# Luka140/paig_reproduction

Measured on AMD Instinct MI355X. Metric: video-seqs/sec (train step) spring_color B=100 @ 1/2/4/8 MI355X, higher is better.
Workload: dtype fp32; 1 GPU; spring_color PhysicsNet train step (get_batch gather+fwd+loss+bwd+allreduce+RMSprop), B=100/rank, 32x32x3, seq_len 50 (4 in / 6 pred / 40 extrap); global_batch=100, seq_len=50, parallelism=dp1, conv_math=split, split_graph=False, optimizer_in_graph=True, byte_targets=True, dataset_seqs=800

## Files before the change

include/paig_hip.h:

```cpp
#ifndef PAIG_HIP_H
#define PAIG_HIP_H
#include <stddef.h>

#ifdef __cplusplus
extern "C" {
#endif

#define PAIG_ABI_VERSION 10
const char* paig_last_error(void);
int paig_abi_version(void);
int paig_f16_range_status(int clear);

int paig_conv2d_fwd(const float* in, long long in_fs, int in_grp, long long in_gs, float* out, long long out_fs,
                    const float* aux, long long aux_fs, const float* w, const float* bias, int F, int Cin, int Cout,
                    int H, int W, int ks, int flags, void* stream);
#define PAIG_XMAX_SLOTS 2048
int paig_conv2d_fwd_ex(const float* in, long long in_fs, int in_grp, long long in_gs, float* out, long long out_fs,
                       const float* aux, long long aux_fs, const float* w, const float* bias, int F, int Cin,
                       int Cout, int H, int W, int ks, int flags, float* xmax, int xmax_n, void* stream);
int paig_conv2d_fwd_pw(const float* in, long long in_fs, int in_grp, long long in_gs, float* out, long long out_fs,
                       const float* aux, long long aux_fs, const float* w, const float* bias, int F, int Cin,
                       int Cout, int H, int W, int ks, int flags, float* xmax, int xmax_n, float* pool_out,
                       long long pool_fs, const void* wprep, void* stream);
int paig_conv2d_fwd_pwc(const float* in, long long in_fs, int in_grp, long long in_gs, float* out, long long out_fs,
                        const float* aux, long long aux_fs, const float* w, const float* bias, int F, int Cin,
                        int Cout, int H, int W, int ks, int flags, float* xmax, int xmax_n, float* pool_out,
                        long long pool_fs, unsigned char* pool_code, long long pool_code_fs, const void* wprep,
                        void* stream);
long long paig_conv_wprep_size(int cin, int cout, int ks);
int paig_conv_wprep(int n, const float* const* w, const int* cin, const int* cout, const int* ks, const int* dg,
                    void* const* out, void* stream);
int paig_conv_wprep_defer(int n, const float* const* w, const int* cin, const int* cout, const int* ks, const int* dg,
                          void* const* out, void* stream);
int paig_conv_wprep_flush(void* stream);
int paig_debug_fwd_block_cap(int cap);
int paig_conv2d_mfma_supported(int what, int Cin, int Cout, int H, int W, int ks, int flags);
int paig_conv2d_wgrad(const float* x, long long x_fs, int x_grp, long long x_gs, const float* dy, long long dy_fs,
                      float* slab, int nblk_max, int* nblk_out, int F, int Cin, int Cout, int H, int W, int ks,
                      int flags, void* stream);
int paig_conv2d_wgrad_ex(const float* x, long long x_fs, int x_grp, long long x_gs, const float* dy, long long dy_fs,
                         float* slab, int nblk_max, int* nblk_out, int F, int Cin, int Cout, int H, int W, int ks,
                         int flags, const float* xmax, int xmax_n, void* stream);
int paig_conv2d_bwd_supported(int Cin, int Cout, int H, int W, int ks, int flags);
int paig_conv2d_bwd(const float* x, long long x_fs, int x_grp, long long x_gs, const float* dy, long long dy_fs,
                    float* dx, long long dx_fs, const float* aux, long long aux_fs, const float* w, float* slab,
                    int nblk_max, int* nblk_out, int F, int Cin, int Cout, int H, int W, int ks, int flags,
                    const float* xmax, int xmax_n, const float* dpool, long long dpool_fs,
                    const unsigned char* pcode, long long pcode_fs, const void* wprep, void* stream);

size_t paig_unet_workspace(int net, int F, int H, int K, int math);
int paig_unet_fwd(int net, int F, int H, int K, int math, const float* x, long long x_fs, int x_grp, long long x_gs,
                  const float* const* w, const float* const* b, float* logits, void* ws, size_t ws_bytes,
                  void* stream);
int paig_unet_bwd(int net, int F, int H, int K, int math, const float* x, long long x_fs, int x_grp, long long x_gs,
                  const float* const* w, const float* logits, const float* dlogits, float* const* dwb, void* ws,
                  size_t ws_bytes, void* stream);
#define PAIG_UNET_HEAD_FUSED 1
#define PAIG_UNET_SEPARATE_BWD 2
#define PAIG_UNET_INFERENCE 4
#define PAIG_UNET_EXT_WPREP 8
#define PAIG_UNET_STANDALONE_UP 16
#define PAIG_UNET_STANDALONE_POOL 32
#define PAIG_PROBE_CONV_FWD 0
#define PAIG_PROBE_CONV_BWD 1
#define PAIG_PROBE_CONV_WGRAD 2
#define PAIG_PROBE_CONV_DGRAD 3
typedef void (*paig_unet_probe_fn)(void* ctx, int event, int op, int conv, int kind, int cin, int cout, int H,
                                   int flags);
size_t paig_unet_workspace_ex(int net, int F, int H, int K, int math, int flags);
long long paig_unet_buffer(int net, int F, int H, int K, int math, int flags, int which, int buf);
int paig_unet_query(int net, int K, int what);
int paig_unet_fwd_ex(int net, int F, int H, int K, int math, int flags, const float* x, long long x_fs, int x_grp,
                     long long x_gs, const float* const* w, const float* const* b, float* logits,
                     const void* const* wprep_fwd, const void* const* wprep_dg, void* ws, size_t ws_bytes,
                     paig_unet_probe_fn probe, void* probe_ctx, void* stream);
int paig_unet_bwd_ex(int net, int F, int H, int K, int math, int flags, const float* x, long long x_fs, int x_grp,
                     long long x_gs, const float* const* w, const float* logits, const float* dlogits,
                     float* const* dwb, int n_extra, const float* const* extra_src, const int* extra_nblk,
                     const int* extra_len, float* const* extra_dst, const void* const* wprep_dg, void* ws,
                     size_t ws_bytes, paig_unet_probe_fn probe, void* probe_ctx, void* stream);

int paig_conv2d_wgrad_pf(const float* x, long long x_fs, int x_grp, long long x_gs, const float* dy, long long dy_fs,
                         const float* dpool, long long dpool_fs, const unsigned char* pcode, long long pcode_fs,
                         float* slab, int nblk_max, int* nblk_out, int F, int Cin, int Cout, int H, int W, int ks,
                         int flags, const float* xmax, int xmax_n, void* stream);

int paig_maxpool2_fwd(const float* x, long long x_fs, float* y, long long y_fs, int F, int C, int H, int W,
                      void* stream);
int paig_maxpool2_fwd_codes(const float* x, long long x_fs, float* y, long long y_fs, unsigned char* code,
                            long long code_fs, int F, int C, int H, int W, void* stream);
int paig_maxpool2_bwd_relu(const float* x, long long x_fs, const float* dy, long long dy_fs, float* dx, long long dx_fs,
                           int F, int C, int H, int W, void* stream);
int paig_upsample2_fwd(const float* s, long long s_fs, float* u, long long u_fs, int F, int C, int Hs, int Ws, int Ho,
                       int Wo, void* stream);
int paig_upsample2_bwd(const float* du, long long du_fs, const float* s, long long s_fs, float* ds, long long ds_fs,
                       int F, int C, int Hs, int Ws, int Ho, int Wo, int relu_mask, void* stream);

int paig_mask_softmax_fwd(const float* logits, const float* x, long long x_fs, int x_grp, long long x_gs, float* masks,
                          float* objs, float* pobjs, int F, int K, int C, int H, int W, void* stream);
int paig_mask_softmax_bwd(const float* logits, const float* x, long long x_fs, int x_grp, long long x_gs,
                          const float* masks, const float* dobjs, float* dlogits, int F, int K, int C, int H, int W,
                          int flags, void* stream);
int paig_head_mask_blocks(int F, int H, int W);
int paig_head_mask_fwd(const float* x12, const float* w, const float* b, const float* x, long long x_fs, int x_grp,
                       long long x_gs, float* masks, float* objs, int F, int K, int H, int W, void* stream);
int paig_head_mask_bwd(const float* x12, const float* w, const float* b, const float* x, long long x_fs, int x_grp,
                       long long x_gs, const float* masks, const float* dobjs, float* dx12, float* slab, int F, int K,
                       int H, int W, void* stream);
int paig_head_mask_fwd_ex(const float* xl, const float* w, const float* b, const float* x, long long x_fs, int x_grp,
                          long long x_gs, float* masks, float* objs, float* pobjs, int F, int K, int CI, int H, int W,
                          int flags, void* stream);
int paig_head_mask_bwd_ex(const float* xl, const float* w, const float* b, const float* x, long long x_fs, int x_grp,
                          long long x_gs, const float* masks, const float* dobjs, float* dxl, float* slab, int F, int K,
                          int CI, int H, int W, int flags, void* stream);
int paig_pos_head_fwd(const float* h3, float* pos, int N, int K, float half, void* stream);
int paig_pos_head_bwd(const float* h3, const float* dpos, float* dh3, int N, int K, float half, void* stream);

size_t paig_gemm_workspace(int M, int N, int K);
int paig_gemm_defer_epilogue(int on);
int paig_gemm_flush(void* stream);
int paig_gemm(int ta, int tb, int M, int N, int K, float alpha, const float* A, long long lda, const float* B,
              long long ldb, float beta, float* C, long long ldc, const float* bias, int act, int auxm,
              const float* aux, long long ldaux, float* rowsum, float* ws, size_t ws_floats, void* stream);
int paig_gemm_ex(int ta, int tb, int M, int N, int K, float alpha, const float* A, long long lda, const float* B,
                 long long ldb, float beta, float* C, long long ldc, const float* bias, int act, int auxm,
                 const float* aux, long long ldaux, float* rowsum, float* ws, size_t ws_floats, int math,
                 void* stream);
size_t paig_gemm_parts_size(int M, int N, int K, int math);
int paig_gemm_parts(int ta, int tb, int M, int N, int K, const float* A, long long lda, const float* B,
                    long long ldb, float* part, size_t part_floats, int math, void* stream);
size_t paig_colsum_workspace(int M, int N);
int paig_colsum(const float* X, int M, int N, long long ld, float* out, int accumulate, float* ws, void* stream);
int paig_slab_reduce(const float* slab, int nblk, long long ld, int len, float* out, int accumulate, void* stream);
int paig_slab_reduce_multi(int ntask, const float* const* src, const int* nblk, const int* len, float* const* dst,
                           int accumulate, void* stream);
int paig_axpby(const float* x, float* y, long long n, float a, float b, void* stream);

int paig_vfn_fwd(const float* W1, const float* b1, const float* W2, const float* b2, float* hout, float* y,
                 float* ypost, int P, void* stream);
int paig_vfn_bwd_blocks(int P);
int paig_vfn_bwd(const float* d, const float* y, int sig, const float* h, const float* W2, float* dW1, float* db1,
                 float* dW2, float* db2, float* part, int P, void* stream);
int paig_vfn_fwd_multi(int n, const float* const* W1, const float* const* b1, const float* const* W2,
                       const float* const* b2, float* const* hout, float* const* y, float* const* ypost, const int* P,
                       void* stream);
int paig_vfn_bwd_multi(int n, const float* const* d, const float* const* y, const int* sig, const float* const* h,
                       const float* const* W2, float* const* dW1, float* const* db1, float* const* dW2,
                       float* const* db2, float* const* part, const int* P, void* stream);
int paig_vfn_bwd1_multi(int n, const float* const* d, const float* const* y, const int* sig, const float* const* h,
                        const float* const* W2, float* const* dW1, float* const* db1, float* const* dW2,
                        float* const* db2, float* const* part, const int* P, void* stream);

int paig_velmlp_fwd(const float* pos, int B, int Te, int K, int S, const float* W0, const float* b0, const float* W2,
                    const float* b2, const float* W4, const float* b4, float* X, float* h1, float* h2, float* vel,
                    void* stream);
int paig_velmlp_vfn_fwd(const float* pos, int B, int Te, int K, int S, const float* W0, const float* b0,
                        const float* W2, const float* b2, const float* W4, const float* b4, float* X, float* h1,
                        float* h2, float* vel, int n, const float* const* vW1, const float* const* vb1,
                        const float* const* vW2, const float* const* vb2, float* const* hout, float* const* y,
                        float* const* ypost, const int* P, void* stream);
int paig_velmlp_bwd_blocks(int rows);
int paig_velmlp_slab_len(int S);
int paig_velmlp_bwd(const float* dvel, const float* X, const float* h1, const float* h2, const float* W0,
                    const float* W2, const float* W4, float* dX, float* slab, int rows, int S, void* stream);

int paig_head_fwd(const float* h2, const float* W3, const float* b3, float* h3, float* pos, int F, int K, int IN,
                  float half, void* stream);
int paig_head_bwd_blocks(int rows);
int paig_head_bwd(const float* h2, const float* h3, const float* dpos, const float* W3, float* dh2, float* slab, int F,
                  int K, int IN, float half, void* stream);
int paig_head_bwd_vel(const float* h2, const float* h3, const float* dpos, const float* W3, float* dh2, float* slab,
                      int F, int K, int IN, float half, const float* dX, const float* dpos0, int B, int Te, int S,
                      int alt, void* stream);
int paig_head_bwd_vel_vfn2(const float* h2, const float* h3, const float* dpos, const float* W3, float* dh2,
                           float* slab, int F, int K, int IN, float half, const float* dX, const float* dpos0, int B,
                           int Te, int S, int alt, int n, const float* const* d, const float* const* y,
                           const int* sig, const float* const* h, const float* const* W2, float* const* dW1,
                           float* const* db1, float* const* dW2, float* const* db2, float* const* part, const int* P,
                           void* stream);

int paig_dense_tail_fwd(const float* part, int S, const float* b1, float* h1, const float* W2, float* W2t,
                        const float* b2, float* h2, const float* W3, const float* b3, float* h3, float* pos, int F,
                        int K, int IN, float half, void* stream);
int paig_head_l2_bwd_blocks(int rows);
int paig_head_l2_bwd(const float* h2, const float* h3, const float* dpos, const float* W3, float* dh2, float* slab,
                     int F, int K, int IN, float half, const float* dX, const float* dpos0, int B, int Te, int S,
                     int alt, const float* W2, const float* h1, float* dh1, int n, const float* const* d,
                     const float* const* y, const int* sig, const float* const* h, const float* const* vW2,
                     float* const* dW1, float* const* db1, float* const* dW2, float* const* db2, float* const* part,
                     const int* P, void* stream);

size_t paig_localiser_workspace(int F, int K, int n1, int IN, int math);
int paig_localiser_fwd(const float* x1, const float* W1, const float* b1, const float* W2, const float* b2,
                       const float* W3, const float* b3, float* h1, float* h2, float* h3, float* pos, int F, int K,
                       int n1, int IN, float half, int math, void* ws, size_t ws_bytes, void* stream);
int paig_localiser_bwd(const float* dpos, const float* x1, const float* h1, const float* h2, const float* h3,
                       const float* W1, const float* W2, const float* W3, float* dl1, float* dl2, float* dl3,
                       float* dx1, int F, int K, int n1, int IN, float half, int math, void* ws, size_t ws_bytes,
                       void* stream);
int paig_velmlp_rollout_fwd(int cell, const float* pos, int B, int Te, int K, int S, const float* W0, const float* b0,
                            const float* W2, const float* b2, const float* W4, const float* b4, float* X, float* h1,
                            float* h2, float* vel0, const float* dt, const double* p0, const double* p1, float* pvs,
                            int R, void* stream);
size_t paig_velmlp_rollout_bwd_workspace(int B, int K, int S);
int paig_velmlp_rollout_bwd(int cell, const float* pvs, const float* dpos_roll, const float* dpvs, const float* dt,
                            const double* p0, const double* p1, const float* X, const float* h1, const float* h2,
                            const float* W0, const float* W2, const float* W4, float* dpos, float* dmlp,
                            double* gparam0, double* gparam1, int B, int Te, int K, int S, int R, void* ws,
                            size_t ws_bytes, void* stream);

int paig_vel_pack(const float* pos, float* X, int B, int Te, int K, int S, int alt, void* stream);
int paig_vel_unpack_add(const float* dX, const float* dpos0, float* dpos, int B, int Te, int K, int S, int alt,
                        void* stream);

int paig_rollout_fwd(int cell, const float* pos0, long long pos0_ld, const float* vel0, const float* dt,
                     const double* p0, const double* p1, float* pvs, int B, int D, int R, void* stream);
int paig_rollout_bwd_blocks(int B);
int paig_rollout_bwd(int cell, const float* pvs, const float* dpos_roll, const float* dpvs, const float* dt,
                     const double* p0, const double* p1, float* dpos0, float* dvel0, double* part, double* gparam0,
                     double* gparam1, int accumulate, int B, int D, int R, void* stream);

int paig_decoder_fwd(const float* pos, long long pos_outer, long long pos_inner, int pos_grp, const float* tmpl,
                     const float* cont, const float* bg, float* out, long long out_fs, const float* tgt,
                     long long tgt_fs, int tgt_grp, long long tgt_gs, float* sse, int F, int K, int h, int H,
                     void* stream);
int paig_decoder_fwd_rollout(int cell, const float* pos0, long long pos0_ld, const float* vel0, const float* dt,
                             const double* p0, const double* p1, float* pvs, int B, int D, int R, const float* pos,
                             long long pos_outer, long long pos_inner, int pos_grp, const float* tmpl,
                             const float* cont, const float* bg, float* out, long long out_fs, const float* tgt,
                             long long tgt_fs, int tgt_grp, long long tgt_gs, float* sse, int F, int K, int h, int H,
                             void* stream);
int paig_decoder_fwd_t8(const float* pos, long long pos_outer, long long pos_inner, int pos_grp, const float* tmpl,
                        const float* cont, const float* bg, float* out, long long out_fs, const unsigned char* tgt,
                        const long long* tgt_idx, long long tgt_fs, int tgt_grp, long long tgt_gs, float* sse, int F,
                        int K, int h, int H, void* stream);
int paig_decoder_bwd_blocks(int F, int pos_grp, int live, int K, int h, int H);
size_t paig_decoder_slab_len(int K, int h, int H);
size_t paig_decoder_bwd_scratch(int F, int K, int h, int H);
int paig_decoder_bwd(const float* pos, long long pos_outer, long long pos_inner, int pos_grp, const float* tmpl,
                     const float* cont, const float* bg, const float* tgt, long long tgt_fs, int tgt_grp,
                     long long tgt_gs, const float* dsse, const float* dout, long long dout_fs, float* dpos,
                     float* slab, float* scratch, int F, int live, int K, int h, int H, void* stream);
int paig_decoder_bwd_ex(const float* pos, long long pos_outer, long long pos_inner, int pos_grp, const float* tmpl,
                        const float* cont, const float* bg, const float* tgt, const unsigned char* tgt8,
                        const long long* tgt_idx, long long tgt_fs, int tgt_grp, long long tgt_gs, const float* dsse,
                        int lw_mode, const float* dt, const float* de, const float* dr, float ae, int lB, int lTe,
                        int lR, int lpred, const float* dout, long long dout_fs, float* dpos, float* slab,
                        float* scratch, int F, int live, int K, int h, int H, void* stream);
int paig_decoder_bwd_t8(const float* pos, long long pos_outer, long long pos_inner, int pos_grp, const float* tmpl,
                        const float* cont, const float* bg, const unsigned char* tgt, const long long* tgt_idx,
                        long long tgt_fs, int tgt_grp, long long tgt_gs, const float* dsse, const float* dout,
                        long long dout_fs, float* dpos, float* slab, float* scratch, int F, int live, int K, int h,
                        int H, void* stream);

int paig_decoder_fwd_sigma(const float* pos, long long pos_outer, long long pos_inner, int pos_grp, const float* tmpl,
                           const float* cont, const float* bg, float* out, long long out_fs, const float* tgt,
                           long long tgt_fs, int tgt_grp, long long tgt_gs, float* sse, int F, int K, int h, int H,
                           double sigma, void* stream);
int paig_decoder_fwd_rollout_sigma(int cell, const float* pos0, long long pos0_ld, const float* vel0, const float* dt,
                                   const double* p0, const double* p1, float* pvs, int B, int D, int R,
                                   const float* pos, long long pos_outer, long long pos_inner, int pos_grp,
                                   const float* tmpl, const float* cont, const float* bg, float* out, long long out_fs,
                                   const float* tgt, long long tgt_fs, int tgt_grp, long long tgt_gs, float* sse, int F,
                                   int K, int h, int H, double sigma, void* stream);
int paig_decoder_fwd_t8_sigma(const float* pos, long long pos_outer, long long pos_inner, int pos_grp,
                              const float* tmpl, const float* cont, const float* bg, float* out, long long out_fs,
                              const unsigned char* tgt, const long long* tgt_idx, long long tgt_fs, int tgt_grp,
                              long long tgt_gs, float* sse, int F, int K, int h, int H, double sigma, void* stream);
int paig_decoder_bwd_blocks_sigma(int F, int pos_grp, int live, int K, int h, int H, double sigma);
size_t paig_decoder_bwd_scratch_sigma(int F, int K, int h, int H, double sigma);
int paig_decoder_bwd_ex_sigma(const float* pos, long long pos_outer, long long pos_inner, int pos_grp,
                              const float* tmpl, const float* cont, const float* bg, const float* tgt,
                              const unsigned char* tgt8, const long long* tgt_idx, long long tgt_fs, int tgt_grp,
                              long long tgt_gs, const float* dsse, int lw_mode, const float* dt, const float* de,
                              const float* dr, float ae, int lB, int lTe, int lR, int lpred, const float* dout,
                              long long dout_fs, float* dpos, float* slab, float* scratch, int F, int live, int K,
                              int h, int H, double sigma, void* stream);
int paig_decoder_parts_sigma(const float* pos, long long pos_inner, const float* tmpl, const float* cont,
                             const float* bg, float* contents, float* masks, int F, int K, int h, int H, double sigma,
                             void* stream);

int paig_decoder_parts(const float* pos, long long pos_inner, const float* tmpl, const float* cont, const float* bg,
                       float* contents, float* masks, int F, int K, int h, int H, void* stream);
// ... 45 lines not shown
```

paig_reproduction_amd/_lib.py:

```python
import ctypes
import os

import torch

_HERE = os.path.dirname(os.path.abspath(__file__))
LIB_PATH = os.path.join(_HERE, "libpaig_hip.so")
XMAX_SLOTS = 2048

AB_PATH = os.environ.get("PAIG_AB_LIB")
ABI_VERSION = 10

P = ctypes.c_void_p
I = ctypes.c_int
LL = ctypes.c_longlong
F32 = ctypes.c_float
F64 = ctypes.c_double
SZ = ctypes.c_size_t

SIGNATURES = {
    "paig_last_error": (ctypes.c_char_p, []),
    "paig_abi_version": (I, []),
    "paig_f16_range_status": (I, [I]),
    "paig_conv2d_fwd": (I, [P, LL, I, LL, P, LL, P, LL, P, P, I, I, I, I, I, I, I, P]),
    "paig_conv2d_wgrad": (I, [P, LL, I, LL, P, LL, P, I, P, I, I, I, I, I, I, I, P]),
    "paig_conv2d_fwd_ex": (I, [P, LL, I, LL, P, LL, P, LL, P, P, I, I, I, I, I, I, I, P, I, P]),
    "paig_conv2d_fwd_pw": (I, [P, LL, I, LL, P, LL, P, LL, P, P, I, I, I, I, I, I, I, P, I, P, LL, P, P]),
    "paig_conv_wprep_size": (LL, [I, I, I]),
    "paig_conv_wprep": (I, [I, P, P, P, P, P, P, P]),
    "paig_conv_wprep_defer": (I, [I, P, P, P, P, P, P, P]),
    "paig_conv_wprep_flush": (I, [P]),
    "paig_conv2d_wgrad_ex": (I, [P, LL, I, LL, P, LL, P, I, P, I, I, I, I, I, I, I, P, I, P]),
    "paig_conv2d_wgrad_pf": (I, [P, LL, I, LL, P, LL, P, LL, P, LL, P, I, P, I, I, I, I, I, I, I, P, I, P]),
    "paig_conv2d_mfma_supported": (I, [I, I, I, I, I, I, I]),
    "paig_debug_fwd_block_cap": (I, [I]),
    "paig_conv2d_bwd_supported": (I, [I, I, I, I, I, I]),
    "paig_conv2d_bwd": (I, [P, LL, I, LL, P, LL, P, LL, P, LL, P, P, I, P, I, I, I, I, I, I, I, P, I, P, LL, P, LL,
                            P, P]),
    "paig_conv2d_fwd_pwc": (I, [P, LL, I, LL, P, LL, P, LL, P, P, I, I, I, I, I, I, I, P, I, P, LL, P, LL, P, P]),
    "paig_gather_u8_f32": (I, [P, P, P, I, LL, P]),
    "paig_gather_u8_f32_ex": (I, [P, P, P, I, LL, LL, P, P]),
    "paig_velmlp_fwd": (I, [P, I, I, I, I, P, P, P, P, P, P, P, P, P, P, P]),
    "paig_velmlp_vfn_fwd": (I, [P, I, I, I, I, P, P, P, P, P, P, P, P, P, P, I, P, P, P, P, P, P, P, P, P]),
    "paig_velmlp_bwd_blocks": (I, [I]),
    "paig_velmlp_slab_len": (I, [I]),
    "paig_velmlp_bwd": (I, [P, P, P, P, P, P, P, P, P, I, I, P]),
    "paig_head_fwd": (I, [P, P, P, P, P, I, I, I, F32, P]),
    "paig_dense_tail_fwd": (I, [P, I, P, P, P, P, P, P, P, P, P, P, I, I, I, F32, P]),
    "paig_head_l2_bwd": (I, [P, P, P, P, P, P, I, I, I, F32, P, P, I, I, I, I, P, P, P, I, P, P, P, P, P, P, P, P, P,
                             P, P, P]),
    "paig_head_bwd_blocks": (I, [I]),
    "paig_head_l2_bwd_blocks": (I, [I]),
    "paig_head_bwd": (I, [P, P, P, P, P, P, I, I, I, F32, P]),
    "paig_head_bwd_vel": (I, [P, P, P, P, P, P, I, I, I, F32, P, P, I, I, I, I, P]),
    "paig_head_bwd_vel_vfn2": (I, [P, P, P, P, P, P, I, I, I, F32, P, P, I, I, I, I, I, P, P, P, P, P, P, P, P, P, P, P,
                                   P]),
    "paig_unet_workspace": (SZ, [I, I, I, I, I]),
    "paig_localiser_workspace": (SZ, [I, I, I, I, I]),
    "paig_localiser_fwd": (I, [P, P, P, P, P, P, P, P, P, P, P, I, I, I, I, F32, I, P, SZ, P]),
    "paig_localiser_bwd": (I, [P, P, P, P, P, P, P, P, P, P, P, P, I, I, I, I, F32, I, P, SZ, P]),
    "paig_velmlp_rollout_fwd": (I, [I, P, I, I, I, I, P, P, P, P, P, P, P, P, P, P, P, P, P, P, I, P]),
    "paig_velmlp_rollout_bwd_workspace": (SZ, [I, I, I]),
    "paig_velmlp_rollout_bwd": (I, [I, P, P, P, P, P, P, P, P, P, P, P, P, P, P, P, P, I, I, I, I, I, P, SZ, P]),
    "paig_unet_fwd": (I, [I, I, I, I, I, P, LL, I, LL, P, P, P, P, SZ, P]),
    "paig_unet_bwd": (I, [I, I, I, I, I, P, LL, I, LL, P, P, P, P, P, SZ, P]),
    "paig_unet_workspace_ex": (SZ, [I, I, I, I, I, I]),
    "paig_unet_buffer": (LL, [I, I, I, I, I, I, I, I]),
    "paig_unet_query": (I, [I, I, I]),
    "paig_unet_fwd_ex": (I, [I, I, I, I, I, I, P, LL, I, LL, P, P, P, P, P, P, SZ, P, P, P]),
    "paig_unet_bwd_ex": (I, [I, I, I, I, I, I, P, LL, I, LL, P, P, P, P, I, P, P, P, P, P, P, SZ, P, P, P]),
    "paig_maxpool2_fwd": (I, [P, LL, P, LL, I, I, I, I, P]),
    "paig_maxpool2_fwd_codes": (I, [P, LL, P, LL, P, LL, I, I, I, I, P]),
    "paig_maxpool2_bwd_relu": (I, [P, LL, P, LL, P, LL, I, I, I, I, P]),
    "paig_upsample2_fwd": (I, [P, LL, P, LL, I, I, I, I, I, I, P]),
    "paig_upsample2_bwd": (I, [P, LL, P, LL, P, LL, I, I, I, I, I, I, I, P]),
    "paig_mask_softmax_fwd": (I, [P, P, LL, I, LL, P, P, P, I, I, I, I, I, P]),
    "paig_mask_softmax_bwd": (I, [P, P, LL, I, LL, P, P, P, I, I, I, I, I, I, P]),
    "paig_head_mask_blocks": (I, [I, I, I]),
    "paig_head_mask_fwd": (I, [P, P, P, P, LL, I, LL, P, P, I, I, I, I, P]),
    "paig_head_mask_bwd": (I, [P, P, P, P, LL, I, LL, P, P, P, P, I, I, I, I, P]),
    "paig_head_mask_fwd_ex": (I, [P, P, P, P, LL, I, LL, P, P, P, I, I, I, I, I, I, P]),
    "paig_head_mask_bwd_ex": (I, [P, P, P, P, LL, I, LL, P, P, P, P, I, I, I, I, I, I, P]),
    "paig_pos_head_fwd": (I, [P, P, I, I, F32, P]),
    "paig_pos_head_bwd": (I, [P, P, P, I, I, F32, P]),
    "paig_gemm_workspace": (SZ, [I, I, I]),
    "paig_gemm_parts_size": (SZ, [I, I, I, I]),
    "paig_gemm_parts": (I, [I, I, I, I, I, P, LL, P, LL, P, SZ, I, P]),
    "paig_gemm_defer_epilogue": (I, [I]),
    "paig_gemm_flush": (I, [P]),
    "paig_gemm": (I, [I, I, I, I, I, F32, P, LL, P, LL, F32, P, LL, P, I, I, P, LL, P, P, SZ, P]),
    "paig_gemm_ex": (I, [I, I, I, I, I, F32, P, LL, P, LL, F32, P, LL, P, I, I, P, LL, P, P, SZ, I, P]),
    "paig_colsum_workspace": (SZ, [I, I]),
    "paig_colsum": (I, [P, I, I, LL, P, I, P, P]),
    "paig_slab_reduce": (I, [P, I, LL, I, P, I, P]),
    "paig_slab_reduce_multi": (I, [I, P, P, P, P, I, P]),
    "paig_axpby": (I, [P, P, LL, F32, F32, P]),
    "paig_vfn_fwd": (I, [P, P, P, P, P, P, P, I, P]),
    "paig_vfn_bwd_blocks": (I, [I]),
    "paig_vfn_bwd": (I, [P, P, I, P, P, P, P, P, P, P, I, P]),
    "paig_vfn_fwd_multi": (I, [I, P, P, P, P, P, P, P, P, P]),
    "paig_vfn_bwd_multi": (I, [I, P, P, P, P, P, P, P, P, P, P, P, P]),
    "paig_vfn_bwd1_multi": (I, [I, P, P, P, P, P, P, P, P, P, P, P, P]),
    "paig_vel_pack": (I, [P, P, I, I, I, I, I, P]),
    "paig_vel_unpack_add": (I, [P, P, P, I, I, I, I, I, P]),
    "paig_rollout_fwd": (I, [I, P, LL, P, P, P, P, P, I, I, I, P]),
    "paig_rollout_bwd_blocks": (I, [I]),
    "paig_rollout_bwd": (I, [I, P, P, P, P, P, P, P, P, P, P, P, I, I, I, I, P]),
    "paig_decoder_fwd": (I, [P, LL, LL, I, P, P, P, P, LL, P, LL, I, LL, P, I, I, I, I, P]),
    "paig_decoder_fwd_rollout": (I, [I, P, LL, P, P, P, P, P, I, I, I, P, LL, LL, I, P, P, P, P, LL, P, LL, I, LL, P, I, I,
                                      I, I, P]),
    "paig_decoder_fwd_t8": (I, [P, LL, LL, I, P, P, P, P, LL, P, P, LL, I, LL, P, I, I, I, I, P]),
    "paig_decoder_bwd_blocks": (I, [I, I, I, I, I, I]),
    "paig_decoder_slab_len": (SZ, [I, I, I]),
    "paig_decoder_bwd_scratch": (SZ, [I, I, I, I]),
    "paig_decoder_bwd": (I, [P, LL, LL, I, P, P, P, P, LL, I, LL, P, P, LL, P, P, P, I, I, I, I, I, P]),
    "paig_decoder_bwd_ex": (I, [P, LL, LL, I, P, P, P, P, P, P, LL, I, LL, P, I, P, P, P, F32, I, I, I, I, P, LL, P, P, P,
                                 I, I, I, I, I, P]),
    "paig_decoder_bwd_t8": (I, [P, LL, LL, I, P, P, P, P, P, LL, I, LL, P, P, LL, P, P, P, I, I, I, I, I, P]),
    "paig_decoder_parts": (I, [P, LL, P, P, P, P, P, I, I, I, I, P]),
    "paig_decoder_fwd_sigma": (I, [P, LL, LL, I, P, P, P, P, LL, P, LL, I, LL, P, I, I, I, I, F64, P]),
    "paig_decoder_fwd_rollout_sigma": (I, [I, P, LL, P, P, P, P, P, I, I, I, P, LL, LL, I, P, P, P, P, LL, P, LL, I, LL,
                                            P, I, I, I, I, F64, P]),
    "paig_decoder_fwd_t8_sigma": (I, [P, LL, LL, I, P, P, P, P, LL, P, P, LL, I, LL, P, I, I, I, I, F64, P]),
    "paig_decoder_bwd_blocks_sigma": (I, [I, I, I, I, I, I, F64]),
    "paig_decoder_bwd_scratch_sigma": (SZ, [I, I, I, I, F64]),
    "paig_decoder_bwd_ex_sigma": (I, [P, LL, LL, I, P, P, P, P, P, P, LL, I, LL, P, I, P, P, P, F32, I, I, I, I, P, LL, P,
                                       P, P, I, I, I, I, I, F64, P]),
    "paig_decoder_parts_sigma": (I, [P, LL, P, P, P, P, P, I, I, I, I, F64, P]),
    "paig_stn_fwd": (I, [P, P, P, I, I, I, I, I, I, P]),
    "paig_stn_bwd": (I, [P, P, P, P, P, I, I, I, I, I, I, P]),
    "paig_stn_fwd_f64": (I, [P, P, P, I, I, I, I, I, I, P]),
    "paig_stn_bwd_f64": (I, [P, P, P, P, P, I, I, I, I, I, I, P]),
    "paig_relu_mask": (I, [P, P, LL, P]),
    "paig_loss_reduce": (I, [P, P, I, I, I, I, F32, P, P, P, P]),
    "paig_loss_bwd": (I, [P, P, P, F32, P, P, I, I, I, I, P]),
    "paig_frame_sse": (I, [P, LL, I, LL, P, LL, I, LL, P, I, I, P]),
    "paig_frame_sse_bwd": (I, [P, LL, I, LL, P, LL, I, LL, P, P, I, I, P]),
    "paig_synth_integrate": (I, [I, P, P, LL, I, I, I, F64, F64, F64, F64, F64, P, P, P]),
    "paig_synth_raster": (I, [P, P, LL, I, I, I, F64, P, P, P]),
    "paig_rmsprop_f32": (I, [P, P, P, LL, F32, F32, F32, P]),
    "paig_rmsprop_f64": (I, [P, P, P, LL, F64, F64, F64, P]),
    "paig_rmsprop_mixed": (I, [P, P, P, LL, P, P, P, LL, F64, F64, F64, P]),
    "paig_adam_f32": (I, [P, P, P, P, LL, F32, F32, F32, F32, F32, F32, P]),
    "paig_adam_f64": (I, [P, P, P, P, LL, F64, F64, F64, F64, F64, F64, P]),
    "paig_sgd_f32": (I, [P, P, P, LL, F32, F32, I, P]),
    "paig_sgd_f64": (I, [P, P, P, LL, F64, F64, I, P]),
}

_QUERY = {"paig_last_error", "paig_abi_version", "paig_f16_range_status", "paig_conv2d_mfma_supported",
          "paig_debug_fwd_block_cap",
          "paig_conv2d_bwd_supported", "paig_velmlp_bwd_blocks",
          "paig_velmlp_slab_len", "paig_head_bwd_blocks", "paig_head_l2_bwd_blocks", "paig_head_mask_blocks", "paig_conv_wprep_size", "paig_gemm_workspace", "paig_colsum_workspace",
          "paig_gemm_parts_size", "paig_gemm_parts", "paig_unet_workspace", "paig_unet_workspace_ex",
          "paig_unet_buffer", "paig_unet_query", "paig_localiser_workspace",
          "paig_velmlp_rollout_bwd_workspace",
          "paig_vfn_bwd_blocks", "paig_rollout_bwd_blocks", "paig_decoder_bwd_blocks", "paig_decoder_slab_len",
          "paig_decoder_bwd_scratch", "paig_decoder_bwd_blocks_sigma", "paig_decoder_bwd_scratch_sigma"}


class PaigError(RuntimeError):
    pass


class _Lib:
    def __init__(self, path=LIB_PATH):
        if not os.path.exists(path):
            raise PaigError(f"libpaig_hip.so not built at {path}: run `make -C paig_reproduction_amd/csrc` "
                            "(or __graft_entry__.build()); there is no CPU fallback")
        self.path = path
        self.dll = ctypes.CDLL(path)
        self.dll.paig_abi_version.restype = I
        self.dll.paig_abi_version.argtypes = []
        ver = self.dll.paig_abi_version()
        if ver != ABI_VERSION:
            raise PaigError(f"{path}: C ABI version {ver}, this binding is version {ABI_VERSION}")
        self.fns = {}
        for name, (rt, args) in SIGNATURES.items():
            if path != LIB_PATH and not hasattr(self.dll, name):
                continue
            f = getattr(self.dll, name)
            f.restype = rt
            f.argtypes = args
            self.fns[name] = f

    def __getattr__(self, name):
        fns = self.__dict__.get("fns")
        if fns is None or name not in fns:
            raise AttributeError(name)
        f = fns[name]
        if name in _QUERY:
            return f

        def call(*a):
            rc = f(*a)
            if rc != 0:
                msg = self.fns["paig_last_error"]().decode(errors="replace")
                raise PaigError(f"{name} failed (rc={rc}): {msg}")
            return rc

        call.__name__ = name
        return call


_lib = None


def lib():
    global _lib
    if _lib is None:
        _lib = _Lib(AB_PATH or LIB_PATH)
    return _lib


def ptr(t):
    return None if t is None else t.data_ptr()


def stream_handle(device=None):
    return torch.cuda.current_stream(device).cuda_stream


def require_device(t):
    if not (torch.is_tensor(t) and t.is_cuda):
        raise PaigError("paig_reproduction_amd runs only on a HIP device (MI355X); got a "
                        f"{'CPU' if torch.is_tensor(t) else type(t).__name__} tensor. There is no CPU fallback.")
```

paig_reproduction_amd/csrc/conv_split.hip:

```cpp
#include "split_common.h"

#ifndef PAIG_FWD_AUXP
#define PAIG_FWD_AUXP 1
#endif

namespace {


constexpr bool sfwd_sla(bool UPS, int PM, int H, int W, int ups_bytes, int lo_bytes) {
  return UPS && PM == 0 && H * W >= 4096 && ups_bytes <= lo_bytes;
}
constexpr int sfwd_lds(int CIN, int H, int W, int KS, bool UPS, int PM, int tpxm, int ntb) {
  const int CC = rup(CIN, 8) / 8, PS = CC % 2 == 0 ? CC + 1 : CC;
  const int NS = ceil_div(KS * KS * CC, 4);
  const int FPT = H * W <= tpxm ? tpxm / (H * W) : 1;
  const int RT = H * W <= tpxm ? H : rows_fit(H, W, tpxm);
  const int TWPX = W + 2 * (KS / 2);
  const int RP = W == 8 ? to_mod16(TWPX * PS, 8) : TWPX * PS;
  const int img = FPT * (RT + KS - 1) * RP * 8, wimg = NS * ntb * 64 * 8;
  const int ups = UPS ? up_window_floats(CIN, FPT, RT, W) * 4 : 0;
  return (img + wimg) * 2 * (PM == 2 ? 1 : 2) + (sfwd_sla(UPS, PM, H, W, ups, img * 2) ? 0 : ups);
}
constexpr int sfwd_vgprs(int CIN, int H, int W, int KS, bool UPS, int tpxm, int ntb) {
  const int CC = rup(CIN, 8) / 8, NS = ceil_div(KS * KS * CC, 4);
  const int FPT = H * W <= tpxm ? tpxm / (H * W) : 1;
  const int RT = H * W <= tpxm ? H : rows_fit(H, W, tpxm);
  const int MW = ceil_div(ceil_div(FPT * RT * W, 16), 4);
  const int NL = UPS ? 1 : ceil_div(FPT * (RT + KS - 1) * (W % 2 == 0 ? W / 2 : W) * CC, 256);
  return MW * ntb * 4 + NL * 30 + ntb * 8 + NS + MW * 8 + 40;
}
#ifndef PAIG_FWD_UPS_TP
#define PAIG_FWD_UPS_TP 256
#endif
#ifndef PAIG_FWD_TP32
#define PAIG_FWD_TP32 256
#endif
constexpr int sfwd_pick(int CIN, int COUT, int H, int W, int KS, bool UPS, int PM) {
  const int base = UPS && H * W < 4096 && PAIG_FWD_UPS_TP < 256   ? PAIG_FWD_UPS_TP
                   : !UPS && H * W == 1024 && PAIG_FWD_TP32 < 256 ? PAIG_FWD_TP32
                                                                  : (W == 8 ? 128 : 256);
  const int NT = ceil_div(COUT, 16);
  for (int pass = UPS && !(PM == 0 && H * W >= 4096) ? 1 : 0; pass < 3; ++pass)
    for (int nb = 1; nb <= NT; ++nb) {
      if (NT % nb != 0 || NT / nb > 4) continue;
      for (int tp = base; tp >= (pass == 1 ? base / 2 : 64); tp /= 2)
        if (sfwd_lds(CIN, H, W, KS, UPS, PM, tp, NT / nb) <= (pass == 0 ? LDS_MAX / 2 : LDS_MAX) &&
            sfwd_vgprs(CIN, H, W, KS, UPS, tp, NT / nb) <= 264 && (pass > 0 || tp >= base / 2))
          return tp * 256 + nb;
    }
  return 0;
}

template <int CIN, int COUT, int H, int W, int KS, bool UPS, int PM>
struct SFwdCfg {
  static constexpr int KK = KS * KS, PADL = KS / 2;
  static constexpr int NIMG = PM == 2 ? 1 : 2;
  static constexpr int CINP = rup(CIN, 8), CC = CINP / 8;
  static constexpr int KC = KK * CC, NS = ceil_div(KC, 4);
  static constexpr int GEO = sfwd_pick(CIN, COUT, H, W, KS, UPS, PM);
  static_assert(GEO > 0, "no forward tile geometry fits the LDS");
  static constexpr int NB = GEO % 256;
  static constexpr int NT = ceil_div(COUT, 16) / NB;
  static constexpr int TPXM = GEO / 256;
  static constexpr int FPT = H * W <= TPXM ? TPXM / (H * W) : 1;
  static constexpr int RT = H * W <= TPXM ? H : rows_fit(H, W, TPXM);
  static constexpr int TPXV = FPT * RT * W;
  static constexpr int NMT = ceil_div(TPXV, 16);
  static constexpr int MW = ceil_div(NMT, 4);
  static constexpr int ROWS = RT + KS - 1;
  static constexpr int TWPX = W + 2 * PADL;
  static constexpr int PS = CC % 2 == 0 ? CC + 1 : CC;
  static constexpr int RP = W == 8 ? to_mod16(TWPX * PS, 8) : TWPX * PS;
  static constexpr int IMG = FPT * ROWS * RP * 8;
  static constexpr int WIMG = NS * NT * 64 * 8;
  static constexpr int SLB = UPS ? up_window_floats(CIN, FPT, RT, W) * 4 : 0;
  static constexpr bool SLA = sfwd_sla(UPS, PM, H, W, SLB, IMG * 2);
  static constexpr int LDS = (IMG + WIMG) * 2 * NIMG + (SLA ? 0 : SLB);
  static constexpr int UPX = W % 2 == 0 ? 2 : 1;
  static constexpr int W2 = W / UPX;
  static constexpr int NI = FPT * ROWS * W2 * CC;
  static constexpr int NL = (NI + 255) / 256;
  static constexpr bool VEC4 = W % 4 == 0;
  static_assert(H % RT == 0, "RT divides H");
  static constexpr int PO = W / 16;
  static constexpr bool POOLOK = !UPS && VEC4 && W % 16 == 0 && PO >= 1 && MW % 2 == 0 && NMT == 4 * MW &&
                                 TPXV % (2 * W) == 0 && RT % 2 == 0;
};

__device__ __forceinline__ float pool4(float a, float b, float c, float d) {
  float m = a;
  if (b > m || b != b) m = b;
  if (c > m || c != c) m = c;
  if (d > m || d != d) m = d;
  return m;
}

__device__ __forceinline__ unsigned char pool_code(float a, float b, float c, float d) {
  float m = a;
  int k = 0;
  if (b > m || b != b) { m = b; k = 1; }
  if (c > m || c != c) { m = c; k = 2; }
  if (d > m || d != d) { m = d; k = 3; }
  return (unsigned char)((a > 0.f ? 1 : 0) | (b > 0.f ? 2 : 0) | (c > 0.f ? 4 : 0) | (d > 0.f ? 8 : 0) | (k << 4));
}

template <int MW, int PO, bool POOL>
__device__ __forceinline__ int fwd_mtile(int wv, int mt) {
  if constexpr (POOL) {
    constexpr int HM = MW / 2;
    const int u = wv * HM + mt % HM;
    return ((u / PO) * 2 + mt / HM) * PO + u % PO;
  } else {
    return wv * MW + mt;
  }
}

template <int CIN, int COUT, int H, int W, int KS, bool DG, bool UPS, int PM, bool POOL = false, bool UPT = false,
          bool PF = false>
__device__ __forceinline__ void conv_fwd_split_body(FView in, FViewW out, FView aux, const float* __restrict__ w,
                                                    const float* __restrict__ bias, int F, int flags, int ntiles, XMax xm,
                                                    const s16x8* __restrict__ wp, PoolOut pout, int bx, int gx) {
  using C = SFwdCfg<CIN, COUT, H, W, KS, UPS, PM>;
  static_assert(!PF || (DG && !UPS && !POOL && !UPT && C::UPX == 2 && H % 2 == 0 && CIN % 8 == 0),
                "pool fold: dgrad staging units of one window's pixel pair");
  static_assert(!UPT || (DG && !UPS && !POOL && C::FPT == 1 && C::RT % 2 == 0 && C::VEC4 && W % 2 == 0),
                "transposed-upsample epilogue: dgrad tiles of whole row pairs");
  constexpr int KK = C::KK, CC = C::CC, KC = C::KC, NS = C::NS, NT = C::NT, MW = C::MW;
  constexpr int RT = C::RT, FPT = C::FPT, ROWS = C::ROWS, PS = C::PS, RP = C::RP;
  constexpr int NI = C::NI, NL = C::NL, PADL = C::PADL, W2 = C::W2;
  constexpr long long PLANE = UPS ? (long long)(H / 2) * (W / 2) : (long long)H * W;
  constexpr long long HW = (long long)H * W;
  extern __shared__ __attribute__((aligned(16))) short lds16[];
  short* Xh = lds16;
  short* Xl = Xh + (C::NIMG == 2 ? C::IMG : 0);
  short* Wh = lds16 + C::NIMG * C::IMG;
  short* Wl = Wh + (C::NIMG == 2 ? C::WIMG : 0);
  const int tid = threadIdx.x, lane = tid & 63, wv = tid >> 6, g = lane >> 4;
  constexpr int NRB = H / RT;
  const int co0 = blockIdx.y * NT * 16;
  float rmax = 0.f;
  __shared__ float smax[4];

  auto wval = [&](int idx, int j) {
    const int ln = idx & 63, snt = idx >> 6, nt = snt % NT, s = snt / NT;
    const int kc = 4 * s + (ln >> 4), co = co0 + nt * 16 + (ln & 15);
    float v = 0.f;
    if (kc < KC && co < COUT) {
      const int tap = kc / CC, ci = (kc % CC) * 8 + j;
      if (ci < CIN) v = DG ? w[(ci * COUT + co) * KK + (KK - 1 - tap)] : w[(co * CIN + ci) * KK + tap];
    }
    return v;
  };
  int ewn[NT];
// ... 1056 lines not shown
        float r1 = 0.f;
        stage_d(t, r1, false);
        __syncthreads();
      }
    }
  };

  auto tile_max = [&](int t) {
    if constexpr (!DSYNC) {
      float m = 0.f;
#pragma unroll
      for (int l = 0; l < NLD; ++l) m = amax2(amax2(m, sd[l][0], sd[l][1]), sd[l][2], sd[l][3]);
      m = wave_max_u(m);
      if (lane == 0) smax[wv] = m;
    }
  };

  if ((int)blockIdx.x < ntiles) issue(xcd_tile(blockIdx.x, ntiles));
  if (PM == 0 && xm.p) {
    float m = 0.f;
    for (int i = tid * 4; i < xm.n; i += 1024) {
      const f32x4 v = *reinterpret_cast<const f32x4*>(xm.p + i);
      m = fmaxf(m, fmaxf(fmaxf(v[0], v[1]), fmaxf(v[2], v[3])));
    }
    m = wave_max_u(m);
    if (lane == 0) smax[wv] = m;
    __syncthreads();
    m = fmaxf(fmaxf(smax[0], smax[1]), fmaxf(smax[2], smax[3]));
    if (m > 0.f) ecx = f16_scale_exp(m);
    __syncthreads();
  }
  xsc = __builtin_amdgcn_ldexpf(1.f, ecx);
  for (int lt = blockIdx.x; lt < ntiles; lt += gridDim.x) {
    const int tile = xcd_tile(lt, ntiles);
    fold_all(tile);
    if constexpr (PM == 0 && PAIG_SCALE_MODE < 2) tile_max(tile);
    __syncthreads();
    commit(tile);
    __syncthreads();
    check_sync(tile);
    issue(lt + (int)gridDim.x < ntiles ? xcd_tile(lt + gridDim.x, ntiles) : ntiles);
#pragma unroll
    for (int kb = wp; kb < KB; kb += WP) {
      const int p0 = kb * 32, fi = p0 / (RT * W), pr = p0 % (RT * W);
      const int base = (fi * ROWS + pr / W) * TWPX + pr % W;
      s16x8 ah[MT], al[MT];
#pragma unroll
      for (int m = 0; m < MT; ++m) {
        const int co = m * 16 + (lane & 15);
        const int o = (co < COUTB ? co : co % COUTB) * DP + p0 + 8 * g;
        ah[m] = *reinterpret_cast<const s16x8*>(Dh + o);
        al[m] = PM != 2 ? *reinterpret_cast<const s16x8*>(Dl + o) : ah[m];
      }
      int r0, r1;
      if constexpr (C::FAST) {
        r0 = (base + roff[0]) * 4;
        r1 = (base + roff[1]) * 4;
      } else {
        auto posof = [&](int j) {
          int pp = p0 + j;
          if (pp >= TPXV) pp = 0;
          const int pf = pp / (RT * W), prr = pp % (RT * W);
          return ((pf * ROWS + prr / W) * TWPX + prr % W + (OFFX - PADL)) * 4;
        };
        r0 = posof(8 * g + qq);
        r1 = posof(8 * g + 4 + qq);
      }
      auto ldb = [&](int jn, s16x8& bh, s16x8& bl) {
        if (wn + jn * WN < NT) {
          bh = __builtin_shufflevector(tr_read(Xh + r0 + colt[jn]), tr_read(Xh + r1 + colt[jn]), 0, 1, 2, 3, 4, 5, 6,
                                       7);
          bl = PM != 2 ? __builtin_shufflevector(tr_read(Xl + r0 + colt[jn]), tr_read(Xl + r1 + colt[jn]), 0, 1, 2,
                                                 3, 4, 5, 6, 7)
                       : bh;
        }
      };
      s16x8 bh[2], bl[2];
      ldb(0, bh[0], bl[0]);
#pragma unroll
      for (int jn = 0; jn < NTW; ++jn) {
        if (jn + 1 < NTW) ldb(jn + 1, bh[(jn + 1) & 1], bl[(jn + 1) & 1]);
        if (wn + jn * WN < NT) {
#pragma unroll
          for (int m = 0; m < MT; ++m) acc[m][jn] = mma3<PM>(ah[m], al[m], bh[jn & 1], bl[jn & 1], acc[m][jn]);
        }
      }
    }
  }
  __syncthreads();
  float* R = reinterpret_cast<float*>(lds16);
#pragma unroll
  for (int m = 0; m < MT; ++m)
#pragma unroll
    for (int j = 0; j < NTW; ++j)
#pragma unroll
      for (int r = 0; r < 4; ++r) R[(((wv * MT + m) * NTW + j) * 4 + r) * 64 + lane] = acc[m][j][r];
  __syncthreads();
  float* s = slab + (long long)blockIdx.x * C::SLAB;
  if (wp == 0) {
#pragma unroll
    for (int m = 0; m < MT; ++m)
#pragma unroll
      for (int j = 0; j < NTW; ++j) {
        const int nt = wn + j * WN;
        if (nt >= NT) continue;
        const int col = nt * 16 + (lane & 15), cq = col >> 2;
        const int tap = cq / CQ, ci = (cq % CQ) * 4 + (col & 3);
#pragma unroll
        for (int r = 0; r < 4; ++r) {
          float v = 0.f;
          for (int p = 0; p < WP; ++p) v += R[((((p * WN + wn) * MT + m) * NTW + j) * 4 + r) * 64 + lane];
          const int co = m * 16 + (lane >> 4) * 4 + r;
          if constexpr (PM == 0) v = __builtin_amdgcn_ldexpf(v, -(ecx + ecd));
          if (co < COUTB && cq < NQ && ci < CINB) s[(co0 + co) * NCOL + (ci0 + ci) * KK + tap] = v;
        }
      }
  }
  __syncthreads();
  float* Rb = reinterpret_cast<float*>(lds16);
#pragma unroll
  for (int l = 0; l < NLD; ++l) Rb[l * 256 + tid] = bacc[l];
  __syncthreads();
  if (tid < COUTB && blockIdx.y == 0) {
    float v = 0.f;
    for (int i = tid * NPU; i < (tid + 1) * NPU; ++i) v += Rb[(i / 256) * 256 + i % 256];
    s[COUT * NCOL + co0 + tid] = v;
  }
  if constexpr (PM == 0) f16_range_note(rmax);
}

struct WPrepJob {
  const float* w;
  s16x8* out;
  int cin, cout, ks, dg;
};
constexpr int WPREP_MAX = 64;
struct WPrepJobs {
  WPrepJob j[WPREP_MAX];
  int blk0[WPREP_MAX + 1];
  int n;
};
constexpr int WPREP_T = 256;

__device__ __forceinline__ int wprep_hdr_entries(int cout) { return (cout + 15) / 16 * 16 * 4 / 16; }

#ifndef PAIG_WPREP_S
#define PAIG_WPREP_S 8
#endif
constexpr int WPREP_S = PAIG_WPREP_S;
__device__ __forceinline__ void conv_wprep_body(const WPrepJobs& jobs, int bid) {
  int q = 0;
  while (q + 1 < jobs.n && bid >= jobs.blk0[q + 1]) ++q;
  const WPrepJob jb = jobs.j[q];
  if (jb.dg == 2) {
    __shared__ float T[32][33];
    const int bl = bid - jobs.blk0[q], tx = (bl % ((jb.cin + 31) / 32)) * 32,
              ty = (bl / ((jb.cin + 31) / 32)) * 32, c = threadIdx.x & 31, r = threadIdx.x >> 5;
    for (int y = r; y < 32; y += WPREP_T / 32)
      if (ty + y < jb.cout && tx + c < jb.cin) T[y][c] = jb.w[(long long)(ty + y) * jb.cin + tx + c];
    __syncthreads();
    float* o = reinterpret_cast<float*>(jb.out);
    for (int y = r; y < 32; y += WPREP_T / 32)
      if (tx + y < jb.cin && ty + c < jb.cout) o[(long long)(tx + y) * jb.cout + ty + c] = T[c][y];
    return;
  }
  const int KK = jb.ks * jb.ks, CC = (jb.cin + 7) / 8, KC = KK * CC, NTT = (jb.cout + 15) / 16, NS = (KC + 3) / 4;
  const int NSC = (NS + WPREP_S - 1) / WPREP_S;
  const int bl = bid - jobs.blk0[q], nt = bl / NSC, s0 = (bl % NSC) * WPREP_S;
  const int tid = threadIdx.x;
  auto wv = [&](int kc, int j, int co) {
    float v = 0.f;
    if (kc < KC && co < jb.cout) {
      const int tap = kc / CC, ci = (kc % CC) * 8 + j;
      if (ci < jb.cin) v = jb.dg ? jb.w[(ci * jb.cout + co) * KK + (KK - 1 - tap)] : jb.w[(co * jb.cin + ci) * KK + tap];
    }
    return v;
  };
  __shared__ float red[WPREP_T];
  __shared__ int ex[16];
  const int cl = tid & 15, co = nt * 16 + cl;
  float m = 0.f;
#pragma unroll 8
  for (int i = tid >> 4; i < KC * 8; i += WPREP_T / 16) m = fmaxf(m, fabsf(wv(i >> 3, i & 7, co)));
  red[tid] = m;
  __syncthreads();
  if (tid < 16) {
    float mm = 0.f;
    for (int r = 0; r < WPREP_T / 16; ++r) mm = fmaxf(mm, red[r * 16 + tid]);
    ex[tid] = f16_scale_exp_v(mm);
    if (s0 == 0) reinterpret_cast<int*>(jb.out)[nt * 16 + tid] = ex[tid];
  }
  __syncthreads();
  const int HDR = wprep_hdr_entries(jb.cout), ENT = NS * NTT * 64;
  short* img = reinterpret_cast<short*>(jb.out + HDR);
  const int ns = NS - s0 < WPREP_S ? NS - s0 : WPREP_S;
#pragma unroll 8
  for (int t = tid; t < ns * 64 * 8; t += WPREP_T) {
    const int j = t & 7, ln = (t >> 3) & 63, s = s0 + (t >> 9);
    const int kc = 4 * s + (ln >> 4), c = nt * 16 + (ln & 15);
    float rm = 0.f;
    short h, l;
    split<0>(__builtin_amdgcn_ldexpf(wv(kc, j, c), ex[ln & 15]), h, l, rm);
    const long long e = (long long)(s * NTT + nt) * 64 + ln;
    img[e * 8 + j] = h;
    img[((long long)ENT + e) * 8 + j] = l;
  }
}

__global__ void __launch_bounds__(WPREP_T) conv_wprep_k(WPrepJobs jobs) { conv_wprep_body(jobs, blockIdx.x); }

template <int CIN, int COUT, int H, int W, int KS, int PM>
__global__ void __launch_bounds__(256, 2)
conv_fwd_wprep_k(FView in, FViewW out, FView aux, const float* __restrict__ w, const float* __restrict__ bias, int F,
                 int flags, int ntiles, XMax xm, PoolOut pout, WPrepJobs jobs, int nwp) {
  if ((int)blockIdx.x < nwp) {
    conv_wprep_body(jobs, blockIdx.x);
    return;
  }
  conv_fwd_split_body<CIN, COUT, H, W, KS, false, false, PM>(in, out, aux, w, bias, F, flags, ntiles, xm, nullptr, pout,
                                                            (int)blockIdx.x - nwp, (int)gridDim.x - nwp);
}

WPrepJobs g_wpend{};
int g_wpend_blocks = 0;
int wprep_build(WPrepJobs& jobs, int n, const float* const* w, const int* cin, const int* cout, const int* ks,
                const int* dg, void* const* out, int* blocks_out) {
  jobs = WPrepJobs{};
  jobs.n = n;
  int blocks = 0;
  for (int q = 0; q < n; ++q) {
    PAIG_REQUIRE(w[q] && out[q] && cin[q] > 0 && cout[q] > 0 && ks[q] > 0, "conv_wprep: job %d", q);
    PAIG_REQUIRE(((uintptr_t)out[q] & 15) == 0, "conv_wprep: job %d output not 16-byte aligned", q);
    jobs.j[q] = WPrepJob{w[q], static_cast<s16x8*>(out[q]), cin[q], cout[q], ks[q], dg[q]};
    jobs.blk0[q] = blocks;
    if (dg[q] == 2) {
      blocks += (cin[q] + 31) / 32 * ((cout[q] + 31) / 32);
      continue;
    }
    const int NS = (ks[q] * ks[q] * ((cin[q] + 7) / 8) + 3) / 4;
    blocks += (cout[q] + 15) / 16 * ((NS + WPREP_S - 1) / WPREP_S);
  }
  jobs.blk0[n] = blocks;
  *blocks_out = blocks;
  return 0;
}
int wprep_flush(hipStream_t st) {
  if (!g_wpend_blocks) return 0;
  const int nb = g_wpend_blocks;
  g_wpend_blocks = 0;
  hipLaunchKernelGGL(conv_wprep_k, dim3(nb), dim3(WPREP_T), 0, st, g_wpend);
  PAIG_CHECK_LAUNCH();
  return 0;
}

static int g_fwd_block_cap = 0;
static XMax g_prezero{};

template <int CIN, int COUT, int H, int W, int KS, bool DG, bool UPS, int PM, bool UPT = false, bool PF = false>
static int sfwd_launch(FView in, FViewW out, FView aux, const float* w, const float* b, int F, int flags,
                       hipStream_t st, XMax xm, const void* wp, PoolOut pout) {
  using C = SFwdCfg<CIN, COUT, H, W, KS, UPS, PM>;
  constexpr int LDS = C::LDS;
  static_assert(C::SLB == (UPS ? UpStage<CIN, H, W, C::FPT, C::RT>::SL * 4 : 0), "upsample window bytes");
  const int ntiles = cdiv(F, C::FPT) * (H / C::RT);
  constexpr bool POOLABLE = C::POOLOK && !DG;
  auto k = PF ? conv_fwd_split_k<CIN, COUT, H, W, KS, DG, UPS, PM, false, false, PF>
         : UPT ? conv_fwd_split_k<CIN, COUT, H, W, KS, DG, UPS, PM, false, UPT>
              : (POOLABLE && (flags & 64)) ? conv_fwd_split_k<CIN, COUT, H, W, KS, DG, UPS, PM, POOLABLE>
                                           : conv_fwd_split_k<CIN, COUT, H, W, KS, DG, UPS, PM, false>;
  static int resident[2] = {0, 0};
  const int kv = (POOLABLE && (flags & 64)) ? 1 : 0;
  if (!resident[kv]) {
    if (LDS > 64 * 1024) (void)hipFuncSetAttribute((const void*)k, hipFuncAttributeMaxDynamicSharedMemorySize, LDS);
    resident[kv] = persistent_grid((const void*)k, LDS);
  }
  static const int bpc = [] {
    const char* e = getenv("PAIG_FWD_BPC");
    return e ? atoi(e) : 0;
  }();
  int res = resident[kv];
  if (bpc > 0 && res > bpc * 256) res = bpc * 256;
  int nb = res / C::NB;
  if (nb > (UPT ? F : ntiles)) nb = UPT ? F : ntiles;
  if (g_fwd_block_cap > 0 && nb > g_fwd_block_cap) nb = g_fwd_block_cap;
  if (nb < 1) nb = 1;
  if (PM != 0 || DG) xm.p = nullptr;
  PAIG_REQUIRE(!xm.p || nb <= xm.n, "conv split fwd: %d blocks need more than %d xmax slots", nb, xm.n);
  if (xm.p && g_prezero.z) {
    xm.z = g_prezero.z;
    xm.zn = g_prezero.zn;
    g_prezero = XMax{};
  }
  if (PF) PAIG_REQUIRE(pout.p && pout.code, "conv split dgrad: the pool fold needs the pooled gradient and codes");
  else if (flags & 64) PAIG_REQUIRE(C::POOLOK && pout.p, "conv split fwd: no fused pool for Cin=%d Cout=%d H=%d", CIN, COUT, H);
  if constexpr (CIN == 3 && PM == 0 && !DG && !UPS && !UPT && !PF && C::NB == 1) {
    if (g_wpend_blocks && !(flags & 64)) {
      auto km = conv_fwd_wprep_k<CIN, COUT, H, W, KS, PM>;
      static bool attr = false;
      if (!attr && LDS > 64 * 1024) (void)hipFuncSetAttribute((const void*)km, hipFuncAttributeMaxDynamicSharedMemorySize, LDS);
      attr = true;
      const int nwp = g_wpend_blocks;
      g_wpend_blocks = 0;
      hipLaunchKernelGGL(km, dim3(nwp + nb), dim3(256), LDS, st, in, out, aux, w, b, F, flags, ntiles, xm, pout, g_wpend,
                         nwp);
      PAIG_CHECK_LAUNCH();
      return 0;
    }
  }
  if (int rc = wprep_flush(st)) return rc;
  hipLaunchKernelGGL(k, dim3(nb, C::NB), dim3(256), LDS, st, in, out, aux, w, b, F, flags, ntiles, xm,
                     PM == 0 ? static_cast<const s16x8*>(wp) : nullptr, pout);
  PAIG_CHECK_LAUNCH();
  return 0;
}

template <int CIN, int COUT, int H, int W, int KS, bool UPS, int PM, bool PF = false>
static int swg_launch(FView x, FView dy, float* slab, int nblk_max, int* nblk_out, int F, hipStream_t st, XMax xm,
                      PoolOut pin = PoolOut{nullptr, 0, nullptr, 0}) {
  using C = SWgCfg<CIN, COUT, H, W, KS, UPS, PM>;
  constexpr int STG = C::STG + (UPS && !C::SLA ? UpStage<C::CINB, H, W, C::FPT, C::RT>::SL * 4 : 0);
  constexpr int LDS = STG > C::RED ? STG : C::RED;
  const int ntiles = cdiv(F, C::FPT) * (H / C::RT);
  auto k = conv_wgrad_split_k<CIN, COUT, H, W, KS, UPS, PM, PF>;
  if constexpr (PF) PAIG_REQUIRE(pin.p && pin.code, "conv split wgrad: the pool fold needs the pooled gradient and codes");
  static int resident = 0;
  if (!resident) {
    if (LDS > 64 * 1024) (void)hipFuncSetAttribute((const void*)k, hipFuncAttributeMaxDynamicSharedMemorySize, LDS);
    resident = persistent_grid((const void*)k, LDS);
  }
  int nb = ntiles < nblk_max ? ntiles : nblk_max;
  if (nb > resident / (C::NSI * C::NSO)) nb = resident / (C::NSI * C::NSO);
  if (nb < 1) nb = 1;
  *nblk_out = nb;
  PAIG_REQUIRE(!xm.p || (xm.n % 4 == 0 && (reinterpret_cast<uintptr_t>(xm.p) & 15) == 0),
               "conv split wgrad: xmax needs 16-byte alignment and a multiple of 4 slots (%d)", xm.n);
  hipLaunchKernelGGL(k, dim3(nb, C::NSI, C::NSO), dim3(256), LDS, st, x, dy, slab, F, ntiles, xm, pin);
  PAIG_CHECK_LAUNCH();
  return 0;
}

#define PAIG_SPLIT_FWD(X)                                                                                 \
  X(3, 8, 32, 3) X(8, 8, 32, 3) X(8, 16, 16, 3) X(16, 16, 16, 3) X(16, 32, 8, 3) X(32, 32, 8, 3)         \
  X(32, 16, 16, 3) X(16, 16, 32, 3) X(24, 8, 32, 3) X(8, 2, 32, 1) X(16, 8, 16, 3) X(8, 24, 32, 3)       \
  X(2, 8, 32, 1) X(32, 16, 8, 3) X(16, 32, 16, 3)                                                         \
  PAIG_SPLIT_FWD_3BP(X) PAIG_SPLIT_FWD_UNET(X)
#define PAIG_SPLIT_WG(X)                                                                                  \
  X(3, 8, 32, 3) X(8, 8, 32, 3) X(8, 16, 16, 3) X(16, 16, 16, 3) X(16, 32, 8, 3) X(32, 32, 8, 3)         \
  X(32, 16, 16, 3) X(16, 16, 32, 3) X(24, 8, 32, 3) X(8, 2, 32, 1)                                        \
  PAIG_SPLIT_WG_3BP(X) PAIG_SPLIT_WG_UNET(X)
#define PAIG_SPLIT_UP(X)                                                                                  \
  X(32, 16, 16, 3) X(16, 16, 32, 3) X(32, 16, 18, 3) X(16, 16, 36, 3) X(128, 32, 16, 3) X(64, 32, 32, 3) \
  X(32, 32, 64, 3)
#define PAIG_SPLIT_PF(X) X(32, 32, 32, 3) PAIG_SPLIT_PF_C6(X)
#ifndef PAIG_PF_C6
#define PAIG_PF_C6 0
#endif
#if PAIG_PF_C6
#define PAIG_SPLIT_PF_C6(X) X(64, 64, 16, 3)
#else
#define PAIG_SPLIT_PF_C6(X)
#endif
#define PAIG_SPLIT_UPT(X) X(32, 128, 16, 3) X(32, 64, 32, 3) X(32, 32, 64, 3)
#define PAIG_SPLIT_FWD_3BP(X)                                                                             \
  X(3, 8, 36, 3) X(8, 8, 36, 3) X(8, 16, 18, 3) X(16, 16, 18, 3) X(16, 32, 9, 3) X(32, 32, 9, 3)         \
  X(32, 16, 18, 3) X(16, 16, 36, 3) X(24, 8, 36, 3) X(8, 3, 36, 1) X(16, 8, 18, 3) X(32, 16, 9, 3)       \
  X(16, 32, 18, 3) X(8, 24, 36, 3) X(3, 8, 36, 1)
#define PAIG_SPLIT_FWD_UNET(X)                                                                            \
  X(3, 16, 64, 3) X(16, 16, 64, 3) X(16, 32, 32, 3) X(32, 32, 32, 3) X(32, 64, 16, 3) X(64, 64, 16, 3)   \
  X(64, 128, 8, 3) X(128, 128, 8, 3) X(96, 64, 16, 3) X(64, 32, 32, 3) X(48, 16, 64, 3) X(16, 2, 64, 1)   \
  X(32, 16, 32, 3) X(64, 32, 16, 3) X(128, 64, 8, 3) X(32, 128, 16, 3) X(64, 96, 16, 3) X(32, 64, 32, 3)  \
  X(32, 32, 64, 3) X(16, 48, 64, 3) X(2, 16, 64, 1)
#define PAIG_SPLIT_WG_UNET(X)                                                                             \
  X(3, 16, 64, 3) X(16, 16, 64, 3) X(16, 32, 32, 3) X(32, 32, 32, 3) X(32, 64, 16, 3) X(64, 64, 16, 3)   \
  X(64, 128, 8, 3) X(128, 128, 8, 3) X(96, 64, 16, 3) X(64, 32, 32, 3) X(48, 16, 64, 3) X(16, 2, 64, 1)
#define PAIG_SPLIT_WG_3BP(X)                                                                              \
  X(3, 8, 36, 3) X(8, 8, 36, 3) X(8, 16, 18, 3) X(16, 16, 18, 3) X(16, 32, 9, 3) X(32, 32, 9, 3)         \
  X(32, 16, 18, 3) X(16, 16, 36, 3) X(24, 8, 36, 3) X(8, 3, 36, 1)

}

int paig_conv_split_fwd(FView in, FViewW out, FView aux, const float* w, const float* b, int F, int Cin, int Cout,
                        int H, int W, int ks, int flags, hipStream_t st, int* rc, XMax xm, const void* wp,
                        PoolOut pout) {
  const bool dg = (flags & 8) != 0, up = (flags & 32) != 0, b16 = (flags & 256) != 0;
  const int fl = flags & (7 | 64);
  if (H != W || !(flags & (128 | 256))) return 0;
  if (in.grp > 0 && H * W < 256) return 0;
// ... 184 lines not shown
```

paig_reproduction_amd/csrc/gemm.hip:

```cpp
#include "common.h"

#include <algorithm>
#include <cstdlib>

namespace {

constexpr int BM = 64, BN = 64, BK = 32;
constexpr int LDRK = BK + 2;
constexpr int LDKR = 64 + 16;
constexpr int IMG = (BK * LDKR > 64 * LDRK ? BK * LDKR : 64 * LDRK);

typedef float f32x4 __attribute__((ext_vector_type(4)));

__device__ __attribute__((aligned(16))) float zero16[4];

template <bool KCONTIG>
struct Tile {
  f32x4 v[2];
  __device__ __forceinline__ void load(const float* __restrict__ p, long long ld, int r0, int k0, int R, int K,
                                       bool vec, int tid) {
#pragma unroll
    for (int e = 0; e < 2; ++e) {
      int r, k;
      if (KCONTIG) { r = (tid >> 3) + 32 * e; k = (tid & 7) * 4; }
      else { k = (tid >> 4) + 16 * e; r = (tid & 15) * 4; }
      const int gr = r0 + r, gk = k0 + k;
      f32x4 x = f32x4{0.f, 0.f, 0.f, 0.f};
      if (KCONTIG) {
        if (gr < R) {
          const float* q = p + (long long)gr * ld + gk;
          if (vec && gk + 3 < K) x = *reinterpret_cast<const f32x4*>(q);
          else
#pragma unroll
            for (int i = 0; i < 4; ++i) x[i] = (gk + i < K) ? q[i] : 0.f;
        }
      } else {
        if (gk < K) {
          const float* q = p + (long long)gk * ld + gr;
          if (vec && gr + 3 < R) x = *reinterpret_cast<const f32x4*>(q);
          else
#pragma unroll
            for (int i = 0; i < 4; ++i) x[i] = (gr + i < R) ? q[i] : 0.f;
        }
      }
      v[e] = x;
    }
  }
  template <bool VEC>
  __device__ __forceinline__ void load_bf(const float* __restrict__ p, long long ld, int r0, int k0, int R, int K,
                                          int tid) {
#pragma unroll
    for (int e = 0; e < 2; ++e) {
      int r, k;
      if (KCONTIG) { r = (tid >> 3) + 32 * e; k = (tid & 7) * 4; }
      else { k = (tid >> 4) + 16 * e; r = (tid & 15) * 4; }
      const int gr = r0 + r, gk = k0 + k;
      if constexpr (VEC) {
        const bool ok = gr < R && gk < K;
        const float* q = ok ? p + (KCONTIG ? (long long)gr * ld + gk : (long long)gk * ld + gr) : zero16;
        v[e] = *reinterpret_cast<const f32x4*>(q);
      } else {
#pragma unroll
        for (int i = 0; i < 4; ++i) {
          const int rr = KCONTIG ? gr : gr + i, kk = KCONTIG ? gk + i : gk;
          const bool ok = rr < R && kk < K;
          v[e][i] = *(ok ? p + (KCONTIG ? (long long)rr * ld + kk : (long long)kk * ld + rr) : zero16);
        }
      }
    }
  }
  __device__ __forceinline__ void store(float* img, int tid) const {
#pragma unroll
    for (int e = 0; e < 2; ++e) {
      if (KCONTIG) {
        const int r = (tid >> 3) + 32 * e, k = (tid & 7) * 4;
        float* q = img + r * LDRK + k;
        *reinterpret_cast<float2*>(q) = make_float2(v[e][0], v[e][1]);
        *reinterpret_cast<float2*>(q + 2) = make_float2(v[e][2], v[e][3]);
      } else {
        const int k = (tid >> 4) + 16 * e, r = (tid & 15) * 4;
        *reinterpret_cast<f32x4*>(img + k * LDKR + r) = v[e];
      }
    }
  }
  static __device__ __forceinline__ float at(const float* img, int r, int k) {
    return KCONTIG ? img[r * LDRK + k] : img[k * LDKR + r];
  }
};

struct PendEpi {
  int M, N, S;
  const float* part;
  float* C;
  long long ldc;
  float beta;
  const float* bias;
  int act, auxm;
  const float* aux;
  long long ldaux;
  const float* rowpart;
  float* rowsum;
  int v4;
};
__device__ void splitk_epi_run(const PendEpi& pe, int bid, int nb);
#define PAIG_PENDING_EPI(pe)                                                      \
  if ((pe).S && (int)blockIdx.z == (int)gridDim.z - 1) {                          \
    splitk_epi_run((pe), blockIdx.x + gridDim.x * blockIdx.y, gridDim.x * gridDim.y); \
    return;                                                                      \
  }

struct TileId {
  int x, y, z;
};
__device__ __forceinline__ TileId xcd_tile(int gz) {
  const int nx = gridDim.x, ny = gridDim.y, total = nx * ny * gz;
  int lin = blockIdx.x + nx * (blockIdx.y + ny * blockIdx.z);
  if (total % 8 == 0) lin = (lin % 8) * (total / 8) + lin / 8;
  TileId t;
  if (nx <= ny) {
    t.x = lin % nx;
    t.y = (lin / nx) % ny;
    t.z = lin / (nx * ny);
  } else {
    t.y = lin % ny;
    t.x = (lin / ny) % nx;
    t.z = lin / (nx * ny);
  }
  return t;
}

template <bool TA, bool TB>
__global__ void __launch_bounds__(256)
gemm_k(int M, int N, int K, int kchunk, float alpha, const float* __restrict__ A, long long lda, int veca,
       const float* __restrict__ B, long long ldb, int vecb, float* __restrict__ C, long long ldc, float beta,
       const float* __restrict__ bias, int act, int auxm, const float* __restrict__ aux, long long ldaux,
       float* __restrict__ part, float* __restrict__ rowsum, float* __restrict__ rowpart, PendEpi pe) {
  PAIG_PENDING_EPI(pe)
  __shared__ __attribute__((aligned(16))) float As[IMG];
  __shared__ __attribute__((aligned(16))) float Bs[IMG];
  const int tid = threadIdx.x;
  const int lane = tid & 63, wv = tid >> 6;
  const int wm = wv >> 1, wn = wv & 1;
  const TileId bt = xcd_tile((int)gridDim.z - (pe.S ? 1 : 0));
  const int m0 = bt.y * BM, n0 = bt.x * BN;
  const int kbeg = bt.z * kchunk;
  int kend = kbeg + kchunk;
  if (kend > K) kend = K;
  const bool do_rs = rowsum != nullptr && bt.x == 0;

  f32x4 acc[2][2];
#pragma unroll
  for (int i = 0; i < 2; ++i)
#pragma unroll
    for (int j = 0; j < 2; ++j) acc[i][j] = f32x4{0.f, 0.f, 0.f, 0.f};
  float rs = 0.f;

  Tile<!TA> ta;
  Tile<TB> tb;
  if (kbeg < kend) {
    ta.load(A, lda, m0, kbeg, M, kend, veca, tid);
    tb.load(B, ldb, n0, kbeg, N, kend, vecb, tid);
  }
  for (int k0 = kbeg; k0 < kend; k0 += BK) {
    __syncthreads();
    ta.store(As, tid);
    tb.store(Bs, tid);
    __syncthreads();
    if (k0 + BK < kend) {
      ta.load(A, lda, m0, k0 + BK, M, kend, veca, tid);
      tb.load(B, ldb, n0, k0 + BK, N, kend, vecb, tid);
    }
    if (do_rs && tid < BM) {
#pragma unroll 8
      for (int k = 0; k < BK; ++k) rs += Tile<!TA>::at(As, tid, k);
    }
#pragma unroll
    for (int ks = 0; ks < BK; ks += 4) {
      const int kr = ks + (lane >> 4);
      float a[2], b[2];
#pragma unroll
      for (int i = 0; i < 2; ++i) a[i] = Tile<!TA>::at(As, wm * 32 + i * 16 + (lane & 15), kr);
#pragma unroll
      for (int j = 0; j < 2; ++j) b[j] = Tile<TB>::at(Bs, wn * 32 + j * 16 + (lane & 15), kr);
#pragma unroll
      for (int i = 0; i < 2; ++i)
#pragma unroll
        for (int j = 0; j < 2; ++j) acc[i][j] = __builtin_amdgcn_mfma_f32_16x16x4f32(a[i], b[j], acc[i][j], 0, 0, 0);
    }
  }
  if (do_rs && tid < BM && m0 + tid < M) {
    if (rowpart) rowpart[(long long)bt.z * M + m0 + tid] = alpha * rs;
    else rowsum[m0 + tid] = alpha * rs;
  }

#pragma unroll
  for (int i = 0; i < 2; ++i)
#pragma unroll
    for (int j = 0; j < 2; ++j)
#pragma unroll
      for (int r = 0; r < 4; ++r) {
        const int m = m0 + wm * 32 + i * 16 + (lane >> 4) * 4 + r;
        const int n = n0 + wn * 32 + j * 16 + (lane & 15);
        if (m < M && n < N) {
          float v = alpha * acc[i][j][r];
          if (part) {
            part[((long long)bt.z * M + m) * N + n] = v;
          } else {
            if (beta != 0.f) v += beta * C[(long long)m * ldc + n];
            if (bias) v += bias[n];
            C[(long long)m * ldc + n] = epi(v, act, auxm, aux, (long long)m * ldaux + n);
          }
        }
      }
}

typedef short s16x8 __attribute__((ext_vector_type(8)));
typedef short s16x4 __attribute__((ext_vector_type(4)));
typedef __bf16 bf16x8 __attribute__((ext_vector_type(8)));
typedef _Float16 f16x8 __attribute__((ext_vector_type(8)));
typedef __attribute__((address_space(3))) s16x4 lds_s16x4;
typedef unsigned u32x2 __attribute__((ext_vector_type(2)));

constexpr int SPK = 48;
constexpr int SPR = 80;
constexpr int SIMG = 64 * SPK > BK * SPR ? 64 * SPK : BK * SPR;

__device__ __forceinline__ int kperm(int k) {
  const int g = k >> 3, h = (k >> 2) & 1, q = k & 3;
  return 16 * (g >> 1) + 8 * h + 4 * (g & 1) + q;
}

#define F16PM(PM) ((PM) == 1 || (PM) == 4 || (PM) == 5 || (PM) == 6)
#define SCALED(PM) ((PM) >= 4)

template <int PM>
__device__ __forceinline__ void gsplit(float v, short& h, short& l, float& rmax) {
  if constexpr (F16PM(PM)) {
    rmax = fmaxf(rmax, fabsf(v));
    const _Float16 a = (_Float16)v;
    h = __builtin_bit_cast(short, a);
    l = __builtin_bit_cast(short, (_Float16)(v - (float)a));
  } else {
    const __bf16 a = (__bf16)v;
    h = __builtin_bit_cast(short, a);
    l = PM == 2 ? __builtin_bit_cast(short, (__bf16)(v - (float)a)) : (short)0;
  }
}

template <int PM>
__device__ __forceinline__ f32x4 gmma(s16x8 a, s16x8 b, f32x4 c) {
  if constexpr (F16PM(PM))
    return __builtin_amdgcn_mfma_f32_16x16x32_f16(__builtin_bit_cast(f16x8, a), __builtin_bit_cast(f16x8, b), c, 0,
                                                  0, 0);
  else
    return __builtin_amdgcn_mfma_f32_16x16x32_bf16(__builtin_bit_cast(bf16x8, a), __builtin_bit_cast(bf16x8, b), c,
                                                   0, 0, 0);
}

template <bool KCONTIG, int PM>
__device__ __forceinline__ void store16(const Tile<KCONTIG>& t, short* ih, short* il, int tid, float sc,
                                        float& rmax) {
#pragma unroll
  for (int e = 0; e < 2; ++e) {
    s16x4 hv, lv;
    if constexpr (F16PM(PM)) {
      const pf32x2 a = pf32x2{t.v[e][0], t.v[e][1]} * sc, b = pf32x2{t.v[e][2], t.v[e][3]} * sc;
      rmax = amax2(amax2(rmax, a.x, a.y), b.x, b.y);
      u32x2 h, l;
      { const HiLo q_ = split_pk(a.x, a.y); h[0] = q_.h; l[0] = q_.l; }
      { const HiLo q_ = split_pk(b.x, b.y); h[1] = q_.h; l[1] = q_.l; }
      hv = __builtin_bit_cast(s16x4, h);
      lv = __builtin_bit_cast(s16x4, l);
    } else {
#pragma unroll
      for (int i = 0; i < 4; ++i) {
        short h, l;
        gsplit<PM>(t.v[e][i] * sc, h, l, rmax);
        hv[i] = h;
        lv[i] = l;
      }
    }
    int o;
    if (KCONTIG) o = ((tid >> 3) + 32 * e) * SPK + (tid & 7) * 4;
    else o = kperm((tid >> 4) + 16 * e) * SPR + (tid & 15) * 4;
    *reinterpret_cast<s16x4*>(ih + o) = hv;
    if (PM != 3) *reinterpret_cast<s16x4*>(il + o) = lv;
  }
}

template <bool KCONTIG>
__device__ __forceinline__ s16x8 frag16(const short* img, int r0, int lane) {
  if (KCONTIG) return *reinterpret_cast<const s16x8*>(img + (r0 + (lane & 15)) * SPK + 8 * (lane >> 4));
  const int g = lane >> 4, q = (lane >> 2) & 3, p = lane & 3;
  const short* b0 = img + kperm(8 * g + q) * SPR + r0 + 4 * p;
  const short* b1 = img + kperm(8 * g + 4 + q) * SPR + r0 + 4 * p;
  const s16x4 lo = __builtin_amdgcn_ds_read_tr16_b64_v4i16((lds_s16x4*)b0);
  const s16x4 hi = __builtin_amdgcn_ds_read_tr16_b64_v4i16((lds_s16x4*)b1);
  return __builtin_shufflevector(lo, hi, 0, 1, 2, 3, 4, 5, 6, 7);
}

template <bool TA, bool TB, int PM, bool VEC>
__global__ void __launch_bounds__(256) __attribute__((amdgpu_waves_per_eu(6)))
gemm_split_k(int M, int N, int K, int kchunk, float alpha, const float* __restrict__ A, long long lda, int veca,
             const float* __restrict__ B, long long ldb, int vecb, float* __restrict__ C, long long ldc, float beta,
             const float* __restrict__ bias, int act, int auxm, const float* __restrict__ aux, long long ldaux,
             float* __restrict__ part, float* __restrict__ rowsum, float* __restrict__ rowpart, PendEpi pe) {
  PAIG_PENDING_EPI(pe)
  constexpr int NI = PM == 3 ? 1 : 2;
  __shared__ __attribute__((aligned(16))) short S16[4 * SIMG];
  short* Ah = S16;
  short* Al = S16 + SIMG;
  short* Bh = S16 + 2 * SIMG;
  short* Bl = S16 + 3 * SIMG;
  const int tid = threadIdx.x;
  const int lane = tid & 63, wv = tid >> 6;
  const int wm = wv >> 1, wn = wv & 1;
  const TileId bt = xcd_tile((int)gridDim.z - (pe.S ? 1 : 0));
  const int m0 = bt.y * BM, n0 = bt.x * BN;
  const int kbeg = bt.z * kchunk;
  int kend = kbeg + kchunk;
  if (kend > K) kend = K;
  const bool do_rs = TA && rowsum != nullptr && bt.x == 0;

  f32x4 acc[2][2];
#pragma unroll
  for (int i = 0; i < 2; ++i)
#pragma unroll
    for (int j = 0; j < 2; ++j) acc[i][j] = f32x4{0.f, 0.f, 0.f, 0.f};
  f32x4 rs4 = f32x4{0.f, 0.f, 0.f, 0.f};
  float rmax = 0.f;
  constexpr bool DA = PM == 4 || PM == 6, DB = PM == 6;
  int eca = DA ? 100 : (PM == 5 ? PAIG_A_EXP : 0);
  int ecb = DB ? 100 : (PM == 4 || PM == 5 ? PAIG_A_EXP : 0);
  float asc = __builtin_amdgcn_ldexpf(1.f, eca);
  float bsc = __builtin_amdgcn_ldexpf(1.f, ecb);
  __shared__ float smx[8];

  constexpr int NS = 1;
  Tile<!TA> ta[NS];
  Tile<TB> tb[NS];
#pragma unroll
  for (int st = 0; st < NS; ++st) {
    ta[st].template load_bf<VEC>(A, lda, m0, kbeg + st * BK, M, kend, tid);
    tb[st].template load_bf<VEC>(B, ldb, n0, kbeg + st * BK, N, kend, tid);
  }
  for (int k0 = kbeg; k0 < kend; k0 += NS * BK) {
#pragma unroll
    for (int st = 0; st < NS; ++st) {
      const int kk = k0 + st * BK;
      if (kk < kend) {
      if constexpr (DA) {
        float ma = 0.f;
#pragma unroll
        for (int e = 0; e < 2; ++e) ma = amax2(amax2(ma, ta[st].v[e][0], ta[st].v[e][1]), ta[st].v[e][2], ta[st].v[e][3]);
        ma = wave_max_u(ma);
        if (lane == 0) smx[wv] = ma;
      }
      if constexpr (DB) {
        float mb = 0.f;
#pragma unroll
        for (int e = 0; e < 2; ++e) mb = amax2(amax2(mb, tb[st].v[e][0], tb[st].v[e][1]), tb[st].v[e][2], tb[st].v[e][3]);
        mb = wave_max_u(mb);
        if (lane == 0) smx[4 + wv] = mb;
      }
      __syncthreads();
      if constexpr (DA || DB) {
        int na = eca, nb = ecb;
        if constexpr (DA) na = min(eca, f16_scale_exp(fmaxf(fmaxf(smx[0], smx[1]), fmaxf(smx[2], smx[3]))));
        if constexpr (DB) nb = min(ecb, f16_scale_exp(fmaxf(fmaxf(smx[4], smx[5]), fmaxf(smx[6], smx[7]))));
        if (na + nb < eca + ecb) {
#pragma unroll
          for (int i = 0; i < 2; ++i)
#pragma unroll
            for (int j = 0; j < 2; ++j)
#pragma unroll
              for (int r = 0; r < 4; ++r)
                acc[i][j][r] = __builtin_amdgcn_ldexpf(acc[i][j][r], (na + nb) - (eca + ecb));
        }
        eca = na;
        ecb = nb;
        asc = __builtin_amdgcn_ldexpf(1.f, eca);
        bsc = __builtin_amdgcn_ldexpf(1.f, ecb);
      }
      float dmx = 0.f;
      store16<!TA, PM>(ta[st], Ah, Al, tid, asc, DA ? dmx : rmax);
      store16<TB, PM>(tb[st], Bh, Bl, tid, bsc, DB ? dmx : rmax);
      if (do_rs) rs4 += ta[st].v[0] + ta[st].v[1];
      __syncthreads();
      }
      ta[st].template load_bf<VEC>(A, lda, m0, kk + NS * BK, M, kend, tid);
      tb[st].template load_bf<VEC>(B, ldb, n0, kk + NS * BK, N, kend, tid);
      if (kk < kend) {
      s16x8 ah[2], al[2], bh[2], bl[2];
#pragma unroll
      for (int i = 0; i < 2; ++i) {
        ah[i] = frag16<!TA>(Ah, wm * 32 + i * 16, lane);
        al[i] = PM != 3 ? frag16<!TA>(Al, wm * 32 + i * 16, lane) : ah[i];
      }
#pragma unroll
      for (int j = 0; j < 2; ++j) {
        bh[j] = frag16<TB>(Bh, wn * 32 + j * 16, lane);
        bl[j] = PM != 3 ? frag16<TB>(Bl, wn * 32 + j * 16, lane) : bh[j];
      }
#pragma unroll
      for (int i = 0; i < 2; ++i)
#pragma unroll
        for (int j = 0; j < 2; ++j) {
          if constexpr (PM != 3) {
            acc[i][j] = gmma<PM>(al[i], bh[j], acc[i][j]);
            acc[i][j] = gmma<PM>(ah[i], bl[j], acc[i][j]);
          }
          acc[i][j] = gmma<PM>(ah[i], bh[j], acc[i][j]);
        }
      }
    }
  }
  if (do_rs) {
    __syncthreads();
    float* red = reinterpret_cast<float*>(S16);
    *reinterpret_cast<f32x4*>(red + (tid >> 4) * 64 + (tid & 15) * 4) = rs4;
    __syncthreads();
    if (tid < BM && m0 + tid < M) {
      float v = 0.f;
#pragma unroll
      for (int k = 0; k < 16; ++k) v += red[k * 64 + tid];
      if (rowpart) rowpart[(long long)bt.z * M + m0 + tid] = alpha * v;
      else rowsum[m0 + tid] = alpha * v;
    }
  }
#pragma unroll
  for (int i = 0; i < 2; ++i)
#pragma unroll
    for (int j = 0; j < 2; ++j)
#pragma unroll
      for (int r = 0; r < 4; ++r) {
        const int m = m0 + wm * 32 + i * 16 + (lane >> 4) * 4 + r;
        const int n = n0 + wn * 32 + j * 16 + (lane & 15);
        if (m < M && n < N) {
          float v = alpha * (SCALED(PM) ? __builtin_amdgcn_ldexpf(acc[i][j][r], -(eca + ecb)) : acc[i][j][r]);
          if (part) {
            part[((long long)bt.z * M + m) * N + n] = v;
          } else {
            if (beta != 0.f) v += beta * C[(long long)m * ldc + n];
            if (bias) v += bias[n];
            C[(long long)m * ldc + n] = epi(v, act, auxm, aux, (long long)m * ldaux + n);
          }
        }
      }
  if constexpr (F16PM(PM)) f16_range_note(rmax);
}

template <bool KCONTIG, int ROWS>
struct WTile {
  static constexpr int NTHR = 512;
  static constexpr int E = ROWS * BK / (4 * NTHR);
  static constexpr int RQ = ROWS / 4;
  f32x4 v[E];
  static __device__ __forceinline__ void rk(int tid, int e, int& r, int& k) {
    if (KCONTIG) { r = (tid >> 3) + (NTHR / 8) * e; k = (tid & 7) * 4; }
    else { r = (tid % RQ) * 4; k = tid / RQ + (NTHR / RQ) * e; }
  }
  template <bool VEC>
  __device__ __forceinline__ void load_bf(const float* __restrict__ p, long long ld, int r0, int k0, int R, int K,
                                          int tid) {
#pragma unroll
    for (int e = 0; e < E; ++e) {
      int r, k;
      rk(tid, e, r, k);
      const int gr = r0 + r, gk = k0 + k;
      if constexpr (VEC) {
        const bool ok = gr < R && gk < K;
        const float* q = ok ? p + (KCONTIG ? (long long)gr * ld + gk : (long long)gk * ld + gr) : zero16;
        v[e] = *reinterpret_cast<const f32x4*>(q);
      } else {
#pragma unroll
        for (int i = 0; i < 4; ++i) {
          const int rr = KCONTIG ? gr : gr + i, kk = KCONTIG ? gk + i : gk;
          const bool ok = rr < R && kk < K;
          v[e][i] = *(ok ? p + (KCONTIG ? (long long)rr * ld + kk : (long long)kk * ld + rr) : zero16);
        }
      }
    }
  }
  static constexpr int SPRW = ROWS + 16;
  static constexpr int IMG = ROWS * SPK > BK * SPRW ? ROWS * SPK : BK * SPRW;
  template <int PM>
  __device__ __forceinline__ void store16(short* ih, short* il, int tid, float sc, float& rmax) const {
#pragma unroll
    for (int e = 0; e < E; ++e) {
      const pf32x2 a = pf32x2{v[e][0], v[e][1]} * sc, b = pf32x2{v[e][2], v[e][3]} * sc;
      s16x4 hv, lv;
      if constexpr (F16PM(PM)) {
        rmax = amax2(amax2(rmax, a.x, a.y), b.x, b.y);
        u32x2 h, l;
        { const HiLo q_ = split_pk(a.x, a.y); h[0] = q_.h; l[0] = q_.l; }
        { const HiLo q_ = split_pk(b.x, b.y); h[1] = q_.h; l[1] = q_.l; }
        hv = __builtin_bit_cast(s16x4, h);
        lv = __builtin_bit_cast(s16x4, l);
      } else {
        const float t[4] = {a.x, a.y, b.x, b.y};
#pragma unroll
        for (int i = 0; i < 4; ++i) {
          short hh, ll;
          gsplit<PM>(t[i], hh, ll, rmax);
          hv[i] = hh;
          lv[i] = ll;
        }
      }
      int r, k;
      rk(tid, e, r, k);
      const int o = KCONTIG ? r * SPK + k : kperm(k) * SPRW + r;
      *reinterpret_cast<s16x4*>(ih + o) = hv;
      if (PM != 3) *reinterpret_cast<s16x4*>(il + o) = lv;
    }
  }
  __device__ __forceinline__ float amax() const {
    float m = 0.f;
#pragma unroll
    for (int e = 0; e < E; ++e) m = amax2(amax2(m, v[e][0], v[e][1]), v[e][2], v[e][3]);
    return m;
  }
  static __device__ __forceinline__ s16x8 frag(const short* img, int r0, int lane) {
    if (KCONTIG) return *reinterpret_cast<const s16x8*>(img + (r0 + (lane & 15)) * SPK + 8 * (lane >> 4));
    const int g = lane >> 4, q = (lane >> 2) & 3, p = lane & 3;
    const short* b0 = img + kperm(8 * g + q) * SPRW + r0 + 4 * p;
    const short* b1 = img + kperm(8 * g + 4 + q) * SPRW + r0 + 4 * p;
    const s16x4 lo = __builtin_amdgcn_ds_read_tr16_b64_v4i16((lds_s16x4*)b0);
    const s16x4 hi = __builtin_amdgcn_ds_read_tr16_b64_v4i16((lds_s16x4*)b1);
    return __builtin_shufflevector(lo, hi, 0, 1, 2, 3, 4, 5, 6, 7);
  }
};

template <bool TA, bool TB, int PM, bool VEC, int BMT, int BNT>
__global__ void __launch_bounds__(512)
gemm_split_w_k(int M, int N, int K, int kchunk, float alpha, const float* __restrict__ A, long long lda, int veca,
               const float* __restrict__ B, long long ldb, int vecb, float* __restrict__ C, long long ldc, float beta,
               const float* __restrict__ bias, int act, int auxm, const float* __restrict__ aux, long long ldaux,
               float* __restrict__ part, float* __restrict__ rowsum, float* __restrict__ rowpart, PendEpi pe) {
  PAIG_PENDING_EPI(pe)
  constexpr int WM = BMT == 64 ? 2 : 4, WN = 8 / WM;
  constexpr int PMW = BMT / WM, PNW = BNT / WN;
  constexpr int MI = PMW / 16, NJ = PNW / 16;
  using TTA = WTile<!TA, BMT>;
  using TTB = WTile<TB, BNT>;
  constexpr int IA = TTA::IMG, IB = TTB::IMG;
  __shared__ __attribute__((aligned(16))) short S16[2 * IA + 2 * IB];
  short* Ah = S16;
  short* Al = S16 + IA;
  short* Bh = S16 + 2 * IA;
  short* Bl = Bh + IB;
  const int tid = threadIdx.x;
  const int lane = tid & 63, wv = tid >> 6;
  const int wm = wv / WN, wn = wv % WN;
  const TileId bt = xcd_tile((int)gridDim.z - (pe.S ? 1 : 0));
  const int m0 = bt.y * BMT, n0 = bt.x * BNT;
  const int kbeg = bt.z * kchunk;
  int kend = kbeg + kchunk;
  if (kend > K) kend = K;
  const bool do_rs = TA && rowsum != nullptr && bt.x == 0;

  f32x4 acc[MI][NJ];
#pragma unroll
  for (int i = 0; i < MI; ++i)
#pragma unroll
    for (int j = 0; j < NJ; ++j) acc[i][j] = f32x4{0.f, 0.f, 0.f, 0.f};
  f32x4 rs4 = f32x4{0.f, 0.f, 0.f, 0.f};
  float rmax = 0.f;
  constexpr bool DA = PM == 4 || PM == 6, DB = PM == 6;
  int eca = DA ? 100 : (PM == 5 ? PAIG_A_EXP : 0);
  int ecb = DB ? 100 : (PM == 4 || PM == 5 ? PAIG_A_EXP : 0);
  float asc = __builtin_amdgcn_ldexpf(1.f, eca);
  float bsc = __builtin_amdgcn_ldexpf(1.f, ecb);
  __shared__ float smx[16];

  constexpr int NS = 3;
  TTA ta[NS];
  TTB tb[NS];
#pragma unroll
  for (int st = 0; st < NS; ++st) {
    ta[st].template load_bf<VEC>(A, lda, m0, kbeg + st * BK, M, kend, tid);
    tb[st].template load_bf<VEC>(B, ldb, n0, kbeg + st * BK, N, kend, tid);
  }
  for (int k0 = kbeg; k0 < kend; k0 += NS * BK) {
#pragma unroll
    for (int st = 0; st < NS; ++st) {
      const int kk = k0 + st * BK;
      if (kk < kend) {
      if constexpr (DA) {
        const float ma = wave_max_u(ta[st].amax());
        if (lane == 0) smx[wv] = ma;
      }
      if constexpr (DB) {
        const float mb = wave_max_u(tb[st].amax());
        if (lane == 0) smx[8 + wv] = mb;
      }
      __syncthreads();
      if constexpr (DA || DB) {
        int na = eca, nb = ecb;
        if constexpr (DA) {
          float m = smx[0];
#pragma unroll
          for (int w = 1; w < 8; ++w) m = fmaxf(m, smx[w]);
          na = min(eca, f16_scale_exp(m));
        }
        if constexpr (DB) {
          float m = smx[8];
#pragma unroll
          for (int w = 9; w < 16; ++w) m = fmaxf(m, smx[w]);
          nb = min(ecb, f16_scale_exp(m));
        }
        if (na + nb < eca + ecb) {
#pragma unroll
          for (int i = 0; i < MI; ++i)
#pragma unroll
            for (int j = 0; j < NJ; ++j)
#pragma unroll
              for (int r = 0; r < 4; ++r)
                acc[i][j][r] = __builtin_amdgcn_ldexpf(acc[i][j][r], (na + nb) - (eca + ecb));
        }
        eca = na;
        ecb = nb;
        asc = __builtin_amdgcn_ldexpf(1.f, eca);
        bsc = __builtin_amdgcn_ldexpf(1.f, ecb);
      }
      float dmx = 0.f;
      ta[st].template store16<PM>(Ah, Al, tid, asc, DA ? dmx : rmax);
      tb[st].template store16<PM>(Bh, Bl, tid, bsc, DB ? dmx : rmax);
      if (do_rs) {
#pragma unroll
        for (int e = 0; e < TTA::E; ++e) rs4 += ta[st].v[e];
      }
      __syncthreads();
      }
      ta[st].template load_bf<VEC>(A, lda, m0, kk + NS * BK, M, kend, tid);
      tb[st].template load_bf<VEC>(B, ldb, n0, kk + NS * BK, N, kend, tid);
      if (kk < kend) {
      s16x8 ah[MI], al[MI], bh[NJ], bl[NJ];
#pragma unroll
      for (int i = 0; i < MI; ++i) {
        ah[i] = TTA::frag(Ah, wm * PMW + i * 16, lane);
        al[i] = PM != 3 ? TTA::frag(Al, wm * PMW + i * 16, lane) : ah[i];
      }
#pragma unroll
      for (int j = 0; j < NJ; ++j) {
        bh[j] = TTB::frag(Bh, wn * PNW + j * 16, lane);
        bl[j] = PM != 3 ? TTB::frag(Bl, wn * PNW + j * 16, lane) : bh[j];
      }
#pragma unroll
      for (int i = 0; i < MI; ++i)
#pragma unroll
        for (int j = 0; j < NJ; ++j) {
          if constexpr (PM != 3) {
            acc[i][j] = gmma<PM>(al[i], bh[j], acc[i][j]);
            acc[i][j] = gmma<PM>(ah[i], bl[j], acc[i][j]);
          }
          acc[i][j] = gmma<PM>(ah[i], bh[j], acc[i][j]);
        }
      }
    }
  }
  if (do_rs) {
    constexpr int RQ = TTA::RQ, G = 512 / RQ;
    __syncthreads();
    float* red = reinterpret_cast<float*>(S16);
    *reinterpret_cast<f32x4*>(red + (tid / RQ) * BMT + (tid % RQ) * 4) = rs4;
    __syncthreads();
    if (tid < BMT && m0 + tid < M) {
      float v = 0.f;
#pragma unroll
      for (int k = 0; k < G; ++k) v += red[k * BMT + tid];
      if (rowpart) rowpart[(long long)bt.z * M + m0 + tid] = alpha * v;
      else rowsum[m0 + tid] = alpha * v;
    }
  }
#pragma unroll
  for (int i = 0; i < MI; ++i)
#pragma unroll
    for (int j = 0; j < NJ; ++j)
#pragma unroll
      for (int r = 0; r < 4; ++r) {
        const int m = m0 + wm * PMW + i * 16 + (lane >> 4) * 4 + r;
        const int n = n0 + wn * PNW + j * 16 + (lane & 15);
        if (m < M && n < N) {
          float v = alpha * (SCALED(PM) ? __builtin_amdgcn_ldexpf(acc[i][j][r], -(eca + ecb)) : acc[i][j][r]);
          if (part) {
            part[((long long)bt.z * M + m) * N + n] = v;
          } else {
            if (beta != 0.f) v += beta * C[(long long)m * ldc + n];
            if (bias) v += bias[n];
            C[(long long)m * ldc + n] = epi(v, act, auxm, aux, (long long)m * ldaux + n);
          }
        }
      }
  if constexpr (F16PM(PM)) f16_range_note(rmax);
}

__device__ __forceinline__ float sum_strided(const float* __restrict__ p, long long ld, int S) {
  float v = 0.f;
  int s = 0;
  for (; s + 8 <= S; s += 8) {
    float t[8];
#pragma unroll
    for (int j = 0; j < 8; ++j) t[j] = p[(long long)(s + j) * ld];
#pragma unroll
    for (int j = 0; j < 8; ++j) v += t[j];
  }
  for (; s < S; ++s) v += p[(long long)s * ld];
  return v;
}

__device__ __forceinline__ void splitk_epi_scalar(int M, int N, int S, const float* __restrict__ part,
                                                  float* __restrict__ C, long long ldc, float beta,
                                                  const float* __restrict__ bias, int act, int auxm,
                                                  const float* __restrict__ aux, long long ldaux,
                                                  const float* __restrict__ rowpart, float* __restrict__ rowsum, int bid,
                                                  int nb) {
  const long long n_el = (long long)M * N;
  const long long tot = n_el + (rowsum ? M : 0);
  for (long long i = bid * (long long)blockDim.x + threadIdx.x; i < tot; i += (long long)nb * blockDim.x) {
    if (i >= n_el) {
      const int m = (int)(i - n_el);
      rowsum[m] = sum_strided(rowpart + m, M, S);
      continue;
    }
    const int m = (int)(i / N), n = (int)(i % N);
    float v = sum_strided(part + i, n_el, S);
    if (beta != 0.f) v += beta * C[(long long)m * ldc + n];
    if (bias) v += bias[n];
    C[(long long)m * ldc + n] = epi(v, act, auxm, aux, (long long)m * ldaux + n);
  }
}
__global__ void gemm_splitk_epilogue_k(int M, int N, int S, const float* __restrict__ part, float* __restrict__ C,
                                       long long ldc, float beta, const float* __restrict__ bias, int act, int auxm,
                                       const float* __restrict__ aux, long long ldaux, const float* __restrict__ rowpart,
                                       float* __restrict__ rowsum) {
  splitk_epi_scalar(M, N, S, part, C, ldc, beta, bias, act, auxm, aux, ldaux, rowpart, rowsum, blockIdx.x, gridDim.x);
}

__device__ __forceinline__ void splitk_epi_vec(int M, int N, int S, const float* __restrict__ part,
                                               float* __restrict__ C, int ldc, float beta,
                                               const float* __restrict__ bias, int act, int auxm,
                                               const float* __restrict__ aux, int ldaux,
                                               const float* __restrict__ rowpart, float* __restrict__ rowsum, int bid,
                                               int nb) {
  const int n_el = M * N, n4 = n_el >> 2;
  const int tot = n4 + (rowsum ? M : 0);
  for (int i = bid * blockDim.x + threadIdx.x; i < tot; i += nb * blockDim.x) {
    if (i >= n4) {
      const int m = i - n4;
      rowsum[m] = sum_strided(rowpart + m, M, S);
      continue;
    }
    const int e = i << 2, m = e / N, n = e - m * N;
    float4 v = make_float4(0.f, 0.f, 0.f, 0.f);
    int s = 0;
    for (; s + 8 <= S; s += 8) {
      float4 t[8];
#pragma unroll
      for (int j = 0; j < 8; ++j) t[j] = *reinterpret_cast<const float4*>(part + (s + j) * n_el + e);
#pragma unroll
      for (int j = 0; j < 8; ++j) { v.x += t[j].x; v.y += t[j].y; v.z += t[j].z; v.w += t[j].w; }
    }
    for (; s < S; ++s) {
      const float4 a = *reinterpret_cast<const float4*>(part + s * n_el + e);
      v.x += a.x; v.y += a.y; v.z += a.z; v.w += a.w;
    }
    float* c = C + m * ldc + n;
    if (beta != 0.f) {
      const float4 o = *reinterpret_cast<const float4*>(c);
      v.x += beta * o.x; v.y += beta * o.y; v.z += beta * o.z; v.w += beta * o.w;
    }
    if (bias) {
      const float4 b = *reinterpret_cast<const float4*>(bias + n);
      v.x += b.x; v.y += b.y; v.z += b.z; v.w += b.w;
    }
    const long long ao = (long long)m * ldaux + n;
    v.x = epi(v.x, act, auxm, aux, ao);
    v.y = epi(v.y, act, auxm, aux, ao + 1);
    v.z = epi(v.z, act, auxm, aux, ao + 2);
    v.w = epi(v.w, act, auxm, aux, ao + 3);
    *reinterpret_cast<float4*>(c) = v;
  }
}
__global__ void __launch_bounds__(256) gemm_splitk_epilogue_v_k(int M, int N, int S, const float* __restrict__ part,
                                                                float* __restrict__ C, int ldc, float beta,
                                                                const float* __restrict__ bias, int act, int auxm,
                                                                const float* __restrict__ aux, int ldaux,
                                                                const float* __restrict__ rowpart,
                                                                float* __restrict__ rowsum) {
  splitk_epi_vec(M, N, S, part, C, ldc, beta, bias, act, auxm, aux, ldaux, rowpart, rowsum, blockIdx.x, gridDim.x);
}

__device__ void splitk_epi_run(const PendEpi& pe, int bid, int nb) {
  if (pe.v4)
    splitk_epi_vec(pe.M, pe.N, pe.S, pe.part, pe.C, (int)pe.ldc, pe.beta, pe.bias, pe.act, pe.auxm, pe.aux,
                   (int)pe.ldaux, pe.rowpart, pe.rowsum, bid, nb);
  else
    splitk_epi_scalar(pe.M, pe.N, pe.S, pe.part, pe.C, pe.ldc, pe.beta, pe.bias, pe.act, pe.auxm, pe.aux, pe.ldaux,
                      pe.rowpart, pe.rowsum, bid, nb);
}

static int choose_split(int M, int N, int K) {
  const int tiles = cdiv(M, BM) * cdiv(N, BN);
  int s = 1;
  if (K < 512) {
    static int sk = -1;
    if (sk < 0) {
      const char* e = getenv("PAIG_GEMM_SMALLK");
      sk = e ? atoi(e) : 0;
    }
    return (sk && tiles < 256 && K >= 4 * BK) ? 2 : 1;
  }
  while (tiles * s < 512 && cdiv(K, 2 * s) >= BK && (long long)(2 * s) * M * N <= (4ll << 20)) s *= 2;
  return s;
}

struct GemmPlan {
  int tile, S;
};
static int gemm_tile_env() {
  static int v = -2;
  if (v == -2) {
    const char* e = getenv("PAIG_GEMM_TILE");
    v = e ? atoi(e) : -1;
  }
  return v;
}
static GemmPlan plan_gemm(int M, int N, int K, int math) {
  GemmPlan p{0, K > 0 ? choose_split(M, N, K) : 1};
  if (!(math == 3 || math == 4 || math == 6) || gemm_tile_env() == 0 || K <= 0) return p;
  int tile = 0;
  if (N > 128 && N <= 256 && M >= 512 && K >= 512) tile = 1;
  if (!tile) return p;
  int S = 1;
  while (K / (2 * S) >= 384) S *= 2;
  if ((long long)S * M * N > (8ll << 20) || cdiv(M, 64) * S < 128) return p;
  return GemmPlan{tile, S};
}

static inline bool vec_ok(const float* p, long long ld) {
  return ((uintptr_t)p % 16 == 0) && (ld % 4 == 0);
}

template <bool TA, bool TB>
static void launch_gemm(int math, int tile, dim3 grid, hipStream_t st, int M, int N, int K, int kchunk, float alpha,
                        const float* A, long long lda, int va, const float* B, long long ldb, int vb, float* C,
                        long long ldc, float beta, const float* bias, int act, int auxm, const float* aux,
                        long long ldaux, float* part, float* rowsum, float* rowpart, const PendEpi& pe) {
  if (pe.S) grid.z += 1;
#define PAIG_L(KERN)                                                                                          \
  hipLaunchKernelGGL(KERN, grid, dim3(256), 0, st, M, N, K, kchunk, alpha, A, lda, va, B, ldb, vb, C, ldc, beta, \
                     bias, act, auxm, aux, ldaux, part, rowsum, rowpart, pe)
  const bool v = va && vb;
#define PAIG_W(KERN) \
  hipLaunchKernelGGL(KERN, grid, dim3(512), 0, st, M, N, K, kchunk, alpha, A, lda, va, B, ldb, vb, C, ldc, beta, \
                     bias, act, auxm, aux, ldaux, part, rowsum, rowpart, pe)
#define PAIG_S(PM_) \
  do {                                              \
    if (v) PAIG_L((gemm_split_k<TA, TB, PM_, true>)); \
    else PAIG_L((gemm_split_k<TA, TB, PM_, false>));  \
  } while (0)
#define PAIG_SW(PM_) \
  do {                                                                  \
    if (tile == 1) PAIG_W((gemm_split_w_k<TA, TB, PM_, true, 64, 256>)); \
    else if (tile == 2) PAIG_W((gemm_split_w_k<TA, TB, PM_, true, 256, 64>)); \
    else PAIG_S(PM_);                                                   \
  } while (0)
  if (math == 1) PAIG_S(1);
  else if (math == 2) PAIG_S(2);
  else if (math == 3) PAIG_SW(3);
  else if (math == 4) PAIG_SW(4);
  else if (math == 5) PAIG_S(5);
  else if (math == 6) PAIG_SW(6);
  else PAIG_L((gemm_k<TA, TB>));
#undef PAIG_SW
#undef PAIG_S
#undef PAIG_W
#undef PAIG_L
}

}

static PendEpi make_epi(int M, int N, int S, const float* part, float* C, long long ldc, float beta, const float* bias,
                        int act, int auxm, const float* aux, long long ldaux, const float* rowpart, float* rowsum) {
  const bool v4 = N % 4 == 0 && vec_ok(C, ldc) && (!bias || (uintptr_t)bias % 16 == 0) &&
                  (!aux || auxm == AUX_NONE || vec_ok(aux, ldaux)) && (uintptr_t)part % 16 == 0 &&
                  (long long)S * M * N < (1ll << 31) && (long long)M * ldc < (1ll << 31) &&
                  (long long)M * ldaux < (1ll << 31) &&
                  (long long)M * N >= (1 << 19);
  return PendEpi{M, N, S, part, C, ldc, beta, bias, act, auxm, aux, ldaux, rowpart, rowsum, v4 ? 1 : 0};
}
static void launch_epi(const PendEpi& e, hipStream_t st) {
  long long n_el = (e.v4 ? (long long)e.M * e.N / 4 : (long long)e.M * e.N) + (e.rowsum ? e.M : 0);
  int g = cdiv(n_el, 256);
  if (g > 4096) g = 4096;
  if (e.v4)
    hipLaunchKernelGGL(gemm_splitk_epilogue_v_k, dim3(g), dim3(256), 0, st, e.M, e.N, e.S, e.part, e.C, (int)e.ldc,
                       e.beta, e.bias, e.act, e.auxm, e.aux, (int)e.ldaux, e.rowpart, e.rowsum);
  else
    hipLaunchKernelGGL(gemm_splitk_epilogue_k, dim3(g), dim3(256), 0, st, e.M, e.N, e.S, e.part, e.C, e.ldc, e.beta,
                       e.bias, e.act, e.auxm, e.aux, e.ldaux, e.rowpart, e.rowsum);
}
void paig_gemm_splitk_finish(int M, int N, int S, const float* part, float* C, long long ldc, float beta,
                             const float* bias, int act, int auxm, const float* aux, long long ldaux,
                             const float* rowpart, float* rowsum, hipStream_t st) {
  launch_epi(make_epi(M, N, S, part, C, ldc, beta, bias, act, auxm, aux, ldaux, rowpart, rowsum), st);
}

static PendEpi g_pend{};
static bool g_defer_next = false;
static PendEpi take_pending() {
  const PendEpi e = g_pend;
  g_pend = PendEpi{};
  return e;
}

extern "C" {

int paig_gemm_ex(int ta, int tb, int M, int N, int K, float alpha, const float* A, long long lda, const float* B,
                 long long ldb, float beta, float* C, long long ldc, const float* bias, int act, int auxm,
                 const float* aux, long long ldaux, float* rowsum, float* ws, size_t ws_floats, int math,
                 void* stream);

size_t paig_gemm_workspace(int M, int N, int K) {
  size_t need = 0;
  for (int math : {0, 4}) {
    const GemmPlan p = plan_gemm(M, N, K, math);
    if (p.S > 1) need = std::max(need, (size_t)p.S * M * N + (size_t)p.S * M);
  }
  return need;
}

int paig_gemm_defer_epilogue(int on) {
  g_defer_next = on != 0;
  return 0;
}

int paig_gemm_flush(void* stream) {
  const PendEpi e = take_pending();
  if (!e.S) return 0;
  launch_epi(e, (hipStream_t)stream);
  PAIG_CHECK_LAUNCH();
  return 0;
}

int paig_gemm(int ta, int tb, int M, int N, int K, float alpha, const float* A, long long lda, const float* B,
              long long ldb, float beta, float* C, long long ldc, const float* bias, int act, int auxm,
              const float* aux, long long ldaux, float* rowsum, float* ws, size_t ws_floats, void* stream) {
  return paig_gemm_ex(ta, tb, M, N, K, alpha, A, lda, B, ldb, beta, C, ldc, bias, act, auxm, aux, ldaux, rowsum, ws,
                      ws_floats, 0, stream);
}

size_t paig_gemm_parts_size(int M, int N, int K, int math) {
  if (M <= 0 || N <= 0) return 0;
  const GemmPlan p = plan_gemm(M, N, K, math);
  return (size_t)(p.S > 1 ? p.S : 1) * M * N;
}

int paig_gemm_parts(int ta, int tb, int M, int N, int K, const float* A, long long lda, const float* B,
                    long long ldb, float* part, size_t part_floats, int math, void* stream) {
  hipStream_t st = (hipStream_t)stream;
  if (int rc = paig_gemm_flush(stream)) return rc;
  PAIG_REQUIRE(math >= 0 && math <= 6, "paig_gemm_parts: math must be 0..6, got %d", math);
  PAIG_REQUIRE(M > 0 && N > 0 && K > 0 && part, "paig_gemm_parts: empty shape (%d x %d x %d) or no slabs", M, N, K);
  const int va = vec_ok(A, lda) && (ta ? M % 4 == 0 : K % 4 == 0);
  const int vb = vec_ok(B, ldb) && (tb ? K % 4 == 0 : N % 4 == 0);
  GemmPlan plan = plan_gemm(M, N, K, math);
  if (plan.tile && !(va && vb)) plan = GemmPlan{0, choose_split(M, N, K)};
  int S = plan.S;
  if (S > 1 && part_floats < (size_t)S * M * N) S = 1;
  PAIG_REQUIRE(part_floats >= (size_t)M * N, "paig_gemm_parts: %zu floats for a %d x %d slab", part_floats, M, N);
  const int kchunk = S > 1 ? cdiv(cdiv(K, S), BK) * BK : K;
  S = cdiv(K, kchunk);
  const int bm = plan.tile == 2 ? 256 : BM, bn = plan.tile == 1 ? 256 : BN;
  dim3 grid(cdiv(N, bn), cdiv(M, bm), S);
#define PAIG_G(TA_, TB_)                                                                                        \
  launch_gemm<TA_, TB_>(math, plan.tile, grid, st, M, N, K, kchunk, 1.f, A, lda, va, B, ldb, vb, nullptr, N, 0.f, \
                        nullptr, 0, 0, nullptr, 0, part, nullptr, nullptr, PendEpi{})
  if (ta && tb) PAIG_G(true, true);
  else if (ta) PAIG_G(true, false);
  else if (tb) PAIG_G(false, true);
  else PAIG_G(false, false);
#undef PAIG_G
  PAIG_CHECK_LAUNCH();
  return S;
}

int paig_gemm_ex(int ta, int tb, int M, int N, int K, float alpha, const float* A, long long lda, const float* B,
                 long long ldb, float beta, float* C, long long ldc, const float* bias, int act, int auxm,
                 const float* aux, long long ldaux, float* rowsum, float* ws, size_t ws_floats, int math,
                 void* stream) {
  hipStream_t st = (hipStream_t)stream;
  if (math < 0 || math > 6) {
    paig_set_error("paig_gemm_ex: math must be 0..6, got %d", math);
    return PAIG_E_UNSUPPORTED;
  }
  if (rowsum && !ta) math = 0;
  const bool defer = g_defer_next;
  g_defer_next = false;
  if (M <= 0 || N <= 0) return paig_gemm_flush(stream);
  const int va = vec_ok(A, lda) && (ta ? M % 4 == 0 : K % 4 == 0);
  const int vb = vec_ok(B, ldb) && (tb ? K % 4 == 0 : N % 4 == 0);
  GemmPlan plan = plan_gemm(M, N, K, math);
  if (plan.tile && !(va && vb)) plan = GemmPlan{0, K > 0 ? choose_split(M, N, K) : 1};
  const int tile = plan.tile;
  int S = plan.S;
  if (S > 1 && (ws == nullptr || ws_floats < (size_t)S * M * N + (size_t)S * M)) S = 1;
  const int kchunk = S > 1 ? cdiv(cdiv(K, S), BK) * BK : (K > 0 ? K : 1);
  S = K > 0 ? cdiv(K, kchunk) : 1;
  const int bm = tile == 2 ? 256 : BM, bn = tile == 1 ? 256 : BN;
  dim3 grid(cdiv(N, bn), cdiv(M, bm), S);
  float* part = S > 1 ? ws : nullptr;
  float* rowpart = (S > 1 && rowsum) ? ws + (size_t)S * M * N : nullptr;
  const PendEpi pe = take_pending();
  PAIG_REQUIRE(!pe.S || !part || (pe.part != part && pe.rowpart != part),
               "paig_gemm_ex: the deferred epilogue's partial slabs share this GEMM's workspace");
#define PAIG_G(TA_, TB_)                                                                                       \
  launch_gemm<TA_, TB_>(math, tile, grid, st, M, N, K, kchunk, alpha, A, lda, va, B, ldb, vb, C, ldc, beta, bias, act, auxm, \
                        aux, ldaux, part, rowsum, rowpart, pe)
  if (ta && tb) PAIG_G(true, true);
  else if (ta) PAIG_G(true, false);
  else if (tb) PAIG_G(false, true);
  else PAIG_G(false, false);
#undef PAIG_G
  PAIG_CHECK_LAUNCH();
  if (S > 1) {
    const PendEpi e = make_epi(M, N, S, part, C, ldc, beta, bias, act, auxm, aux, ldaux, rowpart, rowsum);
    if (defer) {
      g_pend = e;
    } else {
      launch_epi(e, st);
      PAIG_CHECK_LAUNCH();
    }
  }
  return 0;
}

}

PAIG_F16_RANGE_ACCESSOR(paig_f16_range_gemm)
```

paig_reproduction_amd/engine.py:

```python
import ctypes
import os
from dataclasses import dataclass, field
from typing import NamedTuple

import torch

from ._lib import PaigError, lib, ptr, stream_handle, require_device



class Switches(NamedTuple):
    fuse_head: bool
    dense_tail: bool
    fuse_vfn: bool
    merge_roll: bool
    fused_bwd: bool
    upt: bool
    pool_fold: bool
    wprep_merge: bool
    fuse_vel: bool
    fuse_vfn2: bool
    gemm_epi_merge: bool


def read_switches():
    return Switches(*[os.environ.get("PAIG_" + f.upper(), "1") != "0" for f in Switches._fields])


class LossAdjoints(NamedTuple):
    dt: object
    de: object
    dr: object
    ae: float
    B: int
    Te: int
    R: int
    pred: int


def materialise(adj, mode, dev):
    w = _empty(adj.B * (adj.Te if mode == 1 else adj.R), dev)
    lib().paig_loss_bwd(ptr(adj.dt), ptr(adj.de), ptr(adj.dr), float(adj.ae), ptr(w) if mode == 1 else None,
                        ptr(w) if mode == 2 else None, adj.B, adj.Te, adj.R, adj.pred, stream_handle(dev))
    return w


def live_steps(d_out, d_sse_roll, ent_roll):
    if d_out is None and d_sse_roll is None and ent_roll and all(adj.de is None for _, adj in ent_roll):
        return ent_roll[0][1].pred
    return 0


class Layout:

    def __init__(self, model, B, T, sw, frames=None, net=None):
        self.B, self.T, self.sw = B, T, sw
        self.sequences = frames is None
        self.K = model.n_objs
        self.D = model.coord_units // 2
        self.H = model.conv_input_shape[1]
        self.h = self.H // 2
        self.ins, self.pred = model.input_steps, model.pred_steps
        self.Te = self.ins + self.pred
        self.R = model.pred_steps + model.extrap_steps
        if frames is None:
            assert T == model.seq_len, f"input has {T} frames, model expects seq_len={model.seq_len}"
            self.F = B * self.Te
        else:
            self.F = frames
        self.alt_vel = model.alt_vel
        self.cell = {"spring_ode_cell": 0, "bouncing_ode_cell": 1, "gravity_ode_cell": 2}[model.cell_type]
        self.unet = self.H >= 40 if net is None else net == "unet"
        L = lib()
        self.net = 1 if self.unet else 0
        self.prefix = "encoder.unet." if self.unet else "encoder.shallow_unet."
        self.nconv = L.paig_unet_query(self.net, self.K, 0)
        self.lg_relu = not self.unet
        self.l1_in = 3 * (self.H // 2) ** 2 if self.unet else 3 * self.H * self.H
        self.HW = self.H * self.H
        self.frame = 3 * self.HW
        self.vfn_sizes = (self.K * self.h * self.h, self.K * 3 * self.h * self.h, 3 * self.HW)
        self.head_buf = L.paig_unet_query(self.net, self.K, 2)
        self.head_ci = L.paig_unet_query(self.net, self.K, 3)
        self.head_name = f"c{self.nconv}"
        self.head_flags = (1 if self.lg_relu else 0) | (2 if self.unet else 0)
        self.fuse_head = (self.K in (2, 3) and self.HW % 4 == 0 and sw.fuse_head and
                          ((not self.unet and self.head_ci == 8) or (self.unet and self.head_ci == 16 and
                                                                     self.H % 4 == 0)))
        if self.fuse_head:
            off, cbuf = L.paig_unet_query(self.net, self.K, 5), L.paig_unet_query(self.net, self.K, 6)
            if off != 0 or cbuf != self.head_ci:
                raise PaigError(f"U-Net head input at channel offset {off} of a {cbuf}-channel buffer: the fused "
                                f"head needs the whole buffer ({self.head_ci} channels from offset 0)")


class KernelProbe:

    backlog_cycles = 1 << 20

    def __init__(self, tag):
        self.tag = tag
        self.events = {}
        self.work = {}

    def wrap(self, tag, flops, nbytes=0):
        probe = self
        want = probe.tag is None or tag == probe.tag

        class _Ctx:
            def __enter__(self):
                if want:
                    self.e0 = torch.cuda.Event(enable_timing=True)
                    self.e1 = torch.cuda.Event(enable_timing=True)
                    torch.cuda._sleep(probe.backlog_cycles)
                    self.e0.record()
                return self

            def __exit__(self, *exc):
                if want:
                    self.e1.record()
                    probe.events.setdefault(tag, []).append((self.e0, self.e1))
                    probe.work[tag] = (flops, nbytes)
                return False

        return _Ctx()

    def overhead_ms(self, n=20):
        pairs = []
        for _ in range(n):
            e0, e1 = torch.cuda.Event(enable_timing=True), torch.cuda.Event(enable_timing=True)
            torch.cuda._sleep(self.backlog_cycles)
            e0.record()
            torch.cuda._sleep(0)
            e1.record()
            pairs.append((e0, e1))
        torch.cuda.synchronize()
        return min(a.elapsed_time(b) for a, b in pairs)

    def summaries(self):
        torch.cuda.synchronize()
        ovh = self.overhead_ms() if self.events else 0.0
        out = {}
        for tag, evs in self.events.items():
            ms = [a.elapsed_time(b) for a, b in evs]
            fl, nb = self.work[tag]
            raw = sum(ms) / len(ms)
            out[tag] = {"tag": tag, "n": len(ms), "avg_ms": max(raw - ovh, 1e-6), "avg_ms_raw": raw,
                        "overhead_ms": ovh, "flops": fl, "bytes": nb}
        return out

    def summary(self):
        s = self.summaries()
        return s.get(self.tag) if self.tag is not None else None


class _NoProbe:
    def __enter__(self):
        return self

    def __exit__(self, *exc):
        return False


_NOPROBE = _NoProbe()


def _parr(ptrs):
    return (ctypes.c_void_p * len(ptrs))(*ptrs)


def _iarr(vals):
    return (ctypes.c_int * len(vals))(*vals)


def _empty(n, device, dtype=torch.float32):
    return torch.empty(n, device=device, dtype=dtype)


_VFN = ("var_net_template", "var_net_content", "var_net_background")
_NO_VEL = (None, None, 0, 0, 0, 0)
_NO_VFN2 = (0,) + (None,) * 11


@dataclass(slots=True, eq=False)
class StepState:
    lay: Layout = None
    x: object = None
    ws: object = None
    dev: object = None
    cm: int = 0
    need_saved: bool = True
    sw: Switches = None
    x_view: tuple = None
    sigma: float = 1.0
    tb: int = 0
    tgt_roll: tuple = None
    src: dict = None
    Xv: object = None
    v1: object = None
    v2: object = None
    vel0: object = None
    pvs: object = None
    wprep: dict = None
    wprep_buf: object = None
    logits: object = None
    head_in: object = None
    unet_ws: object = None
    unet_flags: int = 0
    unet_wp: tuple = None
    dense_tail: bool = False
    w2t: object = None
    masks: object = None
    objs: object = None
    l1_x: object = None
    h1: object = None
    h2: object = None
    h3: object = None
    enc_pos: object = None
    extra_slabs: list = field(default_factory=list)
    consumed: bool = False
    probe_cb: object = None

    def release(self):
        self.unet_ws = None
        self.consumed = True

    def check_fresh(self):
        if self.consumed:
            raise PaigError("a second backward through one forward (retain_graph=True) is not supported: the "
                            "forward's saved state (its U-Net workspace) was released by the first backward")


class Engine:

    def __init__(self, model):
        self.model = model
        self.L = lib()
        self.probe = None
        self.last_masked_objs = None
        self.last_sigma = 1.0
        self.last_loss_handoff = None
        self.bucket_hook = model._flat.allreduce_early
        self.byte_targets = None

    CONV_MATH = {"split": 128, "fp32": 0, "bf16": 256}

    GEMM_MATH = {"split": (6, 6, 6), "fp32": (0, 0, 0), "bf16": (3, 3, 3)}
    FWD, WGRAD, DGRAD = 0, 1, 2

    def gemm_math(self, kind):
        return self.GEMM_MATH[getattr(self.model, "conv_math", "split")][kind]

    def conv_flags(self):
        m = getattr(self.model, "conv_math", "split")
        if m not in self.CONV_MATH:
            raise ValueError(f"conv_math must be one of {sorted(self.CONV_MATH)}, got {m!r}")
        return self.CONV_MATH[m]

    @staticmethod
    def _dec_bytes(n, lay, tb=4):
        return n * lay.frame * (tb + 4)

    @staticmethod
    def _dec_bwd_bytes(live, n, lay, dense, tb=4):
        return (live * lay.frame * (tb + (4 if dense else 0)) + n * 2 * lay.D * 4
                + (4 * lay.K * lay.h * lay.h + 3 * lay.HW) * 4)

    def _p(self, tag, flops=0, nbytes=0):
        return self.probe.wrap(tag, flops, nbytes) if self.probe is not None else _NOPROBE

    def p(self, name):
        return self.model._param_by_name[name]

    def g(self, name):
        return self.model._flat.grad_view(name)

    def linear(self, x, rows, name, out, act, st, ws):
        W, b = self.p(name + ".weight"), self.p(name + ".bias")
        O, I = W.shape
        with self._p("gemm_fwd:" + name, 2 * rows * O * I, 4 * (rows * I + O * I + rows * O)):
            self.L.paig_gemm_ex(0, 1, rows, O, I, 1.0, ptr(x), I, ptr(W), I, 0.0, ptr(out), O, ptr(b), act, 0, None,
                                0, None, ptr(ws), ws.numel() if ws is not None else 0, self.gemm_math(self.FWD), st)

    def linear_bwd(self, x, dy, rows, name, dx, aux, auxm, st, ws, need_dx=True, defer_epi=False):
        W = self.p(name + ".weight")
        O, I = W.shape
        gW, gb = self.g(name + ".weight"), self.g(name + ".bias")
        n_ws = ws.numel()
        if defer_epi:
            self.L.paig_gemm_defer_epilogue(1)
        with self._p("gemm_wgrad:" + name, 2 * rows * O * I, 4 * (rows * O + rows * I + O * I + O)):
            self.L.paig_gemm_ex(1, 0, O, I, rows, 1.0, ptr(dy), O, ptr(x), I, 0.0, ptr(gW), I, None, 0, 0, None, 0,
                                ptr(gb), ptr(ws), n_ws, self.gemm_math(self.WGRAD), st)
        if need_dx:
            with self._p("gemm_dgrad:" + name, 2 * rows * O * I, 4 * (rows * O + O * I + (2 if auxm else 1) * rows * I)):
                self.L.paig_gemm_ex(0, 0, rows, I, O, 1.0, ptr(dy), O, ptr(W), I, 0.0, ptr(dx), I, None, 0, auxm,
                                    ptr(aux), I, None, ptr(ws), n_ws, self.gemm_math(self.DGRAD), st)

    def dense_tail(self, sw):
        return self.gemm_math(self.FWD) == 6 and sw.dense_tail

    def workspace_floats(self, lay):
        K, F, B = lay.K, lay.F, lay.B
        n1 = lay.l1_in
        need = [self.L.paig_gemm_workspace(K * F, 200, n1), self.L.paig_gemm_workspace(K * F, 200, 200),
                self.L.paig_gemm_workspace(200, n1, K * F), self.L.paig_gemm_workspace(K * F, n1, 200), self.L.paig_gemm_workspace(200, 200, K * F),
                self.L.paig_gemm_workspace(2, 200, K * F), self.L.paig_gemm_workspace(100, 100, K * B),
                self.L.paig_gemm_workspace(200, 200, K * F) + self.L.paig_gemm_workspace(200, n1, K * F),
                self.L.paig_gemm_workspace(K * B, 100, 100), 1 << 16,
                self.L.paig_gemm_parts_size(K * F, 200, n1, self.gemm_math(self.FWD))]
        return int(max(need))

    def _velmlp_params(self):
        pm = "velocity_encoder.init_vel_mlp."
        return tuple(ptr(self.p(pm + n)) for n in ("0.weight", "0.bias", "2.weight", "2.bias", "4.weight", "4.bias"))

    def _vfn_fwd_args(self, S):
        return (3, *[_parr([ptr(self.p(nm + suf)) for nm in _VFN])
                     for suf in (".l1.weight", ".l1.bias", ".l2.weight", ".l2.bias")],
                *[_parr([ptr(S.src[nm][i]) for nm in _VFN]) for i in range(3)], _iarr(S.lay.vfn_sizes))

    def _vfn_bwd_args(self, S, dsrc, vparts):
        P = S.lay.vfn_sizes
        return (3, _parr([ptr(dsrc) + o * 4 for o in (0, P[0], P[0] + P[1])]),
                _parr([ptr(S.src[nm][1]) for nm in _VFN]), _iarr([0, 1, 1]),
                _parr([ptr(S.src[nm][0]) for nm in _VFN]), _parr([ptr(self.p(nm + ".l2.weight")) for nm in _VFN]),
                *[_parr([ptr(self.g(nm + suf)) for nm in _VFN])
                  for suf in (".l1.weight", ".l1.bias", ".l2.weight", ".l2.bias")],
                _parr([ptr(pt) for pt in vparts]), _iarr(P))

    def _rollout_args(self, S):
        lay = S.lay
        dt, p0, p1 = self.cell_params(lay)
        return (lay.cell, ptr(S.enc_pos) + (lay.ins - 1) * lay.D * 4, lay.Te * lay.D, ptr(S.vel0), ptr(dt), ptr(p0),
                ptr(p1), ptr(S.pvs), lay.B, lay.D, lay.R)

    def _head_bwd_prefix(self, S, denc, dh2, hslab):
        lay = S.lay
        return (ptr(S.h2), ptr(S.h3), ptr(denc), ptr(self.p("encoder.l3.weight")), ptr(dh2), ptr(hslab), lay.F, lay.K,
                200, float(lay.H / 2))

    def new_state(self, lay, x, need_saved):
        S = StepState()
        S.lay, S.x, S.need_saved, S.sw = lay, x, need_saved, lay.sw
        S.dev = x.device
        S.cm = self.conv_flags()
        S.ws = _empty(self.workspace_floats(lay), S.dev)
        S.x_view = (ptr(x), lay.T * lay.frame, lay.Te, lay.frame) if lay.sequences else (ptr(x), lay.frame, 0, 0)
        return S

    def forward(self, x, need_saved=True):
        require_device(x)
        model = self.model
        model._flat.ensure()
        B, T = x.shape[0], x.shape[1]
        lay = Layout(model, B, T, read_switches())
        L = self.L
        x = x.contiguous()
        sigma = model.decoder_sigma()
        S = self.new_state(lay, x, need_saved)
        S.sigma = self.last_sigma = sigma
        dev, ws, sw = S.dev, S.ws, S.sw
        st = stream_handle(dev)
        K, F, HW, H, h, D = lay.K, lay.F, lay.HW, lay.H, lay.h, lay.D

        S.src = {nm: (_empty(200, dev), _empty(P, dev), _empty(P, dev) if nm == "var_net_background" else None)
                 for nm, P in zip(_VFN, lay.vfn_sizes)}
        tmpl, cont, bgp = S.src["var_net_template"][1], S.src["var_net_content"][1], S.src["var_net_background"][2]

        bt = self.byte_targets
        if bt is not None and bt.covers(x, lay):
            S.tb = 1
            S.tgt_roll = (bt.base + lay.ins * lay.frame, bt.idx_ptr, T * lay.frame, lay.R, lay.frame)
        else:
            S.tgt_roll = (ptr(x) + lay.ins * lay.frame * 4, T * lay.frame, lay.R, lay.frame)
        self._encoder_forward(S, st)
        enc_pos = S.enc_pos

        recons = _empty(F * lay.frame, dev)
        sse_rec = _empty(F, dev)
        if lay.ins > 1:
            S.Xv = _empty(K * B * 2 * (lay.ins - 1 if lay.alt_vel else lay.ins), dev)
            S.vel0 = _empty(K * B * 2, dev)
            if not lay.alt_vel:
                S.v1 = _empty(K * B * 100, dev)
                S.v2 = _empty(K * B * 100, dev)
        S.pvs = _empty(B * (lay.R + 1) * 2 * D, dev)
        roll = self._rollout_args(S)
        vel_act = (ptr(S.Xv), ptr(S.v1), ptr(S.v2), ptr(S.vel0))
        dec = (ptr(enc_pos), 0, 2 * K, 0, ptr(tmpl), ptr(cont), ptr(bgp), ptr(recons), lay.frame, *S.x_view,
               ptr(sse_rec), F, K, h, H, S.sigma)
        fuse_vfn = S.vel0 is not None and not lay.alt_vel and sw.fuse_vfn
        merge_roll = fuse_vfn and self._merge_roll_rec(lay)
        if fuse_vfn:
            L.paig_velmlp_vfn_fwd(ptr(enc_pos), B, lay.Te, K, lay.ins, *self._velmlp_params(), *vel_act,
                                  *self._vfn_fwd_args(S), st)
        elif S.vel0 is not None and lay.alt_vel:
            L.paig_vel_pack(ptr(enc_pos), ptr(S.Xv), B, lay.Te, K, lay.ins, 1, st)
            self.linear(S.Xv, K * B, "velocity_encoder.init_vel_linear", S.vel0, 0, st, ws)
        elif S.vel0 is not None:
            L.paig_velmlp_fwd(ptr(enc_pos), B, lay.Te, K, lay.ins, *self._velmlp_params(), *vel_act, st)
        if not merge_roll:
            L.paig_rollout_fwd(*roll, st)
        if not fuse_vfn:
            L.paig_vfn_fwd_multi(*self._vfn_fwd_args(S), st)
        with self._p("dec_fwd:recon+rollout" if merge_roll else "dec_fwd:recon", 0, self._dec_bytes(F, lay)):
            if merge_roll:
                L.paig_decoder_fwd_rollout_sigma(*roll, *dec, st)
            else:
                L.paig_decoder_fwd_sigma(*dec, st)

        out = _empty(B * lay.R * lay.frame, dev)
        sse_roll = _empty(B * lay.R, dev)
        dec_fwd = L.paig_decoder_fwd_t8_sigma if S.tb else L.paig_decoder_fwd_sigma
        with self._p("dec_fwd:rollout", 0, self._dec_bytes(B * lay.R, lay, S.tb or 4)):
            dec_fwd(ptr(S.pvs) + 2 * D * 4, (lay.R + 1) * 2 * D, 2 * D, lay.R, ptr(tmpl), ptr(cont), ptr(bgp),
                    ptr(out), lay.frame, *S.tgt_roll, ptr(sse_roll), B * lay.R, K, h, H, S.sigma, st)

        masks, objs = S.masks, S.objs
        res = {
            "output_seq": out.view(B, lay.R, 3, H, H),
            "recons_out": recons.view(B, lay.Te, 3, H, H),
            "enc_pos": enc_pos.view(B, lay.Te, D),
            "pos_vel_seq": S.pvs.view(B, lay.R + 1, 2 * D),
            "enc_masks": masks.view(F, K + 1, H, H),
            "masked_objs": [objs[k * F * 3 * HW:(k + 1) * F * 3 * HW].view(F, 3, H, H) for k in range(K)],
            "sse_rec": sse_rec,
            "sse_roll": sse_roll,
            "template": tmpl.view(K, 1, h, h),
            "contents": cont.view(K, 3, h, h),
            "background_content": bgp.view(1, 3, H, H),
        }
        if not need_saved:
            S.release()
        return res, (S if need_saved else None)

    _ROLL_REC = {(2, 32, 0): 256, (2, 32, 1): 256, (3, 36, 2): 384, (2, 64, 0): 1024}

    def _merge_roll_rec(self, lay):
        nt = self._ROLL_REC.get((lay.K, lay.H, lay.cell))
        if nt is None or not lay.sw.merge_roll:
            return False
        return min((lay.F + 1) // 2, 1024) + -(-lay.B // nt) <= 1024

    _PROBE_TAG = {0: "conv_fwd", 1: "conv_bwd", 2: "conv_wgrad", 3: "conv_dgrad"}
    _PROBE_FN = ctypes.CFUNCTYPE(None, ctypes.c_void_p, ctypes.c_int, ctypes.c_int, ctypes.c_int, ctypes.c_int,
                                 ctypes.c_int, ctypes.c_int, ctypes.c_int, ctypes.c_int)

    def _unet_probe(self, S):
        if self.probe is None:
            return None
        lay, F = S.lay, S.lay.F
        open_ = {}

        def cb(ctx, ev, op, conv, kind, cin, cout, Hl, fl):
            if ev == 1:
                open_.pop(op).__exit__(None, None, None)
                return
            ks = self.p(lay.prefix + f"c{conv + 1}.weight").shape[-1]
            flops = 2 * F * cin * cout * ks * ks * Hl * Hl
            up = bool(fl & 32)
            hin = Hl // 2 if up else Hl
            if kind == 0 or kind == 2:
                nbytes = 4 * F * (cin * hin * hin + cout * Hl * Hl)
            elif kind == 1:
                flops *= 2
                if up:
                    nbytes = 4 * F * (cin * hin * hin * (2 if fl & 2 else 1) + cout * Hl * Hl)
                else:
                    nbytes = 4 * F * Hl * Hl * (cin + cout + cin * (2 if fl & 4 else 1))
                    if fl & 64:
                        nbytes += F * (4 * cout + cout) * (Hl // 2) ** 2
            elif fl & 512:
                nbytes = 4 * F * (cout * Hl * Hl + cin * (Hl // 2) ** 2 * (2 if fl & 2 else 1))
            else:
                nbytes = 4 * F * Hl * Hl * (cout + cin * (1 + (1 if fl & 2 else 0) + (1 if fl & 4 else 0)))
            c = self._p(f"{self._PROBE_TAG[kind]}:c{conv + 1}", flops, nbytes)
            c.__enter__()
            open_[op] = c

        S.probe_cb = self._PROBE_FN(cb)
        return ctypes.cast(S.probe_cb, ctypes.c_void_p)

    def _unet_forward(self, S, st, fuse_head=False):
        L = self.L
        lay, sw, dev, cm = S.lay, S.sw, S.dev, S.cm
        F, H, K = lay.F, lay.H, lay.K
        flags = ((1 if fuse_head else 0) | (0 if S.need_saved else 4) |
                 (0 if sw.fused_bwd else 2) |
                 (0 if sw.upt else 16) |
                 (0 if sw.pool_fold else 32))
        Ws = [self.p(lay.prefix + f"c{c + 1}.weight") for c in range(lay.nconv)]
        Bs = [self.p(lay.prefix + f"c{c + 1}.bias") for c in range(lay.nconv)]
        wp = {}
        wpf = wpd = None
        if cm == self.CONV_MATH["split"]:
            flags |= 8
            jobs = []
            for c, W_ in enumerate(Ws):
                cout, cin, ks = W_.shape[0], W_.shape[1], W_.shape[-1]
                jobs.append((c, 0, W_, cin, cout, ks))
                if c > 0:
                    jobs.append((c, 1, W_, cout, cin, ks))
            sizes = [int(L.paig_conv_wprep_size(j[3], j[4], j[5])) for j in jobs]
            if self.dense_tail(sw):
                jobs.append((-1, 2, self.p("encoder.l2.weight"), 200, 200, 1))
                sizes.append(2 * 200 * 200)
            buf = torch.empty(sum(-(-n // 8) * 8 for n in sizes), dtype=torch.int16, device=dev)
            outs, off = [], 0
            for j, n in zip(jobs, sizes):
                wp[(j[0], j[1])] = buf.data_ptr() + 2 * off
                outs.append(wp[(j[0], j[1])])
                off += -(-n // 8) * 8
            n = len(jobs)
            wprep = L.paig_conv_wprep_defer if sw.wprep_merge else L.paig_conv_wprep
            wprep(n, (ctypes.c_void_p * n)(*[ptr(j[2]) for j in jobs]),
                  (ctypes.c_int * n)(*[j[3] for j in jobs]), (ctypes.c_int * n)(*[j[4] for j in jobs]),
                  (ctypes.c_int * n)(*[j[5] for j in jobs]), (ctypes.c_int * n)(*[j[1] for j in jobs]),
                  (ctypes.c_void_p * n)(*outs), st)
            S.wprep_buf = buf
            wpf = _parr([wp[(c, 0)] for c in range(lay.nconv)])
            wpd = _parr([wp.get((c, 1), 0) for c in range(lay.nconv)])
        S.wprep = wp
        nb = int(L.paig_unet_workspace_ex(lay.net, F, H, K, cm, flags))
        if nb <= 0:
            raise PaigError(f"paig_unet_workspace_ex: no U-Net for net={lay.net} F={F} H={H} K={K} math={cm}")
        ws = torch.empty(nb, dtype=torch.uint8, device=dev)
        logits = None if fuse_head else _empty(F * K * lay.HW, dev)
        probe = self._unet_probe(S)
        L.paig_unet_fwd_ex(lay.net, F, H, K, cm, flags, *S.x_view, _parr([ptr(t) for t in Ws]),
                           _parr([ptr(t) for t in Bs]), ptr(logits), wpf, wpd, ptr(ws), nb, probe, None, st)
        if fuse_head:
            off = int(L.paig_unet_buffer(lay.net, F, H, K, cm, flags, 0, lay.head_buf))
            S.head_in = ws[off:off + F * lay.head_ci * lay.HW * 4].view(torch.float32)
        S.logits, S.unet_ws, S.unet_flags, S.unet_wp = logits, ws, flags, (wpf, wpd)

    def _unet_grad(self, S, buf, n):
        lay = S.lay
        off = int(self.L.paig_unet_buffer(lay.net, lay.F, lay.H, lay.K, S.cm, S.unet_flags, 1, buf))
        assert off >= 0, f"no gradient buffer {buf} in the U-Net workspace"
        return S.unet_ws[off:off + n * 4].view(torch.float32)

    def _encoder_forward(self, S, st):
        L = self.L
        lay, x_view, ws, dev = S.lay, S.x_view, S.ws, S.dev
        F, H, HW, K = lay.F, lay.H, lay.HW, lay.K
        self._unet_forward(S, st, fuse_head=lay.fuse_head)
        masks = _empty(F * (K + 1) * HW, dev)
        objs = _empty(K * F * 3 * HW, dev)
        pobjs = _empty(K * F * lay.l1_in, dev) if lay.unet else None
        if lay.fuse_head:
            hn = lay.prefix + lay.head_name
            L.paig_head_mask_fwd_ex(ptr(S.head_in), ptr(self.p(hn + ".weight")), ptr(self.p(hn + ".bias")),
                                    *x_view, ptr(masks), ptr(objs), ptr(pobjs), F, K, lay.head_ci, H, H,
                                    lay.head_flags, st)
        else:
            L.paig_mask_softmax_fwd(ptr(S.logits), *x_view, ptr(masks), ptr(objs), ptr(pobjs), F, K, 3, H, H, st)
        l1_x = pobjs if lay.unet else objs
        h1 = _empty(K * F * 200, dev)
        h2 = _empty(K * F * 200, dev)
        h3 = _empty(K * F * 2, dev)
        if not self.dense_tail(S.sw):
            self.linear(l1_x, K * F, "encoder.l1", h1, 1, st, ws)
            self.linear(h1, K * F, "encoder.l2", h2, 1, st, ws)
            enc_pos = _empty(F * 2 * K, dev)
            L.paig_head_fwd(ptr(h2), ptr(self.p("encoder.l3.weight")), ptr(self.p("encoder.l3.bias")), ptr(h3),
                            ptr(enc_pos), F, K, 200, float(H / 2), st)
        else:
            S.dense_tail = True
            n1, KF = lay.l1_in, K * F
            enc_pos = _empty(F * 2 * K, dev)
            with self._p("gemm_fwd:encoder.l1", 2 * KF * 200 * n1, 4 * (KF * n1 + 200 * n1)):
                nS = L.paig_gemm_parts(0, 1, KF, 200, n1, ptr(l1_x), n1, ptr(self.p("encoder.l1.weight")), n1, ptr(ws),
                                       ws.numel(), self.gemm_math(self.FWD), st)
            if nS <= 0:
                raise PaigError(f"paig_gemm_parts failed (rc={nS}): {L.paig_last_error().decode(errors='replace')}")
            with self._p("dense_tail_fwd", 2 * KF * 200 * 200 + 4 * KF * 200,
                         4 * (nS * KF * 200 + 2 * KF * 200 + 200 * 200 + 2 * KF + 2 * KF)):
                w2t = S.wprep.get((-1, 2))
                w2 = None if w2t is not None else self.p("encoder.l2.weight")
                if w2t is None:
                    S.w2t = _empty(200 * 200, dev)
                    w2t = ptr(S.w2t)
                L.paig_dense_tail_fwd(ptr(ws), nS, ptr(self.p("encoder.l1.bias")), ptr(h1), ptr(w2), w2t,
                                      ptr(self.p("encoder.l2.bias")), ptr(h2),
                                      ptr(self.p("encoder.l3.weight")), ptr(self.p("encoder.l3.bias")), ptr(h3),
                                      ptr(enc_pos), F, K, 200, float(H / 2), st)
        S.masks, S.objs, S.l1_x, S.h1, S.h2, S.h3, S.enc_pos = masks, objs, l1_x, h1, h2, h3, enc_pos

    def cell_params(self, lay):
        m = self.model
        dt = m.rollout_cell.dt
        if lay.cell == 0:
            return dt, m.rollout_cell.k, m.rollout_cell.equil
        if lay.cell == 2:
            return dt, m.rollout_cell.g, m.rollout_cell.m
        return dt, None, None

    def _decoder_bwd(self, S, pos, po, pi, pg, tgt, dsse, lw, dout, dpos, slab_p, scr, nfr, live, st):
        lay = S.lay
        tf, t8, ti = (tgt[0], None, None) if len(tgt) == 4 else (None, tgt[0], tgt[1])
        fs, grp, gs = tgt[-3:]
        if lw is not None:
            mode, adj = lw
            lwa = (mode, ptr(adj.dt), ptr(adj.de), ptr(adj.dr), float(adj.ae), adj.B, adj.Te, adj.R, adj.pred)
            dsse = None
        else:
            lwa = (0, None, None, None, 0.0, 0, 0, 0, 0)
        self.L.paig_decoder_bwd_ex_sigma(pos, po, pi, pg, ptr(S.src["var_net_template"][1]),
                                         ptr(S.src["var_net_content"][1]), ptr(S.src["var_net_background"][2]), tf, t8,
                                         ti, fs, grp, gs, ptr(dsse), *lwa, ptr(dout), lay.frame, dpos, slab_p, scr, nfr,
                                         live, lay.K, lay.h, lay.H, S.sigma, st)

    def backward(self, S, d_sse_rec=None, d_sse_roll=None, d_out=None, d_recons=None, d_enc_pos=None, d_pvs=None,
                 roll_live=0, lossw=None):
        S.check_fresh()
        lay, sw, dev, L = S.lay, S.sw, S.dev, self.L
        st = stream_handle(dev)
        K, F, H, h, D, B, R = lay.K, lay.F, lay.H, lay.h, lay.D, lay.B, lay.R
        lossw = dict(lossw or {})

        if (K, H) not in ((2, 32), (3, 36), (2, 64)):
            if "rec" in lossw:
                d_sse_rec = materialise(lossw.pop("rec")[1], 1, dev)
            if "roll" in lossw:
                d_sse_roll = materialise(lossw.pop("roll")[1], 2, dev)
        if d_out is not None:
            d_out = d_out.contiguous()
        if d_recons is not None:
            d_recons = d_recons.contiguous()

        slab_len = int(L.paig_decoder_slab_len(K, h, H))
        roll_live = roll_live if (d_out is None and 0 < roll_live < R) else 0
        nb_rec = L.paig_decoder_bwd_blocks_sigma(F, 0, 0, K, h, H, S.sigma)
        nb_roll = L.paig_decoder_bwd_blocks_sigma(B * R, R, roll_live, K, h, H, S.sigma)
        slab = _empty((nb_rec + nb_roll) * slab_len, dev)
        scr_n = max(L.paig_decoder_bwd_scratch_sigma(F, K, h, H, S.sigma),
                    L.paig_decoder_bwd_scratch_sigma(B * R, K, h, H, S.sigma))
        scratch = _empty(scr_n, dev) if scr_n else None
        denc = _empty(F * D, dev)
        dpos_roll = _empty(B * R * D, dev)
        dsrc = _empty(slab_len, dev)
        dpos0 = _empty(B * D, dev)
        dvel0 = _empty(K * B * 2, dev) if S.vel0 is not None else None
        rpart = _empty(2 * L.paig_rollout_bwd_blocks(B), dev, torch.float64)
        dXv = vslab = None
        if S.vel0 is not None:
            dXv = _empty(K * B * 2 * (lay.ins - 1 if lay.alt_vel else lay.ins), dev)
            if not lay.alt_vel:
                vblk, vlen = L.paig_velmlp_bwd_blocks(K * B), L.paig_velmlp_slab_len(lay.ins)
                vslab = _empty(vblk * vlen, dev)
        vparts = [_empty(L.paig_vfn_bwd_blocks(P) * 200, dev) for P in lay.vfn_sizes]
        if d_pvs is not None:
            d_pvs = d_pvs.contiguous()
        if d_enc_pos is not None:
            d_enc_pos = d_enc_pos.contiguous()

        live_frames = B * roll_live if roll_live else B * R
        with self._p("dec_bwd:rollout", 0, self._dec_bwd_bytes(live_frames, B * R, lay, d_out is not None, S.tb or 4)):
            self._decoder_bwd(S, ptr(S.pvs) + 2 * D * 4, (R + 1) * 2 * D, 2 * D, R, S.tgt_roll, d_sse_roll,
                              lossw.get("roll"), d_out, ptr(dpos_roll), ptr(slab) + nb_rec * slab_len * 4,
                              ptr(scratch), B * R, roll_live, st)

        prm = self.cell_params(lay)
        gk = gq = None
        if lay.cell == 0:
            gk, gq = self.g("rollout_cell.k"), self.g("rollout_cell.equil")
        elif lay.cell == 2:
            gk = self.g("rollout_cell.g")
        L.paig_rollout_bwd(lay.cell, ptr(S.pvs), ptr(dpos_roll), ptr(d_pvs), ptr(prm[0]), ptr(prm[1]), ptr(prm[2]),
                           ptr(dpos0), ptr(dvel0), ptr(rpart), ptr(gk), ptr(gq), 0, B, D, R, st)
        if S.vel0 is not None and lay.alt_vel:
            self.linear_bwd(S.Xv, dvel0, K * B, "velocity_encoder.init_vel_linear", dXv, None, 0, st, S.ws)
        elif S.vel0 is not None:
            W0, _, W2, _, W4, _ = self._velmlp_params()
            L.paig_velmlp_bwd(ptr(dvel0), ptr(S.Xv), ptr(S.v1), ptr(S.v2), W0, W2, W4, ptr(dXv), ptr(vslab), K * B,
                              lay.ins, st)
            pm = "velocity_encoder.init_vel_mlp."
            g0 = self.g(pm + "0.weight")
            assert self.g(pm + "4.bias").data_ptr() == g0.data_ptr() + (vlen - 2) * 4, \
                "velocity MLP grads not contiguous"
            S.extra_slabs.append((vslab, vblk, vlen, g0))

        with self._p("dec_bwd:recon", 0, self._dec_bwd_bytes(F, F, lay, d_recons is not None)):
            self._decoder_bwd(S, ptr(S.enc_pos), 0, 2 * K, 0, S.x_view, d_sse_rec, lossw.get("rec"), d_recons,
                              ptr(denc), ptr(slab), ptr(scratch), F, 0, st)

        L.paig_slab_reduce_multi(1, (ctypes.c_void_p * 1)(ptr(slab)), (ctypes.c_int * 1)(nb_rec + nb_roll),
                                 (ctypes.c_int * 1)(slab_len), (ctypes.c_void_p * 1)(ptr(dsrc)), 0, st)
        vfn2 = self._vfn_bwd_args(S, dsrc, vparts)
        if sw.fuse_vel and sw.fuse_vfn2:
            L.paig_vfn_bwd1_multi(*vfn2, st)
        else:
            L.paig_vfn_bwd_multi(*vfn2, st)
            vfn2 = None
        if d_enc_pos is not None:
            L.paig_axpby(ptr(d_enc_pos), ptr(denc), F * D, 1.0, 1.0, st)
        vel = (ptr(dXv), ptr(dpos0), B, lay.Te, lay.ins, int(lay.alt_vel))
        if not sw.fuse_vel:
            L.paig_vel_unpack_add(vel[0], vel[1], ptr(denc), B, lay.Te, K, lay.ins, int(lay.alt_vel), st)
            vel = None
        self._encoder_backward(S, denc, st, vel=vel, vfn2=vfn2)

    def _encoder_backward(self, S, denc, st, hook=True, vel=None, vfn2=None):
        lay, dev, ws, x_view, L = S.lay, S.dev, S.ws, S.x_view, self.L
        K, F, HW, H = lay.K, lay.F, lay.HW, lay.H
        dh2 = _empty(K * F * 200, dev)
        dh1 = _empty(K * F * 200, dev)
        fused_l2 = S.dense_tail
        hblk = L.paig_head_l2_bwd_blocks(K * F) if fused_l2 else L.paig_head_bwd_blocks(K * F)
        hslab = _empty(hblk * (2 * 200 + 2), dev)
        head = self._head_bwd_prefix(S, denc, dh2, hslab)
        if fused_l2:
            L.paig_head_l2_bwd(*head, *(vel or _NO_VEL), ptr(self.p("encoder.l2.weight")), ptr(S.h1), ptr(dh1),
                               *(vfn2 or _NO_VFN2), st)
        elif vfn2 is not None:
            L.paig_head_bwd_vel_vfn2(*head, *vel, *vfn2, st)
        elif vel is not None:
            L.paig_head_bwd_vel(*head, *vel, st)
        else:
            L.paig_head_bwd(*head, st)
        g3 = self.g("encoder.l3.weight")
        assert self.g("encoder.l3.bias").data_ptr() == g3.data_ptr() + 400 * 4, "l3 grads not contiguous"
        S.extra_slabs.append((hslab, hblk, 402, g3))
        dobjs = _empty(K * F * lay.l1_in, dev)
        merge = S.sw.gemm_epi_merge and not self.probe
        w2 = int(L.paig_gemm_workspace(200, 200, K * F)) if merge else 0
        self.linear_bwd(S.h1, dh2, K * F, "encoder.l2", dh1, S.h1, 1, st, ws, need_dx=not fused_l2,
                        defer_epi=merge)
        self.linear_bwd(S.l1_x, dh1, K * F, "encoder.l1", dobjs, None, 0, st, ws[w2:] if merge else ws,
                        defer_epi=merge)
        if merge:
            L.paig_gemm_flush(st)
        if hook and self.bucket_hook is not None:
            self.bucket_hook()

        if S.head_in is not None:
            hn, c = lay.prefix + lay.head_name, lay.head_ci
            dXl = self._unet_grad(S, lay.head_buf, F * c * HW)
            nb = L.paig_head_mask_blocks(F, H, H)
            nw = K * c + K
            hs = _empty(nb * nw, dev)
            L.paig_head_mask_bwd_ex(ptr(S.head_in), ptr(self.p(hn + ".weight")), ptr(self.p(hn + ".bias")),
                                    *x_view, ptr(S.masks), ptr(dobjs), ptr(dXl), ptr(hs), F, K, c, H, H,
                                    lay.head_flags, st)
            gh = self.g(hn + ".weight")
            assert self.g(hn + ".bias").data_ptr() == gh.data_ptr() + K * c * 4, "head grads not contiguous"
            S.extra_slabs.append((hs, nb, nw, gh))
            self._unet_backward(S, None, st)
        else:
            dLG = _empty(F * K * HW, dev)
            L.paig_mask_softmax_bwd(ptr(S.logits), *x_view, ptr(S.masks), ptr(dobjs), ptr(dLG), F, K, 3, H, H,
                                    (1 if lay.lg_relu else 0) | (2 if lay.unet else 0), st)
            self._unet_backward(S, dLG, st)

    def _unet_backward(self, S, dlogits, st):
        S.check_fresh()
        lay = S.lay
        L = self.L
        Ws = [self.p(lay.prefix + f"c{c + 1}.weight") for c in range(lay.nconv)]
        dwb = []
        for c in range(lay.nconv):
            gw = self.g(lay.prefix + f"c{c + 1}.weight")
            assert self.g(lay.prefix + f"c{c + 1}.bias").data_ptr() == gw.data_ptr() + gw.numel() * 4, \
                "flat grads: weight and bias must be adjacent"
            dwb.append(ptr(gw))
        extra = S.extra_slabs
        n = len(extra)
        ws = S.unet_ws
        _, wpd = S.unet_wp
        L.paig_unet_bwd_ex(lay.net, lay.F, lay.H, lay.K, S.cm, S.unet_flags, *S.x_view,
                           _parr([ptr(t) for t in Ws]), ptr(S.logits), ptr(dlogits), _parr(dwb), n,
                           _parr([ptr(e[0]) for e in extra]), _iarr([e[1] for e in extra]),
                           _iarr([e[2] for e in extra]), _parr([ptr(e[3]) for e in extra]), wpd, ptr(ws), ws.numel(),
                           self._unet_probe(S), None, st)
        S.release()
```

Measured before the change: 98770 video-seqs/s.

## Pre-split encoder.l1 weight into f16 hi/lo tiles once per step for GEMMs

Adds a weight-prep job that converts the encoder.l1 weight into per-K-chunk scaled f16 hi/lo tile images, with a per-tile exponent, inside the existing conv_wprep launch. The forward parts-GEMM and the backward dgrad GEMM then load these pre-split tiles directly instead of reading fp32 B, computing the absmax and splitting it in every block. This removes repeated conversion work and the per-tile B max reduction, at the cost of an extra prep pass, an extra buffer, and new PRE template kernel variants. A wide-tile force flag and a shared split4_scaled helper are also added.

```diff
diff --git a/include/paig_hip.h b/include/paig_hip.h
--- a/include/paig_hip.h
+++ b/include/paig_hip.h
@@ -129,6 +129,17 @@
 size_t paig_gemm_parts_size(int M, int N, int K, int math);
 int paig_gemm_parts(int ta, int tb, int M, int N, int K, const float* A, long long lda, const float* B,
                     long long ldb, float* part, size_t part_floats, int math, void* stream);
+int paig_gemm_presplit_kchunk(int form, int M, int N, int K, int math);
+long long paig_gemm_presplit_size(int form, int N, int K);
+int paig_gemm_presplit_count(int clear);
+int paig_debug_gemm_wide(int on);
+int paig_gemm_parts_pre(int ta, int tb, int M, int N, int K, const float* A, long long lda, const float* B,
+                        long long ldb, float* part, size_t part_floats, int math, void* stream, const void* bpre,
+                        int pre_n, int pre_k, int pre_kchunk);
+int paig_gemm_ex_pre(int ta, int tb, int M, int N, int K, float alpha, const float* A, long long lda, const float* B,
+                     long long ldb, float beta, float* C, long long ldc, const float* bias, int act, int auxm,
+                     const float* aux, long long ldaux, float* rowsum, float* ws, size_t ws_floats, int math,
+                     void* stream, const void* bpre, int pre_n, int pre_k, int pre_kchunk);
 size_t paig_colsum_workspace(int M, int N);
 int paig_colsum(const float* X, int M, int N, long long ld, float* out, int accumulate, float* ws, void* stream);
 int paig_slab_reduce(const float* slab, int nblk, long long ld, int len, float* out, int accumulate, void* stream);
diff --git a/paig_reproduction_amd/_lib.py b/paig_reproduction_amd/_lib.py
--- a/paig_reproduction_amd/_lib.py
+++ b/paig_reproduction_amd/_lib.py
@@ -85,6 +85,12 @@
     "paig_gemm_workspace": (SZ, [I, I, I]),
     "paig_gemm_parts_size": (SZ, [I, I, I, I]),
     "paig_gemm_parts": (I, [I, I, I, I, I, P, LL, P, LL, P, SZ, I, P]),
+    "paig_gemm_presplit_kchunk": (I, [I, I, I, I, I]),
+    "paig_gemm_presplit_size": (LL, [I, I, I]),
+    "paig_gemm_presplit_count": (I, [I]),
+    "paig_debug_gemm_wide": (I, [I]),
+    "paig_gemm_parts_pre": (I, [I, I, I, I, I, P, LL, P, LL, P, SZ, I, P, P, I, I, I]),
+    "paig_gemm_ex_pre": (I, [I, I, I, I, I, F32, P, LL, P, LL, F32, P, LL, P, I, I, P, LL, P, P, SZ, I, P, P, I, I, I]),
     "paig_gemm_defer_epilogue": (I, [I]),
     "paig_gemm_flush": (I, [P]),
     "paig_gemm": (I, [I, I, I, I, I, F32, P, LL, P, LL, F32, P, LL, P, I, I, P, LL, P, P, SZ, P]),
@@ -150,7 +156,8 @@
           "paig_debug_fwd_block_cap",
           "paig_conv2d_bwd_supported", "paig_velmlp_bwd_blocks",
           "paig_velmlp_slab_len", "paig_head_bwd_blocks", "paig_head_l2_bwd_blocks", "paig_head_mask_blocks", "paig_conv_wprep_size", "paig_gemm_workspace", "paig_colsum_workspace",
-          "paig_gemm_parts_size", "paig_gemm_parts", "paig_unet_workspace", "paig_unet_workspace_ex",
+          "paig_gemm_parts_size", "paig_gemm_parts", "paig_gemm_parts_pre", "paig_gemm_presplit_kchunk",
+          "paig_gemm_presplit_size", "paig_gemm_presplit_count", "paig_debug_gemm_wide", "paig_unet_workspace", "paig_unet_workspace_ex",
           "paig_unet_buffer", "paig_unet_query", "paig_localiser_workspace",
           "paig_velmlp_rollout_bwd_workspace",
           "paig_vfn_bwd_blocks", "paig_rollout_bwd_blocks", "paig_decoder_bwd_blocks", "paig_decoder_slab_len",
diff --git a/paig_reproduction_amd/csrc/conv_split.hip b/paig_reproduction_amd/csrc/conv_split.hip
--- a/paig_reproduction_amd/csrc/conv_split.hip
+++ b/paig_reproduction_amd/csrc/conv_split.hip
@@ -1,4 +1,5 @@
 #include "split_common.h"
+#include "gemm_presplit.h"
 
 #ifndef PAIG_FWD_AUXP
 #define PAIG_FWD_AUXP 1
@@ -1361,6 +1362,12 @@
   int q = 0;
   while (q + 1 < jobs.n && bid >= jobs.blk0[q + 1]) ++q;
   const WPrepJob jb = jobs.j[q];
+  if (jb.dg >= 3) {
+    const int form = jb.dg - 3;
+    gemm_presplit_body(jb.w, reinterpret_cast<short*>(jb.out), form, form == 0 ? jb.cout : jb.cin,
+                       form == 0 ? jb.cin : jb.cout, jb.cin, jb.ks, bid - jobs.blk0[q]);
+    return;
+  }
   if (jb.dg == 2) {
     __shared__ float T[32][33];
     const int bl = bid - jobs.blk0[q], tx = (bl % ((jb.cin + 31) / 32)) * 32,
@@ -1442,6 +1449,13 @@
     PAIG_REQUIRE(((uintptr_t)out[q] & 15) == 0, "conv_wprep: job %d output not 16-byte aligned", q);
     jobs.j[q] = WPrepJob{w[q], static_cast<s16x8*>(out[q]), cin[q], cout[q], ks[q], dg[q]};
     jobs.blk0[q] = blocks;
+    if (dg[q] == 3 || dg[q] == 4) {
+      PAIG_REQUIRE(((uintptr_t)w[q] & 15) == 0 && cin[q] % 4 == 0, "conv_wprep: job %d needs float4 weight rows", q);
+      const int form = dg[q] - 3;
+      blocks += presplit_blocks(form == 0 ? cout[q] : cin[q], form == 0 ? cin[q] : cout[q], form);
+      continue;
+    }
+    PAIG_REQUIRE(dg[q] >= 0 && dg[q] <= 2, "conv_wprep: job %d kind %d", q, dg[q]);
     if (dg[q] == 2) {
       blocks += (cin[q] + 31) / 32 * ((cout[q] + 31) / 32);
       continue;
diff --git a/paig_reproduction_amd/csrc/gemm.hip b/paig_reproduction_amd/csrc/gemm.hip
--- a/paig_reproduction_amd/csrc/gemm.hip
+++ b/paig_reproduction_amd/csrc/gemm.hip
@@ -1,6 +1,8 @@
 #include "common.h"
+#include "gemm_presplit.h"
 
 #include <algorithm>
+#include <type_traits>
 #include <cstdlib>
 
 namespace {
@@ -225,10 +227,6 @@
 constexpr int SPR = 80;
 constexpr int SIMG = 64 * SPK > BK * SPR ? 64 * SPK : BK * SPR;
 
-__device__ __forceinline__ int kperm(int k) {
-  const int g = k >> 3, h = (k >> 2) & 1, q = k & 3;
-  return 16 * (g >> 1) + 8 * h + 4 * (g & 1) + q;
-}
 
 #define F16PM(PM) ((PM) == 1 || (PM) == 4 || (PM) == 5 || (PM) == 6)
 #define SCALED(PM) ((PM) >= 4)
@@ -264,13 +262,9 @@
   for (int e = 0; e < 2; ++e) {
     s16x4 hv, lv;
     if constexpr (F16PM(PM)) {
-      const pf32x2 a = pf32x2{t.v[e][0], t.v[e][1]} * sc, b = pf32x2{t.v[e][2], t.v[e][3]} * sc;
-      rmax = amax2(amax2(rmax, a.x, a.y), b.x, b.y);
-      u32x2 h, l;
-      { const HiLo q_ = split_pk(a.x, a.y); h[0] = q_.h; l[0] = q_.l; }
-      { const HiLo q_ = split_pk(b.x, b.y); h[1] = q_.h; l[1] = q_.l; }
-      hv = __builtin_bit_cast(s16x4, h);
-      lv = __builtin_bit_cast(s16x4, l);
+      const HiLo4 q_ = split4_scaled(t.v[e][0], t.v[e][1], t.v[e][2], t.v[e][3], sc, rmax);
+      hv = __builtin_bit_cast(s16x4, u32x2{q_.h[0], q_.h[1]});
+      lv = __builtin_bit_cast(s16x4, u32x2{q_.l[0], q_.l[1]});
     } else {
 #pragma unroll
       for (int i = 0; i < 4; ++i) {
@@ -299,13 +293,48 @@
   return __builtin_shufflevector(lo, hi, 0, 1, 2, 3, 4, 5, 6, 7);
 }
 
-template <bool TA, bool TB, int PM, bool VEC>
+typedef unsigned u32x4 __attribute__((ext_vector_type(4)));
+struct PreB {
+  const u32x4* img;
+  const int* ex;
+  int nkt;
+};
+template <int CH, int NTHR, int CPR>
+struct PTile {
+  u32x4 h[CH], l[CH];
+  int e;
+  __device__ __forceinline__ void load(const PreB& pb, int nt, int k0, int kend, int nrows, int tid) {
+    const bool ok = k0 < kend;
+    const long long t = (long long)nt * pb.nkt + k0 / BK;
+    const u32x4* q = pb.img + t * (2 * CH * NTHR) + tid;
+    const u32x4* z = reinterpret_cast<const u32x4*>(zero16);
+#pragma unroll
+    for (int c = 0; c < CH; ++c) {
+      const bool okc = ok && (tid + c * NTHR) / CPR < nrows;
+      h[c] = *(okc ? q + c * NTHR : z);
+      l[c] = *(okc ? q + (CH + c) * NTHR : z);
+    }
+    e = pb.ex[ok ? t : 0];
+  }
+  template <int PITCH>
+  __device__ __forceinline__ void store(short* ih, short* il, int tid) const {
+#pragma unroll
+    for (int c = 0; c < CH; ++c) {
+      const int i = tid + c * NTHR, o = (i / CPR) * PITCH + (i % CPR) * 8;
+      *reinterpret_cast<u32x4*>(ih + o) = h[c];
+      *reinterpret_cast<u32x4*>(il + o) = l[c];
+    }
+  }
+};
+
+template <bool TA, bool TB, int PM, bool VEC, bool PRE = false>
 __global__ void __launch_bounds__(256) __attribute__((amdgpu_waves_per_eu(6)))
 gemm_split_k(int M, int N, int K, int kchunk, float alpha, const float* __restrict__ A, long long lda, int veca,
              const float* __restrict__ B, long long ldb, int vecb, float* __restrict__ C, long long ldc, float beta,
              const float* __restrict__ bias, int act, int auxm, const float* __restrict__ aux, long long ldaux,
-             float* __restrict__ part, float* __restrict__ rowsum, float* __restrict__ rowpart, PendEpi pe) {
+             float* __restrict__ part, float* __restrict__ rowsum, float* __restrict__ rowpart, PendEpi pe, PreB pb) {
   PAIG_PENDING_EPI(pe)
+  static_assert(!PRE || (PM == 6 && !TB && VEC), "pre-split op(B): math 6, row-contiguous B");
   constexpr int NI = PM == 3 ? 1 : 2;
   __shared__ __attribute__((aligned(16))) short S16[4 * SIMG];
   short* Ah = S16;
@@ -338,11 +367,15 @@
 
   constexpr int NS = 1;
   Tile<!TA> ta[NS];
-  Tile<TB> tb[NS];
+  std::conditional_t<PRE, PTile<1, 256, 8>, Tile<TB>> tb[NS];
+  auto load_b = [&](int st, int kk) {
+    if constexpr (PRE) tb[st].load(pb, bt.x, kk, kend, BK, tid);
+    else tb[st].template load_bf<VEC>(B, ldb, n0, kk, N, kend, tid);
+  };
 #pragma unroll
   for (int st = 0; st < NS; ++st) {
     ta[st].template load_bf<VEC>(A, lda, m0, kbeg + st * BK, M, kend, tid);
-    tb[st].template load_bf<VEC>(B, ldb, n0, kbeg + st * BK, N, kend, tid);
+    load_b(st, kbeg + st * BK);
   }
   for (int k0 = kbeg; k0 < kend; k0 += NS * BK) {
 #pragma unroll
@@ -356,7 +389,7 @@
         ma = wave_max_u(ma);
         if (lane == 0) smx[wv] = ma;
       }
-      if constexpr (DB) {
+      if constexpr (DB && !PRE) {
         float mb = 0.f;
 #pragma unroll
         for (int e = 0; e < 2; ++e) mb = amax2(amax2(mb, tb[st].v[e][0], tb[st].v[e][1]), tb[st].v[e][2], tb[st].v[e][3]);
@@ -367,7 +400,8 @@
       if constexpr (DA || DB) {
         int na = eca, nb = ecb;
         if constexpr (DA) na = min(eca, f16_scale_exp(fmaxf(fmaxf(smx[0], smx[1]), fmaxf(smx[2], smx[3]))));
-        if constexpr (DB) nb = min(ecb, f16_scale_exp(fmaxf(fmaxf(smx[4], smx[5]), fmaxf(smx[6], smx[7]))));
+        if constexpr (PRE) nb = uniform_i(tb[st].e);
+        else if constexpr (DB) nb = min(ecb, f16_scale_exp(fmaxf(fmaxf(smx[4], smx[5]), fmaxf(smx[6], smx[7]))));
         if (na + nb < eca + ecb) {
 #pragma unroll
           for (int i = 0; i < 2; ++i)
@@ -384,12 +418,13 @@
       }
       float dmx = 0.f;
       store16<!TA, PM>(ta[st], Ah, Al, tid, asc, DA ? dmx : rmax);
-      store16<TB, PM>(tb[st], Bh, Bl, tid, bsc, DB ? dmx : rmax);
+      if constexpr (PRE) tb[st].template store<SPR>(Bh, Bl, tid);
+      else store16<TB, PM>(tb[st], Bh, Bl, tid, bsc, DB ? dmx : rmax);
       if (do_rs) rs4 += ta[st].v[0] + ta[st].v[1];
       __syncthreads();
       }
       ta[st].template load_bf<VEC>(A, lda, m0, kk + NS * BK, M, kend, tid);
-      tb[st].template load_bf<VEC>(B, ldb, n0, kk + NS * BK, N, kend, tid);
+      load_b(st, kk + NS * BK);
       if (kk < kend) {
       s16x8 ah[2], al[2], bh[2], bl[2];
 #pragma unroll
@@ -488,16 +523,13 @@
   __device__ __forceinline__ void store16(short* ih, short* il, int tid, float sc, float& rmax) const {
 #pragma unroll
     for (int e = 0; e < E; ++e) {
-      const pf32x2 a = pf32x2{v[e][0], v[e][1]} * sc, b = pf32x2{v[e][2], v[e][3]} * sc;
       s16x4 hv, lv;
       if constexpr (F16PM(PM)) {
-        rmax = amax2(amax2(rmax, a.x, a.y), b.x, b.y);
-        u32x2 h, l;
-        { const HiLo q_ = split_pk(a.x, a.y); h[0] = q_.h; l[0] = q_.l; }
-        { const HiLo q_ = split_pk(b.x, b.y); h[1] = q_.h; l[1] = q_.l; }
-        hv = __builtin_bit_cast(s16x4, h);
-        lv = __builtin_bit_cast(s16x4, l);
+        const HiLo4 q_ = split4_scaled(v[e][0], v[e][1], v[e][2], v[e][3], sc, rmax);
+        hv = __builtin_bit_cast(s16x4, u32x2{q_.h[0], q_.h[1]});
+        lv = __builtin_bit_cast(s16x4, u32x2{q_.l[0], q_.l[1]});
       } else {
+        const pf32x2 a = pf32x2{v[e][0], v[e][1]} * sc, b = pf32x2{v[e][2], v[e][3]} * sc;
         const float t[4] = {a.x, a.y, b.x, b.y};
 #pragma unroll
         for (int i = 0; i < 4; ++i) {
@@ -531,13 +563,14 @@
   }
 };
 
-template <bool TA, bool TB, int PM, bool VEC, int BMT, int BNT>
+template <bool TA, bool TB, int PM, bool VEC, int BMT, int BNT, bool PRE = false>
 __global__ void __launch_bounds__(512)
 gemm_split_w_k(int M, int N, int K, int kchunk, float alpha, const float* __restrict__ A, long long lda, int veca,
                const float* __restrict__ B, long long ldb, int vecb, float* __restrict__ C, long long ldc, float beta,
                const float* __restrict__ bias, int act, int auxm, const float* __restrict__ aux, long long ldaux,
-               float* __restrict__ part, float* __restrict__ rowsum, float* __restrict__ rowpart, PendEpi pe) {
+               float* __restrict__ part, float* __restrict__ rowsum, float* __restrict__ rowpart, PendEpi pe, PreB pb) {
   PAIG_PENDING_EPI(pe)
+  static_assert(!PRE || (PM == 6 && TB && VEC && BNT == 256), "pre-split op(B): math 6, k-contiguous B, 64 x 256");
   constexpr int WM = BMT == 64 ? 2 : 4, WN = 8 / WM;
   constexpr int PMW = BMT / WM, PNW = BNT / WN;
   constexpr int MI = PMW / 16, NJ = PNW / 16;
@@ -575,11 +608,15 @@
 
   constexpr int NS = 3;
   TTA ta[NS];
-  TTB tb[NS];
+  std::conditional_t<PRE, PTile<2, 512, 4>, TTB> tb[NS];
+  auto load_b = [&](int st, int kk) {
+    if constexpr (PRE) tb[st].load(pb, bt.x, kk, kend, N - n0, tid);
+    else tb[st].template load_bf<VEC>(B, ldb, n0, kk, N, kend, tid);
+  };
 #pragma unroll
   for (int st = 0; st < NS; ++st) {
     ta[st].template load_bf<VEC>(A, lda, m0, kbeg + st * BK, M, kend, tid);
-    tb[st].template load_bf<VEC>(B, ldb, n0, kbeg + st * BK, N, kend, tid);
+    load_b(st, kbeg + st * BK);
   }
   for (int k0 = kbeg; k0 < kend; k0 += NS * BK) {
 #pragma unroll
@@ -590,7 +627,7 @@
         const float ma = wave_max_u(ta[st].amax());
         if (lane == 0) smx[wv] = ma;
       }
-      if constexpr (DB) {
+      if constexpr (DB && !PRE) {
         const float mb = wave_max_u(tb[st].amax());
         if (lane == 0) smx[8 + wv] = mb;
       }
@@ -603,7 +640,9 @@
           for (int w = 1; w < 8; ++w) m = fmaxf(m, smx[w]);
           na = min(eca, f16_scale_exp(m));
         }
-        if constexpr (DB) {
+        if constexpr (PRE) {
+          nb = uniform_i(tb[st].e);
+        } else if constexpr (DB) {
           float m = smx[8];
 #pragma unroll
           for (int w = 9; w < 16; ++w) m = fmaxf(m, smx[w]);
@@ -625,7 +664,8 @@
       }
       float dmx = 0.f;
       ta[st].template store16<PM>(Ah, Al, tid, asc, DA ? dmx : rmax);
-      tb[st].template store16<PM>(Bh, Bl, tid, bsc, DB ? dmx : rmax);
+      if constexpr (PRE) tb[st].template store<SPK>(Bh, Bl, tid);
+      else tb[st].template store16<PM>(Bh, Bl, tid, bsc, DB ? dmx : rmax);
       if (do_rs) {
 #pragma unroll
         for (int e = 0; e < TTA::E; ++e) rs4 += ta[st].v[e];
@@ -633,7 +673,7 @@
       __syncthreads();
       }
       ta[st].template load_bf<VEC>(A, lda, m0, kk + NS * BK, M, kend, tid);
-      tb[st].template load_bf<VEC>(B, ldb, n0, kk + NS * BK, N, kend, tid);
+      load_b(st, kk + NS * BK);
       if (kk < kend) {
       s16x8 ah[MI], al[MI], bh[NJ], bl[NJ];
 #pragma unroll
@@ -826,15 +866,16 @@
   }
   return v;
 }
+static bool g_force_wide = false;
 static GemmPlan plan_gemm(int M, int N, int K, int math) {
   GemmPlan p{0, K > 0 ? choose_split(M, N, K) : 1};
   if (!(math == 3 || math == 4 || math == 6) || gemm_tile_env() == 0 || K <= 0) return p;
   int tile = 0;
-  if (N > 128 && N <= 256 && M >= 512 && K >= 512) tile = 1;
+  if (N > 128 && N <= 256 && (M >= 512 || g_force_wide) && K >= 512) tile = 1;
   if (!tile) return p;
   int S = 1;
   while (K / (2 * S) >= 384) S *= 2;
-  if ((long long)S * M * N > (8ll << 20) || cdiv(M, 64) * S < 128) return p;
+  if ((long long)S * M * N > (8ll << 20) || (cdiv(M, 64) * S < 128 && !g_force_wide)) return p;
   return GemmPlan{tile, S};
 }
 
@@ -846,15 +887,16 @@
 static void launch_gemm(int math, int tile, dim3 grid, hipStream_t st, int M, int N, int K, int kchunk, float alpha,
                         const float* A, long long lda, int va, const float* B, long long ldb, int vb, float* C,
                         long long ldc, float beta, const float* bias, int act, int auxm, const float* aux,
-                        long long ldaux, float* part, float* rowsum, float* rowpart, const PendEpi& pe) {
+                        long long ldaux, float* part, float* rowsum, float* rowpart, const PendEpi& pe,
+                        const PreB& pb = PreB{}) {
   if (pe.S) grid.z += 1;
 #define PAIG_L(KERN)                                                                                          \
   hipLaunchKernelGGL(KERN, grid, dim3(256), 0, st, M, N, K, kchunk, alpha, A, lda, va, B, ldb, vb, C, ldc, beta, \
-                     bias, act, auxm, aux, ldaux, part, rowsum, rowpart, pe)
+                     bias, act, auxm, aux, ldaux, part, rowsum, rowpart, pe, pb)
   const bool v = va && vb;
 #define PAIG_W(KERN) \
   hipLaunchKernelGGL(KERN, grid, dim3(512), 0, st, M, N, K, kchunk, alpha, A, lda, va, B, ldb, vb, C, ldc, beta, \
-                     bias, act, auxm, aux, ldaux, part, rowsum, rowpart, pe)
+                     bias, act, auxm, aux, ldaux, part, rowsum, rowpart, pe, pb)
 #define PAIG_S(PM_) \
   do {                                              \
     if (v) PAIG_L((gemm_split_k<TA, TB, PM_, true>)); \
@@ -866,13 +908,20 @@
     else if (tile == 2) PAIG_W((gemm_split_w_k<TA, TB, PM_, true, 256, 64>)); \
     else PAIG_S(PM_);                                                   \
   } while (0)
+  if (pb.img) {
+    if constexpr (!TA && TB) PAIG_W((gemm_split_w_k<false, true, 6, true, 64, 256, true>));
+    else if constexpr (!TA && !TB) PAIG_L((gemm_split_k<false, false, 6, true, true>));
+    return;
+  }
   if (math == 1) PAIG_S(1);
   else if (math == 2) PAIG_S(2);
   else if (math == 3) PAIG_SW(3);
   else if (math == 4) PAIG_SW(4);
   else if (math == 5) PAIG_S(5);
   else if (math == 6) PAIG_SW(6);
-  else PAIG_L((gemm_k<TA, TB>));
+  else
+    hipLaunchKernelGGL((gemm_k<TA, TB>), grid, dim3(256), 0, st, M, N, K, kchunk, alpha, A, lda, va, B, ldb, vb, C, ldc,
+                       beta, bias, act, auxm, aux, ldaux, part, rowsum, rowpart, pe);
 #undef PAIG_SW
 #undef PAIG_S
 #undef PAIG_W
@@ -915,6 +964,21 @@
   return e;
 }
 
+struct PreArg {
+  const void* img;
+  int n, k, kchunk;
+};
+static PreB pre_for(const PreArg& pa, int form, int math, int ta, int tb, int tile, bool vec, int N, int K,
+                    int kchunk) {
+  const bool ok = pa.img && math == 6 && !ta && tb == (form == 0) && tile == (form == 0 ? 1 : 0) && vec &&
+                  pa.n == N && pa.k == K && pa.kchunk == kchunk && (uintptr_t)pa.img % 16 == 0;
+  if (!ok) return PreB{};
+  const short* base = static_cast<const short*>(pa.img);
+  return PreB{reinterpret_cast<const u32x4*>(base + presplit_hdr(N, K, form)), reinterpret_cast<const int*>(base),
+              cdiv(K, BK)};
+}
+static int g_pre_used = 0;
+
 extern "C" {
 
 int paig_gemm_ex(int ta, int tb, int M, int N, int K, float alpha, const float* A, long long lda, const float* B,
@@ -957,8 +1021,35 @@
   return (size_t)(p.S > 1 ? p.S : 1) * M * N;
 }
 
+int paig_gemm_presplit_kchunk(int form, int M, int N, int K, int math) {
+  if (math != 6 || M <= 0 || N <= 0 || K <= 0 || (form != 0 && form != 1)) return 0;
+  if ((form == 0 ? K : N) % 4 != 0) return 0;
+  const GemmPlan p = plan_gemm(M, N, K, math);
+  if (p.tile != (form == 0 ? 1 : 0)) return 0;
+  return p.S > 1 ? cdiv(cdiv(K, p.S), BK) * BK : K;
+}
+long long paig_gemm_presplit_size(int form, int N, int K) {
+  return (form != 0 && form != 1) || N <= 0 || K <= 0 ? 0 : presplit_elems(N, K, form);
+}
+int paig_debug_gemm_wide(int on) {
+  const int prev = g_force_wide ? 1 : 0;
+  g_force_wide = on != 0;
+  return prev;
+}
+int paig_gemm_presplit_count(int clear) {
+  const int v = g_pre_used;
+  if (clear) g_pre_used = 0;
+  return v;
+}
+
 int paig_gemm_parts(int ta, int tb, int M, int N, int K, const float* A, long long lda, const float* B,
                     long long ldb, float* part, size_t part_floats, int math, void* stream) {
+  return paig_gemm_parts_pre(ta, tb, M, N, K, A, lda, B, ldb, part, part_floats, math, stream, nullptr, 0, 0, 0);
+}
+
+int paig_gemm_parts_pre(int ta, int tb, int M, int N, int K, const float* A, long long lda, const float* B,
+                        long long ldb, float* part, size_t part_floats, int math, void* stream, const void* bpre,
+                        int pre_n, int pre_k, int pre_kchunk) {
   hipStream_t st = (hipStream_t)stream;
   if (int rc = paig_gemm_flush(stream)) return rc;
   PAIG_REQUIRE(math >= 0 && math <= 6, "paig_gemm_parts: math must be 0..6, got %d", math);
@@ -974,9 +1065,11 @@
   S = cdiv(K, kchunk);
   const int bm = plan.tile == 2 ? 256 : BM, bn = plan.tile == 1 ? 256 : BN;
   dim3 grid(cdiv(N, bn), cdiv(M, bm), S);
+  const PreB pb = pre_for(PreArg{bpre, pre_n, pre_k, pre_kchunk}, 0, math, ta, tb, plan.tile, va && vb, N, K, kchunk);
+  if (pb.img) ++g_pre_used;
 #define PAIG_G(TA_, TB_)                                                                                        \
   launch_gemm<TA_, TB_>(math, plan.tile, grid, st, M, N, K, kchunk, 1.f, A, lda, va, B, ldb, vb, nullptr, N, 0.f, \
-                        nullptr, 0, 0, nullptr, 0, part, nullptr, nullptr, PendEpi{})
+                        nullptr, 0, 0, nullptr, 0, part, nullptr, nullptr, PendEpi{}, pb)
   if (ta && tb) PAIG_G(true, true);
   else if (ta) PAIG_G(true, false);
   else if (tb) PAIG_G(false, true);
@@ -990,6 +1083,14 @@
                  long long ldb, float beta, float* C, long long ldc, const float* bias, int act, int auxm,
                  const float* aux, long long ldaux, float* rowsum, float* ws, size_t ws_floats, int math,
                  void* stream) {
+  return paig_gemm_ex_pre(ta, tb, M, N, K, alpha, A, lda, B, ldb, beta, C, ldc, bias, act, auxm, aux, ldaux, rowsum, ws,
+                          ws_floats, math, stream, nullptr, 0, 0, 0);
+}
+
+int paig_gemm_ex_pre(int ta, int tb, int M, int N, int K, float alpha, const float* A, long long lda, const float* B,
+                     long long ldb, float beta, float* C, long long ldc, const float* bias, int act, int auxm,
+                     const float* aux, long long ldaux, float* rowsum, float* ws, size_t ws_floats, int math,
+                     void* stream, const void* bpre, int pre_n, int pre_k, int pre_kchunk) {
   hipStream_t st = (hipStream_t)stream;
   if (math < 0 || math > 6) {
     paig_set_error("paig_gemm_ex: math must be 0..6, got %d", math);
@@ -1015,9 +1116,12 @@
   const PendEpi pe = take_pending();
   PAIG_REQUIRE(!pe.S || !part || (pe.part != part && pe.rowpart != part),
                "paig_gemm_ex: the deferred epilogue's partial slabs share this GEMM's workspace");
+  const PreB pb = K > 0 ? pre_for(PreArg{bpre, pre_n, pre_k, pre_kchunk}, 1, math, ta, tb, tile, va && vb, N, K, kchunk)
+                        : PreB{};
+  if (pb.img) ++g_pre_used;
 #define PAIG_G(TA_, TB_)                                                                                       \
   launch_gemm<TA_, TB_>(math, tile, grid, st, M, N, K, kchunk, alpha, A, lda, va, B, ldb, vb, C, ldc, beta, bias, act, auxm, \
-                        aux, ldaux, part, rowsum, rowpart, pe)
+                        aux, ldaux, part, rowsum, rowpart, pe, pb)
   if (ta && tb) PAIG_G(true, true);
   else if (ta) PAIG_G(true, false);
   else if (tb) PAIG_G(false, true);
diff --git a/paig_reproduction_amd/csrc/gemm_presplit.h b/paig_reproduction_amd/csrc/gemm_presplit.h
--- /dev/null
+++ b/paig_reproduction_amd/csrc/gemm_presplit.h
@@ -0,0 +1,91 @@
+#pragma once
+#include "common.h"
+
+namespace {
+
+constexpr int PS_BK = 32;
+
+__device__ __forceinline__ int kperm(int k) {
+  const int g = k >> 3, h = (k >> 2) & 1, q = k & 3;
+  return 16 * (g >> 1) + 8 * h + 4 * (g & 1) + q;
+}
+
+struct HiLo4 {
+  unsigned h[2], l[2];
+};
+__device__ __forceinline__ HiLo4 split4_scaled(float v0, float v1, float v2, float v3, float sc, float& rmax) {
+  const pf32x2 a = pf32x2{v0, v1} * sc, b = pf32x2{v2, v3} * sc;
+  rmax = amax2(amax2(rmax, a.x, a.y), b.x, b.y);
+  const HiLo p = split_pk(a.x, a.y), q = split_pk(b.x, b.y);
+  return HiLo4{{p.h, q.h}, {p.l, q.l}};
+}
+
+__host__ __device__ inline int presplit_rows(int form) { return form == 0 ? 256 : 64; }
+__host__ __device__ inline long long presplit_hdr(int N, int K, int form) {
+  const long long t = (long long)((N + presplit_rows(form) - 1) / presplit_rows(form)) * ((K + PS_BK - 1) / PS_BK);
+  return (2 * t + 7) / 8 * 8;
+}
+__host__ __device__ inline int presplit_piece(int form) { return presplit_rows(form) * PS_BK; }
+__host__ __device__ inline long long presplit_elems(int N, int K, int form) {
+  const long long t = (long long)((N + presplit_rows(form) - 1) / presplit_rows(form)) * ((K + PS_BK - 1) / PS_BK);
+  return presplit_hdr(N, K, form) + t * 2 * presplit_piece(form);
+}
+__host__ __device__ inline int presplit_blocks(int N, int K, int form) {
+  return (N + presplit_rows(form) - 1) / presplit_rows(form) * ((K + PS_BK - 1) / PS_BK);
+}
+
+__device__ __forceinline__ void gemm_presplit_body(const float* __restrict__ w, short* __restrict__ out, int form,
+                                                   int N, int K, int ldb, int kchunk, int bl) {
+  typedef float v4f __attribute__((ext_vector_type(4)));
+  const int ROWS = presplit_rows(form), NKT = (K + PS_BK - 1) / PS_BK;
+  const int nt = bl / NKT, kt = bl - nt * NKT;
+  const int n0 = nt * ROWS, k0 = kt * PS_BK;
+  const int kbeg = k0 / kchunk * kchunk;
+  const int kend = kbeg + kchunk < K ? kbeg + kchunk : K;
+  const int kup = k0 + PS_BK < kend ? k0 + PS_BK : kend;
+  const int tid = threadIdx.x, lane = tid & 63, wv = tid >> 6;
+  const int nr = (N - n0 < ROWS ? N - n0 : ROWS), nk = kup - kbeg;
+  float m = 0.f;
+  if (form == 0) {
+    const int q4 = nk >> 2;
+#pragma unroll 4
+    for (int i = tid; i < nr * q4; i += 256) {
+      const int r = i / q4, k = (i - r * q4) * 4;
+      const v4f v = *reinterpret_cast<const v4f*>(w + (long long)(n0 + r) * ldb + kbeg + k);
+      m = amax2(amax2(m, v[0], v[1]), v[2], v[3]);
+    }
+  } else {
+    const int q4 = nr >> 2;
+#pragma unroll 4
+    for (int i = tid; i < nk * q4; i += 256) {
+      const int k = i / q4, c = (i - k * q4) * 4;
+      const v4f v = *reinterpret_cast<const v4f*>(w + (long long)(kbeg + k) * ldb + n0 + c);
+      m = amax2(amax2(m, v[0], v[1]), v[2], v[3]);
+    }
+  }
+  __shared__ float pmx[4];
+  m = wave_max_u(m);
+  if (lane == 0) pmx[wv] = m;
+  __syncthreads();
+  const int e = f16_scale_exp(fmaxf(fmaxf(pmx[0], pmx[1]), fmaxf(pmx[2], pmx[3])));
+  const float sc = __builtin_amdgcn_ldexpf(1.f, e);
+  if (tid == 0) reinterpret_cast<int*>(out)[bl] = e;
+  const int P = presplit_piece(form);
+  short* ih = out + presplit_hdr(N, K, form) + (long long)bl * 2 * P;
+  short* il = ih + P;
+  const int upr = form == 0 ? 8 : 16;
+  for (int u = tid; u < P / 4; u += 256) {
+    const int row = u / upr, c = (u - row * upr) * 4;
+    const int gn = n0 + (form == 0 ? row : c), gk = k0 + (form == 0 ? c : row);
+    v4f v = v4f{0.f, 0.f, 0.f, 0.f};
+    if (gn < N && gk < kend)
+      v = *reinterpret_cast<const v4f*>(w + (form == 0 ? (long long)gn * ldb + gk : (long long)gk * ldb + gn));
+    float dmx = 0.f;
+    const HiLo4 s = split4_scaled(v[0], v[1], v[2], v[3], sc, dmx);
+    const int o = form == 0 ? row * PS_BK + c : kperm(row) * 64 + c;
+    *reinterpret_cast<uint2*>(ih + o) = make_uint2(s.h[0], s.h[1]);
+    *reinterpret_cast<uint2*>(il + o) = make_uint2(s.l[0], s.l[1]);
+  }
+}
+
+}
diff --git a/paig_reproduction_amd/engine.py b/paig_reproduction_amd/engine.py
--- a/paig_reproduction_amd/engine.py
+++ b/paig_reproduction_amd/engine.py
@@ -25,6 +25,10 @@
 
 def read_switches():
     return Switches(*[os.environ.get("PAIG_" + f.upper(), "1") != "0" for f in Switches._fields])
+
+
+def read_l1_wsplit():
+    return os.environ.get("PAIG_L1_WSPLIT", "1") != "0"
 
 
 class LossAdjoints(NamedTuple):
@@ -180,6 +184,7 @@
 _VFN = ("var_net_template", "var_net_content", "var_net_background")
 _NO_VEL = (None, None, 0, 0, 0, 0)
 _NO_VFN2 = (0,) + (None,) * 11
+_NO_PRE = (None, 0, 0, 0)
 
 
 @dataclass(slots=True, eq=False)
@@ -203,6 +208,8 @@
     pvs: object = None
     wprep: dict = None
     wprep_buf: object = None
+    l1_wsplit: bool = True
+    l1_pre: dict = None
     logits: object = None
     head_in: object = None
     unet_ws: object = None
@@ -282,7 +289,7 @@
             self.L.paig_gemm_ex(0, 1, rows, O, I, 1.0, ptr(x), I, ptr(W), I, 0.0, ptr(out), O, ptr(b), act, 0, None,
                                 0, None, ptr(ws), ws.numel() if ws is not None else 0, self.gemm_math(self.FWD), st)
 
-    def linear_bwd(self, x, dy, rows, name, dx, aux, auxm, st, ws, need_dx=True, defer_epi=False):
+    def linear_bwd(self, x, dy, rows, name, dx, aux, auxm, st, ws, need_dx=True, defer_epi=False, bpre=None):
         W = self.p(name + ".weight")
         O, I = W.shape
         gW, gb = self.g(name + ".weight"), self.g(name + ".bias")
@@ -294,8 +301,9 @@
                                 ptr(gb), ptr(ws), n_ws, self.gemm_math(self.WGRAD), st)
         if need_dx:
             with self._p("gemm_dgrad:" + name, 2 * rows * O * I, 4 * (rows * O + O * I + (2 if auxm else 1) * rows * I)):
-                self.L.paig_gemm_ex(0, 0, rows, I, O, 1.0, ptr(dy), O, ptr(W), I, 0.0, ptr(dx), I, None, 0, auxm,
-                                    ptr(aux), I, None, ptr(ws), n_ws, self.gemm_math(self.DGRAD), st)
+                self.L.paig_gemm_ex_pre(0, 0, rows, I, O, 1.0, ptr(dy), O, ptr(W), I, 0.0, ptr(dx), I, None, 0, auxm,
+                                        ptr(aux), I, None, ptr(ws), n_ws, self.gemm_math(self.DGRAD), st,
+                                        *(bpre or _NO_PRE))
 
     def dense_tail(self, sw):
         return self.gemm_math(self.FWD) == 6 and sw.dense_tail
@@ -345,7 +353,8 @@
         S.lay, S.x, S.need_saved, S.sw = lay, x, need_saved, lay.sw
         S.dev = x.device
         S.cm = self.conv_flags()
-        S.ws = _empty(self.workspace_floats(lay), S.dev)
+        S.l1_wsplit = read_l1_wsplit()
+        S.ws =_empty(self.workspace_floats(lay), S.dev)
         S.x_view = (ptr(x), lay.T * lay.frame, lay.Te, lay.frame) if lay.sequences else (ptr(x), lay.frame, 0, 0)
         return S
 
@@ -482,7 +491,7 @@
         S.probe_cb = self._PROBE_FN(cb)
         return ctypes.cast(S.probe_cb, ctypes.c_void_p)
 
-    def _unet_forward(self, S, st, fuse_head=False):
+    def _unet_forward(self, S, st, fuse_head=False, l1=False):
         L = self.L
         lay, sw, dev, cm = S.lay, S.sw, S.dev, S.cm
         F, H, K = lay.F, lay.H, lay.K
@@ -506,7 +515,19 @@
             if self.dense_tail(sw):
                 jobs.append((-1, 2, self.p("encoder.l2.weight"), 200, 200, 1))
                 sizes.append(2 * 200 * 200)
-            buf = torch.empty(sum(-(-n // 8) * 8 for n in sizes), dtype=torch.int16, device=dev)
+            l1_pre = {}
+            if l1 and S.l1_wsplit and self.gemm_math(self.FWD) == 6:
+                W1 = self.p("encoder.l1.weight")
+                O, I = W1.shape
+                KF = K * F
+                plans = [(0, O, I, self.dense_tail(sw))] + ([(1, I, O, True)] if S.need_saved else [])
+                for form, n_, k_, want in plans:
+                    kc = int(L.paig_gemm_presplit_kchunk(form, KF, n_, k_, 6)) if want else 0
+                    if kc > 0:
+                        jobs.append((-1, 3 + form, W1, I, O, kc))
+                        sizes.append(int(L.paig_gemm_presplit_size(form, n_, k_)))
+                        l1_pre[form] = (n_, k_, kc)
+            buf =torch.empty(sum(-(-n // 8) * 8 for n in sizes), dtype=torch.int16, device=dev)
             outs, off = [], 0
             for j, n in zip(jobs, sizes):
                 wp[(j[0], j[1])] = buf.data_ptr() + 2 * off
@@ -519,7 +540,8 @@
                   (ctypes.c_int * n)(*[j[5] for j in jobs]), (ctypes.c_int * n)(*[j[1] for j in jobs]),
                   (ctypes.c_void_p * n)(*outs), st)
             S.wprep_buf = buf
-            wpf = _parr([wp[(c, 0)] for c in range(lay.nconv)])
+            S.l1_pre = {form: (wp[(-1, 3 + form)],) + d for form, d in l1_pre.items()}
+            wpf =_parr([wp[(c, 0)] for c in range(lay.nconv)])
             wpd = _parr([wp.get((c, 1), 0) for c in range(lay.nconv)])
         S.wprep = wp
         nb = int(L.paig_unet_workspace_ex(lay.net, F, H, K, cm, flags))
@@ -545,7 +567,7 @@
         L = self.L
         lay, x_view, ws, dev = S.lay, S.x_view, S.ws, S.dev
         F, H, HW, K = lay.F, lay.H, lay.HW, lay.K
-        self._unet_forward(S, st, fuse_head=lay.fuse_head)
+        self._unet_forward(S, st, fuse_head=lay.fuse_head, l1=True)
         masks = _empty(F * (K + 1) * HW, dev)
         objs = _empty(K * F * 3 * HW, dev)
         pobjs = _empty(K * F * lay.l1_in, dev) if lay.unet else None
@@ -571,8 +593,9 @@
             n1, KF = lay.l1_in, K * F
             enc_pos = _empty(F * 2 * K, dev)
             with self._p("gemm_fwd:encoder.l1", 2 * KF * 200 * n1, 4 * (KF * n1 + 200 * n1)):
-                nS = L.paig_gemm_parts(0, 1, KF, 200, n1, ptr(l1_x), n1, ptr(self.p("encoder.l1.weight")), n1, ptr(ws),
-                                       ws.numel(), self.gemm_math(self.FWD), st)
+                nS = L.paig_gemm_parts_pre(0, 1, KF, 200, n1, ptr(l1_x), n1, ptr(self.p("encoder.l1.weight")), n1,
+                                           ptr(ws), ws.numel(), self.gemm_math(self.FWD), st,
+                                           *((S.l1_pre or {}).get(0) or _NO_PRE))
             if nS <= 0:
                 raise PaigError(f"paig_gemm_parts failed (rc={nS}): {L.paig_last_error().decode(errors='replace')}")
             with self._p("dense_tail_fwd", 2 * KF * 200 * 200 + 4 * KF * 200,
@@ -729,7 +752,7 @@
         self.linear_bwd(S.h1, dh2, K * F, "encoder.l2", dh1, S.h1, 1, st, ws, need_dx=not fused_l2,
                         defer_epi=merge)
         self.linear_bwd(S.l1_x, dh1, K * F, "encoder.l1", dobjs, None, 0, st, ws[w2:] if merge else ws,
-                        defer_epi=merge)
+                        defer_epi=merge, bpre=(S.l1_pre or {}).get(1))
         if merge:
             L.paig_gemm_flush(st)
         if hook and self.bucket_hook is not None:
```

Result: no change. 99290 video-seqs/s, median of 6 (+0.5%).
